# insitro/FastVim

Hardware: AMD Instinct MI355X
Metric: images/sec FastVim-T 224px bs=128/GPU fwd+bwd (+all-reduce +AdamW +EMA), whole job (higher is better)
Workload: dtype bf16; 1 GPU; FastVim-T 224x224 bs=128/GPU bf16 training step, synthetic ImageNet tensors (BASELINE configs[1]); global_batch=128, parallelism=dp1, hip_graph=True, optimizer_in_step=True, final_loss_hex=0x1.779ca20000000p+0

## Files before the change

### fastvim_amd/_lib.py

```python
import ctypes
import os
import threading

import torch

_PKG = os.path.dirname(os.path.abspath(__file__))
LIB_PATH = os.path.join(_PKG, "libfastvim_hip.so")

FV_F32, FV_BF16, FV_F16 = 0, 1, 2
_DTYPES = {torch.float32: FV_F32, torch.bfloat16: FV_BF16, torch.float16: FV_F16}

_lib = None

C_ABI_SYMBOLS = (
    "fv_last_error", "fv_version",
    "fv_selective_scan_fwd", "fv_selective_scan_bwd_workspace", "fv_selective_scan_bwd",
    "fv_causal_conv1d_fwd", "fv_causal_conv1d_bwd", "fv_scan_expand_skip_fwd",
    "fv_mixer_conv_pool_fwd", "fv_mixer_scan_fwd", "fv_mixer_xproj_scan_fwd_ok", "fv_mixer_xproj_scan_fwd", "fv_mixer_combine_fwd",
    "fv_mixer_bwd_blocks", "fv_mixer_combine_bwd", "fv_mixer_scan_bwd_chunks", "fv_mixer_scan_bwd_chunks_b",
    "fv_mixer_scan_bwd_ckpt_floats", "fv_mixer_scan_bwd_partials", "fv_mixer_scan_bwd", "fv_mixer_scan_bwd_dir", "fv_mixer_scan_bwd_ckpt", "fv_mixer_scan_bwd_segments", "fv_mixer_scan_bwd_seg_floats", "fv_mixer_scan_bwd_seg_partials", "fv_mixer_scan_bwd_seg_chunks", "fv_mixer_scan_bwd_seg", "fv_mixer_scan_fwd_ckpt", "fv_mixer_scan_ckpt_floats", "fv_mixer_scan_fwd_segments", "fv_mixer_scan_fwd_seg_floats", "fv_mixer_scan_fwd_seg", "fv_rows_segment_sum", "fv_rows_gather", "fv_mixer_conv_pool_bwd", "fv_mixer_conv_pool_bwd2_ok", "fv_mixer_conv_pool_bwd2", "fv_mixer_scan_bwd_xproj_ok", "fv_mixer_scan_bwd_xproj", "fv_chunk_rows_bf16", "fv_reduce_partials", "fv_reduce_partials_multi",
    "fv_add_norm_blocks", "fv_add_norm_fwd", "fv_add_norm_bwd", "fv_gemm_bf16", "fv_gemm_bf16_tn_grouped", "fv_gemm_bf16_tn_grouped_ld", "fv_mixer_xproj_fwd", "fv_mixer_xproj_bwd_slices", "fv_mixer_xproj_bwd", "fv_mixer_xproj_bwd2", "fv_mixer_xproj_bwd3_ok", "fv_mixer_xproj_bwd3", "fv_adamw_flat", "fv_soft_target_ce",
    "fv_patch_unfold", "fv_gemm_bf16_rowbias", "fv_mean_pool_fwd", "fv_mean_pool_bwd", "fv_droppath_table", "fv_scale_cast",
    "fv_column_sum", "fv_gemm_bf16_addnorm", "fv_gemm_bf16_dgrad_addnorm_blocks", "fv_gemm_bf16_dgrad_addnorm_bwd", "fv_gemm_bf16_dgrad_addnorm_bwd2", "fv_gemm_bf16_addnorm2", "fv_mixer_combine_out_proj_addnorm_ok", "fv_mixer_combine_out_proj_addnorm", "fv_gemm_f32",
    "fv_mixer_conv_pool_bwd_dgrad_ok", "fv_mixer_conv_pool_bwd_dgrad_blocks", "fv_mixer_conv_pool_bwd_dgrad", "fv_transpose_bf16_batched", "fv_gemm_bf16_tn_grouped_wide8",
    "fv_grad_sumsq_blocks", "fv_grad_sumsq_partials", "fv_adamw_flat_groups",
    "fv_pack_weight_frags_batched", "fv_mixer_conv_pool_bwd_dgrad_pk", "fv_mixer_combine_out_proj_addnorm_pk",
    "fv_mix_batch", "fv_patch_unfold_mix", "fv_mixup_target", "fv_label_ce",
    "fv_patch_unfold_chan", "fv_chan_embed_table", "fv_chan_embed_scatter",
    "fv_mixer_plan",
)


_tls = threading.local()


class _DeviceGuarded:

    def __init__(self, cdll):
        self._cdll = cdll
        self._wrapped = {}

    def __getattr__(self, name):
        w = self._wrapped.get(name)
        if w is None:
            fn = getattr(self._cdll, name)

            def call(*args, _fn=fn):
                dev = getattr(_tls, "dev", None)
                if dev is None or dev == torch.cuda.current_device():
                    return _fn(*args)
                with torch.cuda.device(dev):
                    return _fn(*args)

            w = self._wrapped[name] = call
        return w


def lib():
    global _lib
    if _lib is None:
        if not os.path.exists(LIB_PATH):
            raise RuntimeError(
                f"{LIB_PATH} is missing: build it with `python -m fastvim_amd.build` "
                "(or __graft_entry__.build()). fastvim_amd has no CPU / eager fallback.")
        cdll = ctypes.CDLL(LIB_PATH)
        cdll.fv_last_error.restype = ctypes.c_char_p
        cdll.fv_selective_scan_bwd_workspace.restype = ctypes.c_size_t
        cdll.fv_mixer_scan_bwd_ckpt_floats.restype = ctypes.c_size_t
        cdll.fv_mixer_scan_ckpt_floats.restype = ctypes.c_size_t
        cdll.fv_mixer_scan_fwd_seg_floats.restype = ctypes.c_size_t
        cdll.fv_mixer_scan_bwd_seg_floats.restype = ctypes.c_size_t
        _lib = _DeviceGuarded(cdll)
    return _lib


def dtype_code(dt):
    try:
        return _DTYPES[dt]
    except KeyError:
        raise RuntimeError(f"fastvim_amd: unsupported dtype {dt}") from None


def ptr(t):
    return ctypes.c_void_p(0 if t is None else t.data_ptr())


def stream_of(t):
    _tls.dev = t.device.index
    return ctypes.c_void_p(torch.cuda.current_stream(t.device).cuda_stream)


def require_gpu(*tensors):
    for t in tensors:
        if t is not None and not t.is_cuda:
            raise RuntimeError("fastvim_amd ops run on the GPU only (HIP kernels); got a CPU tensor")


def check(rc, what):
    if rc != 0:
        msg = lib().fv_last_error().decode()
        raise RuntimeError(f"{what}: {msg} (code {rc})")


def i32(v):
    return ctypes.c_int(int(v))
```

### fastvim_amd/csrc/combine_gemm.hip

```cpp
#include "mixer_common.h"
#include "packed.h"

namespace {

typedef __bf16 cg_bf16x8 __attribute__((ext_vector_type(8)));
typedef float cg_f32x4 __attribute__((ext_vector_type(4)));

constexpr int CG_K = 384, CG_N = 192, CG_BM = 64, CG_NT = 256;
constexpr int CG_RSA = CG_K * 2 + 16;
constexpr int CG_RSB = CG_N * 2 + 16;
constexpr int CG_PD = 6;
constexpr int CG_KS = CG_K / 32;
#ifndef CG_FORCE_PK
#define CG_FORCE_PK 0
#endif
#ifndef CG_DBG
#define CG_DBG 0
#endif

struct CgParams {
  const void* xz;
  const void* skip;
  const float* yc;
  const float *lnw, *lnb;
  void* g;
  float *mean, *rstd_ln;
  float ln_eps;
  Geo geo;
  int B;
  const bf16_t* W;
  long ldw;
  const float* residual;
  const float* nw;
  const float* row_scale;
  int rows_per_scale;
  float* res_out;
  bf16_t* y;
  float* rstd;
  float eps;
  int M;
  int d_in;
};

__device__ __forceinline__ float cg_hsum(f2 v) { return v.x + v.y; }

template <bool PK>
__global__ __launch_bounds__(CG_NT, 2) void combine_out_proj_addnorm_kernel(CgParams p) {
  extern __shared__ __attribute__((aligned(16))) char smem[];
  typedef PairVec<bf16_t, 3> P;
  const int tid = threadIdx.x, lane = tid & 63;
  const int wv = __builtin_amdgcn_readfirstlane(tid >> 6);
  const Geo g = p.geo;
  const int tiles = (g.rows + 3) / 4;
  const int bimg = blockIdx.x / tiles, i0 = (blockIdx.x - bimg * tiles) * 4;
  const int mimg = bimg * g.L;
  auto tok_of = [&](int rl) {
    const int w = rl >> 4, j = rl & 15;
    return (i0 + w < g.rows && j < g.cols) ? mimg + (i0 + w) * g.s_i + j * g.s_j : -1;
  };

  const int lr = lane % 16, gr = lane / 16;
  const int fn = lane & 15, fk = lane >> 4;
  const bf16_t* wrow[3];
  cg_bf16x8 fb[CG_PD][3];
  const char* wpk = reinterpret_cast<const char*>(p.W) + wv * (CG_KS * 3 * 1024);
  const uint32_t wpk_lane = (uint32_t)lane * 16;
  auto wfrag = [&](int nb, int ks) {
    if constexpr (PK) return *reinterpret_cast<const cg_bf16x8*>(wpk + (ks * 3 + nb) * 1024 + wpk_lane);
    else return *reinterpret_cast<const cg_bf16x8*>(wrow[nb] + ks * 32);
  };
  float4 ne_r[2][2][3], ne_w[3];
  float ne_sc[2][2];
  {
#pragma clang fp reassociate(off) contract(off)
    const int lc = lane * 6, voff = lc * 2;
    const int tok_x = 2 * CG_K * 2, tok_s = CG_K * 2;
    const bool has_ln = p.lnw != nullptr;
    const float inv_d = 1.f / (float)p.d_in;
    const size_t ydir = (size_t)p.B * g.rows * CG_K;
    const __amdgpu_buffer_rsrc_t bz = fv_make_buf((const bf16_t*)p.xz + CG_K, (size_t)p.M * tok_x - tok_s);
    const __amdgpu_buffer_rsrc_t bs = fv_make_buf(p.skip, (size_t)p.M * tok_s);
    const __amdgpu_buffer_rsrc_t bg = fv_make_buf(p.g, (size_t)p.M * tok_s);
    const __amdgpu_buffer_rsrc_t bmean = fv_make_buf(has_ln ? (const void*)p.mean : p.g, has_ln ? (size_t)p.M * 4 : 0);
    const __amdgpu_buffer_rsrc_t brstd = fv_make_buf(has_ln ? (const void*)p.rstd_ln : p.g, has_ln ? (size_t)p.M * 4 : 0);
    const int irow = i0 + wv;
    const bool wlive = irow < g.rows;
    const int irc = wlive ? irow : g.rows - 1;
    const int mbase = mimg + irc * g.s_i;
    char* arow = smem + (wv * 16) * CG_RSA + lane * 12;
    constexpr int TT = 2;
    const int npair = (g.cols + TT - 1) / TT;
    f2 ysum[3], ysf[3], ysb[3];
    {
      const float* yr = p.yc + ((size_t)bimg * g.rows + irc) * CG_K + lc;
#pragma unroll
      for (int q = 0; q < 3; ++q) {
        ysf[q] = *reinterpret_cast<const f2*>(yr + 2 * q);
        ysb[q] = *reinterpret_cast<const f2*>(yr + ydir + 2 * q);
      }
    }
    struct Pre { P sk[TT], z[TT]; };
    Pre pa, pb;
    auto fetch = [&](Pre& r, int j0) {
#pragma unroll
      for (int t = 0; t < TT; ++t) {
        const int m = mbase + min(j0 + t, g.cols - 1) * g.s_j;
        r.sk[t].load(bs, voff, m * tok_s);
        r.z[t].load(bz, voff, m * tok_x);
      }
    };
    fetch(pa, 0);
    fetch(pb, TT);
    __builtin_amdgcn_sched_barrier(0);
    f2 lw[3], lb[3];
    {
      const float* lwp = has_ln ? p.lnw : p.yc;
      const float* lbp = has_ln ? p.lnb : p.yc;
#pragma unroll
      for (int q = 0; q < 3; ++q) {
        lw[q] = *reinterpret_cast<const f2*>(lwp + lc + 2 * q);
        lb[q] = *reinterpret_cast<const f2*>(lbp + lc + 2 * q);
      }
    }
    __builtin_amdgcn_sched_barrier(0);
#pragma unroll
    for (int nb = 0; nb < 3; ++nb) wrow[nb] = PK ? nullptr : p.W + (long)(wv * 48 + nb * 16 + fn) * p.ldw + fk * 8;
#pragma unroll
    for (int s = 0; s < CG_PD; s += 2)
#pragma unroll
      for (int nb = 0; nb < 3; ++nb)
#pragma unroll
        for (int h = 0; h < 2; ++h) fb[s + h][nb] = wfrag(nb, s + h);
    __builtin_amdgcn_sched_barrier(0);
#pragma unroll
    for (int q = 0; q < 3; ++q) ysum[q] = ysf[q] + ysb[q];
    auto process = [&](Pre& r, int j0) {
      f2 o[TT][3], z[TT][3];
      float s1[TT], mean[TT], rstd[TT];
#pragma unroll
      for (int t = 0; t < TT; ++t)
#pragma unroll
        for (int q = 0; q < 3; ++q) {
          o[t][q] = r.sk[t].get(q);
          z[t][q] = r.z[t].get(q);
        }
      fetch(r, j0 + 2 * TT);
      __builtin_amdgcn_sched_barrier(0);
#pragma unroll
      for (int t = 0; t < TT; ++t) {
        f2 acc = splat(0.f);
#pragma unroll
        for (int q = 0; q < 3; ++q) {
          o[t][q] = (ysum[q] + o[t][q]) * 0.5f;
          acc += o[t][q];
        }
        s1[t] = cg_hsum(acc);
      }
      if (has_ln) {
#pragma unroll
        for (int t = 0; t < TT; ++t) s1[t] = wave_sum_uniform(s1[t]);
#pragma unroll
        for (int t = 0; t < TT; ++t) {
          mean[t] = s1[t] * inv_d;
          f2 acc = splat(0.f);
#pragma unroll
          for (int q = 0; q < 3; ++q) {
            const f2 d = o[t][q] - mean[t];
            acc = fma2(d, d, acc);
          }
          s1[t] = cg_hsum(acc);
        }
#pragma unroll
        for (int t = 0; t < TT; ++t) s1[t] = wave_sum_uniform(s1[t]);
#pragma unroll
        for (int t = 0; t < TT; ++t) rstd[t] = rsqrtf(s1[t] * inv_d + p.ln_eps);
      } else {
#pragma unroll
        for (int t = 0; t < TT; ++t) { mean[t] = 0.f; rstd[t] = 1.f; }
      }
#pragma unroll
      for (int t = 0; t < TT; ++t) {
        const bool live = wlive && j0 + t < g.cols;
        const int m = mbase + min(j0 + t, g.cols - 1) * g.s_j;
        f2 out[3];
#pragma unroll
        for (int q = 0; q < 3; ++q) {
          const f2 w_ = has_ln ? lw[q] : splat(1.f), b_ = has_ln ? lb[q] : splat(0.f);
          out[q] = fma2((o[t][q] - mean[t]) * rstd[t], w_, b_) * silu2(z[t][q]);
        }
        uint32_t pk[3];
#pragma unroll
        for (int q = 0; q < 3; ++q) pk[q] = live ? pack_bf16x2(out[q].x, out[q].y) : 0u;
        if (CG_DBG != 4) {
          fv_buf_store_words<3>(bg, live ? voff : 0x7ffffff0, m * tok_s, pk);
          const int so = (has_ln && live && lane == 0) ? 0 : 0x7ffffff0;
          const uint32_t mv[1] = {__float_as_uint(mean[t])}, rv[1] = {__float_as_uint(rstd[t])};
          fv_buf_store_words<1>(bmean, so, m * 4, mv);
          fv_buf_store_words<1>(brstd, so, m * 4, rv);
        }
        uint32_t* ar = reinterpret_cast<uint32_t*>(arow + (j0 + t) * CG_RSA);
        ar[0] = pk[0]; ar[1] = pk[1]; ar[2] = pk[2];
      }
    };
#pragma unroll 1
    for (int pr = 0; pr < (CG_DBG == 1 ? 0 : 8); pr += 2) {
      process(pa, pr * TT);
      process(pb, (pr + 1) * TT);
    }
    (void)npair;
#pragma unroll
    for (int it = 0; it < 2; ++it)
#pragma unroll
      for (int u = 0; u < 2; ++u) {
        const int m = tok_of(wv * 16 + it * 8 + u * 4 + gr), rowc = m >= 0 ? m : mimg;
#pragma unroll
        for (int k = 0; k < 3; ++k)
          ne_r[it][u][k] = *reinterpret_cast<const float4*>(p.residual + (size_t)rowc * CG_N + (k * 16 + lr) * 4);
        ne_sc[it][u] = (p.row_scale ? p.row_scale : p.nw)[p.row_scale ? rowc / p.rows_per_scale : 0];
      }
#pragma unroll
    for (int k = 0; k < 3; ++k) ne_w[k] = *reinterpret_cast<const float4*>(p.nw + (k * 16 + lr) * 4);
    __builtin_amdgcn_sched_barrier(0);
  }
  __syncthreads();

  cg_f32x4 acc[3][4];
#pragma unroll
  for (int a = 0; a < 3; ++a)
#pragma unroll
    for (int b = 0; b < 4; ++b) acc[a][b] = (cg_f32x4){0.f, 0.f, 0.f, 0.f};
  const char* afrag = smem + (lane & 15) * CG_RSA + (lane >> 4) * 16;
  static_assert(CG_PD % 2 == 0 && CG_KS % 2 == 0, "the weight ring is refilled in line pairs");
#pragma unroll
  for (int kp = 0; kp < (CG_DBG == 2 ? 0 : CG_KS); kp += 2) {
    cg_bf16x8 cur[2][3];
#pragma unroll
    for (int h = 0; h < 2; ++h)
#pragma unroll
      for (int nb = 0; nb < 3; ++nb) cur[h][nb] = fb[(kp + h) % CG_PD][nb];
    if (kp + CG_PD < CG_KS) {
#pragma unroll
      for (int nb = 0; nb < 3; ++nb)
#pragma unroll
        for (int h = 0; h < 2; ++h)
          fb[(kp + h) % CG_PD][nb] = wfrag(nb, kp + h + CG_PD);
    }
    __builtin_amdgcn_sched_barrier(0);
#pragma unroll
    for (int h = 0; h < 2; ++h) {
      cg_bf16x8 fa[4];
#pragma unroll
      for (int mb = 0; mb < 4; ++mb) fa[mb] = *reinterpret_cast<const cg_bf16x8*>(afrag + mb * 16 * CG_RSA + (kp + h) * 64);
#pragma unroll
      for (int a = 0; a < 3; ++a)
#pragma unroll
        for (int b = 0; b < 4; ++b) acc[a][b] = __builtin_amdgcn_mfma_f32_16x16x32_bf16(cur[h][a], fa[b], acc[a][b], 0, 0, 0);
    }
    __builtin_amdgcn_sched_barrier(0);
  }
  __syncthreads();

#pragma unroll
  for (int b = 0; b < 4; ++b)
#pragma unroll
    for (int a = 0; a < 3; ++a) {
      const cg_f32x4 v = acc[a][b];
      uint2 pk = {pack_bf16x2(v[0], v[1]), pack_bf16x2(v[2], v[3])};
      *reinterpret_cast<uint2*>(smem + (b * 16 + (lane & 15)) * CG_RSB + (wv * 48 + a * 16 + (lane >> 4) * 4) * 2) = pk;
    }
  __syncthreads();
  if (CG_DBG == 3) return;
  constexpr int LPR = 16, RPW = 4, RU = 2, RW = CG_BM / 4;
  const float inv_n = 1.f / (float)CG_N;
  float w[3][4];
#pragma unroll
  for (int k = 0; k < 3; ++k) {
    const float4 t = ne_w[k];
    w[k][0] = t.x; w[k][1] = t.y; w[k][2] = t.z; w[k][3] = t.w;
  }
#pragma unroll
  for (int it = 0; it < RW / (RPW * RU); ++it) {
    float v[RU][3][4], r[RU][3][4], sc_u[RU];
#pragma unroll
    for (int u = 0; u < RU; ++u) {
      const int rl = wv * RW + it * (RPW * RU) + u * RPW + gr;
      sc_u[u] = p.row_scale ? ne_sc[it][u] : 1.f;
#pragma unroll
      for (int k = 0; k < 3; ++k) {
        const int c = (k * LPR + lr) * 4;
        const uint2 xb = *reinterpret_cast<const uint2*>(smem + rl * CG_RSB + c * 2);
        v[u][k][0] = __uint_as_float(xb.x << 16); v[u][k][1] = __uint_as_float(xb.x & 0xffff0000u);
        v[u][k][2] = __uint_as_float(xb.y << 16); v[u][k][3] = __uint_as_float(xb.y & 0xffff0000u);
        const float4 t = ne_r[it][u][k];
        r[u][k][0] = t.x; r[u][k][1] = t.y; r[u][k][2] = t.z; r[u][k][3] = t.w;
      }
    }
#pragma unroll
    for (int u = 0; u < RU; ++u) {
      const int row = tok_of(wv * RW + it * (RPW * RU) + u * RPW + gr);
      const bool live = row >= 0;
      const size_t base = (size_t)(live ? row : mimg) * CG_N;
      const float sc = sc_u[u];
#pragma unroll
      for (int k = 0; k < 3; ++k) {
        const int c = (k * LPR + lr) * 4;
#pragma unroll
        for (int e = 0; e < 4; ++e) v[u][k][e] = fmaf(v[u][k][e], sc, r[u][k][e]);
        if (live) *reinterpret_cast<float4*>(p.res_out + base + c) = make_float4(v[u][k][0], v[u][k][1], v[u][k][2], v[u][k][3]);
      }
      float q = 0.f;
#pragma unroll
      for (int k = 0; k < 3; ++k)
#pragma unroll
        for (int e = 0; e < 4; ++e) q = fmaf(v[u][k][e], v[u][k][e], q);
#define FV_DPP_ADD(ctrl) q += __int_as_float(__builtin_amdgcn_update_dpp(0, __float_as_int(q), ctrl, 0xf, 0xf, true))
      FV_DPP_ADD(0xB1);
      FV_DPP_ADD(0x4E);
      FV_DPP_ADD(0x141);
      FV_DPP_ADD(0x140);
#undef FV_DPP_ADD
      const float rstd = rsqrtf(q * inv_n + p.eps);
      if (lr == 0 && live) p.rstd[row] = rstd;
#pragma unroll
      for (int k = 0; k < 3; ++k) {
        const int c = (k * LPR + lr) * 4;
        float o[4];
#pragma unroll
        for (int e = 0; e < 4; ++e) {
          float t = v[u][k][e] * rstd;
          asm volatile("" : "+v"(t));
          o[e] = t * w[k][e];
        }
        uint2 pk = {pack_bf16x2(o[0], o[1]), pack_bf16x2(o[2], o[3])};
        if (live) *reinterpret_cast<uint2*>(p.y + base + c) = pk;
      }
    }
  }
}

}

extern "C" int fv_mixer_combine_out_proj_addnorm_ok(int batch, int rows, int cols, int tokens_per_patch, int d_inner,
                                                    int d_model, int dtype) {
  return dtype == FV_BF16 && d_inner == CG_K && d_model == CG_N && tokens_per_patch == 1 && batch > 0 && rows > 0 &&
         cols > 0 && cols <= 16 && (long)batch * rows * cols * CG_K * 4 < 0x7fffffffL;
}

static int cg_launch(bool packed, const void* xz, const void* skip, const float* yc, const float* ln_w,
                                                 const float* ln_b, float ln_eps, void* g, float* mean, float* rstd_ln,
                                                 int batch, int rows, int cols, int tok_stride_row, int tok_stride_col,
                                                 const void* W, long ldw, const float* residual,
                                                 const float* norm_weight, const float* row_scale, int rows_per_scale,
                                                 void* y, float* residual_out, float* rstd, float eps,
                                                 fv_stream_t stream) {
  FV_CHECK(xz && skip && yc && g && W && residual && norm_weight && y && residual_out && rstd,
           "mixer_combine_out_proj_addnorm: null pointer");
  FV_CHECK(!ln_w || (ln_b && mean && rstd_ln), "mixer_combine_out_proj_addnorm: LayerNorm needs weight, bias, mean, rstd");
  FV_CHECK(fv_mixer_combine_out_proj_addnorm_ok(batch, rows, cols, 1, CG_K, CG_N, FV_BF16),
           "mixer_combine_out_proj_addnorm: shape not built (fv_mixer_combine_out_proj_addnorm_ok)");
  FV_CHECK((tok_stride_row == cols && tok_stride_col == 1) || (tok_stride_row == 1 && tok_stride_col == rows),
           "mixer_combine_out_proj_addnorm: token strides (%d,%d) are neither row-major nor transposed for a %dx%d grid",
           tok_stride_row, tok_stride_col, rows, cols);
  FV_CHECK(((uintptr_t)W & 15) == 0 && ldw % 8 == 0 && ldw >= CG_K, "mixer_combine_out_proj_addnorm: weight rows must be 16-byte aligned");
  FV_CHECK(!packed || ldw == CG_K, "mixer_combine_out_proj_addnorm_pk: the packed weight has no row padding (ldw = %d)", CG_K);
  FV_CHECK(((uintptr_t)residual & 15) == 0 && ((uintptr_t)residual_out & 15) == 0 && ((uintptr_t)y & 7) == 0 &&
               ((uintptr_t)norm_weight & 15) == 0, "mixer_combine_out_proj_addnorm: row operands must be 16-byte aligned");
  FV_CHECK(!row_scale || rows_per_scale > 0, "mixer_combine_out_proj_addnorm: rows_per_scale must be positive");
  CgParams p{};
  p.xz = xz; p.skip = skip; p.yc = yc; p.lnw = ln_w; p.lnb = ln_b; p.g = g; p.mean = mean; p.rstd_ln = rstd_ln;
  p.ln_eps = ln_eps;
  p.geo = make_geo(rows, cols, tok_stride_row, tok_stride_col, 1);
  p.B = batch;
  p.W = (const bf16_t*)W; p.ldw = ldw; p.residual = residual; p.nw = norm_weight; p.row_scale = row_scale;
  p.rows_per_scale = rows_per_scale; p.res_out = residual_out; p.y = (bf16_t*)y; p.rstd = rstd; p.eps = eps;
  p.M = batch * rows * cols;
  p.d_in = CG_K;
  const size_t smem = (size_t)CG_BM * CG_RSA;
  const dim3 grid(batch * fv_cdiv(rows, 4)), block(CG_NT);
  if (packed || CG_FORCE_PK) hipLaunchKernelGGL(combine_out_proj_addnorm_kernel<true>, grid, block, smem, (hipStream_t)stream, p);
  else hipLaunchKernelGGL(combine_out_proj_addnorm_kernel<false>, grid, block, smem, (hipStream_t)stream, p);
  FV_LAUNCH_CHECK();
  return FV_OK;
}

#define CG_ARGS_DECL                                                                                                          \
  const void *xz, const void *skip, const float *yc, const float *ln_w, const float *ln_b, float ln_eps, void *g,             \
      float *mean, float *rstd_ln, int batch, int rows, int cols, int tok_stride_row, int tok_stride_col, const void *W,      \
      long ldw, const float *residual, const float *norm_weight, const float *row_scale, int rows_per_scale, void *y,         \
      float *residual_out, float *rstd, float eps, fv_stream_t stream
#define CG_ARGS                                                                                                               \
  xz, skip, yc, ln_w, ln_b, ln_eps, g, mean, rstd_ln, batch, rows, cols, tok_stride_row, tok_stride_col, W, ldw, residual,    \
      norm_weight, row_scale, rows_per_scale, y, residual_out, rstd, eps, stream

extern "C" int fv_mixer_combine_out_proj_addnorm(CG_ARGS_DECL) { return cg_launch(false, CG_ARGS); }

extern "C" int fv_mixer_combine_out_proj_addnorm_pk(CG_ARGS_DECL) { return cg_launch(true, CG_ARGS); }
```

### fastvim_amd/csrc/glue.hip

```cpp
#include "common.h"

namespace {

typedef uint32_t u32x4 __attribute__((ext_vector_type(4)));
typedef uint32_t u32x2 __attribute__((ext_vector_type(2)));

template <typename T> struct Vec4;
template <> struct Vec4<float> {
  static __device__ __forceinline__ void ld(const float* p, float (&v)[4]) {
    const float4 t = *reinterpret_cast<const float4*>(p);
    v[0] = t.x; v[1] = t.y; v[2] = t.z; v[3] = t.w;
  }
  static __device__ __forceinline__ void st(float* p, const float (&v)[4]) {
    *reinterpret_cast<float4*>(p) = make_float4(v[0], v[1], v[2], v[3]);
  }
};
template <> struct Vec4<bf16_t> {
  static __device__ __forceinline__ void ld(const bf16_t* p, float (&v)[4]) {
    const u32x2 t = *reinterpret_cast<const u32x2*>(p);
    v[0] = __uint_as_float(t.x << 16); v[1] = __uint_as_float(t.x & 0xffff0000u);
    v[2] = __uint_as_float(t.y << 16); v[3] = __uint_as_float(t.y & 0xffff0000u);
  }
  static __device__ __forceinline__ void st(bf16_t* p, const float (&v)[4]) {
    u32x2 t;
    t.x = pack_bf16x2(v[0], v[1]);
    t.y = pack_bf16x2(v[2], v[3]);
    *reinterpret_cast<u32x2*>(p) = t;
  }
};

constexpr int UNF_GJ = 16;

template <typename TI, typename TO>
__global__ __launch_bounds__(256) void patch_unfold_kernel(const TI* __restrict__ img, TO* __restrict__ out, int C, int H,
                                                           int W, int ph, int pw, int gw) {
  extern __shared__ __attribute__((aligned(16))) char smem[];
  TO* tile = reinterpret_cast<TO*>(smem);
  const int gj0 = blockIdx.x * UNF_GJ, gi = blockIdx.y, b = blockIdx.z;
  const int gjn = min(UNF_GJ, gw - gj0);
  const int Kp = C * ph * pw;
  const int xv = gjn * pw / 4;
  const TI* src = img + ((size_t)b * C * H + (size_t)gi * ph) * W + (size_t)gj0 * pw;
  for (int e = threadIdx.x; e < C * ph * xv; e += blockDim.x) {
    const int row = e / xv, x = (e - row * xv) * 4;
    const int c = row / ph, pi = row - c * ph;
    float v[4];
    Vec4<TI>::ld(src + ((size_t)c * H + pi) * W + x, v);
    const int gj = x / pw, pj = x - gj * pw;
    Vec4<TO>::st(tile + (size_t)gj * Kp + row * pw + pj, v);
  }
  __syncthreads();
  TO* dst = out + (((size_t)b * gridDim.y + gi) * gw + gj0) * Kp;
  constexpr int EV = 16 / sizeof(TO);
  const int nv = gjn * Kp / EV;
  for (int e = threadIdx.x; e < nv; e += blockDim.x)
    reinterpret_cast<u32x4*>(dst)[e] = reinterpret_cast<const u32x4*>(tile)[e];
}

__device__ __forceinline__ int sel_channel(const int32_t* __restrict__ sel, int k, int Ctot) {
  return sel ? min(max(sel[k], 0), Ctot - 1) : k;
}

template <typename TI, typename TO, bool COLWISE>
__global__ __launch_bounds__(256) void patch_unfold_chan_kernel(const TI* __restrict__ img, TO* __restrict__ out,
                                                                const int32_t* __restrict__ sel, int n, int Ctot, int H, int W,
                                                                int ph, int pw, int gw, int gjc) {
  extern __shared__ __attribute__((aligned(16))) char smem[];
  TO* tile = reinterpret_cast<TO*>(smem);
  const int gj0 = blockIdx.x * gjc, gi = blockIdx.y, b = blockIdx.z, gh = gridDim.y;
  const int gjn = min(gjc, gw - gj0);
  const int Kp = n * ph * pw;
  const int xv = gjn * pw / 4;
  const TI* src = img + ((size_t)b * Ctot * H + (size_t)gi * ph) * W + (size_t)gj0 * pw;
  for (int e = threadIdx.x; e < n * ph * xv; e += blockDim.x) {
    const int row = e / xv, x = (e - row * xv) * 4;
    const int k = row / ph, pi = row - k * ph;
    float v[4];
    Vec4<TI>::ld(src + ((size_t)sel_channel(sel, k, Ctot) * H + pi) * W + x, v);
    const int gj = x / pw, pj = x - gj * pw;
    Vec4<TO>::st(tile + (size_t)gj * Kp + row * pw + pj, v);
  }
  __syncthreads();
  constexpr int EV = 16 / sizeof(TO);
  if constexpr (!COLWISE) {
    TO* dst = out + (((size_t)b * gh + gi) * gw + gj0) * Kp;
    const int nv = gjn * Kp / EV;
    for (int e = threadIdx.x; e < nv; e += blockDim.x)
      reinterpret_cast<u32x4*>(dst)[e] = reinterpret_cast<const u32x4*>(tile)[e];
  } else {
    const int pv = Kp / EV;
    for (int e = threadIdx.x; e < gjn * pv; e += blockDim.x) {
      const int gj = e / pv, r = e - gj * pv;
      TO* dst = out + (((size_t)b * gw + gj0 + gj) * gh + gi) * Kp;
      reinterpret_cast<u32x4*>(dst)[r] = reinterpret_cast<const u32x4*>(tile)[e];
    }
  }
}

__global__ __launch_bounds__(256) void chan_embed_table_kernel(const float* __restrict__ chan, const float* __restrict__ bias,
                                                               const float* __restrict__ pos, float* __restrict__ table,
                                                               const int32_t* __restrict__ sel, int n, int Ctot, int D, size_t total) {
#pragma clang fp reassociate(off) contract(off)
  for (size_t i = (size_t)blockIdx.x * blockDim.x + threadIdx.x; i < total; i += (size_t)gridDim.x * blockDim.x) {
    const int d = (int)(i % D);
    const size_t t = i / D;
    const int k = (int)(t % n);
    const size_t p = t / n;
    float v = chan[(size_t)sel_channel(sel, k, Ctot) * D + d];
    if (bias) v = v + bias[d];
    if (pos) v = v + pos[p * D + d];
    table[i] = v;
  }
}

__global__ __launch_bounds__(256) void chan_embed_scatter_kernel(const float* __restrict__ d_chan, float* __restrict__ d_table,
                                                                 const int32_t* __restrict__ sel, int n, int Ctot, int D) {
  const int i = blockIdx.x * blockDim.x + threadIdx.x;
  if (i >= n * D) return;
  const int k = i / D, d = i - k * D;
  const int c = sel ? sel[k] : k;
  if (c < 0 || c >= Ctot) return;
  d_table[(size_t)c * D + d] += d_chan[i];
}

template <typename T> __device__ __forceinline__ float round_as(float v);
template <> __device__ __forceinline__ float round_as<float>(float v) {
  asm("" : "+v"(v));
  return v;
}
template <> __device__ __forceinline__ float round_as<bf16_t>(float v) { return bf16_bits_to_f32(f32_to_bf16_bits(v)); }

enum { MIX_COPY = 0, MIX_MIXUP = 1, MIX_CUTMIX = 2 };
__device__ __forceinline__ int mix_mode(const fv_mix_params& P) {
  return P.use_cutmix ? MIX_CUTMIX : (P.lam == 1.f ? MIX_COPY : MIX_MIXUP);
}

template <typename T, int N>
__device__ __forceinline__ void mix_pixels(const fv_mix_params& P, int mode, int y, int x0, const float (&a)[N], const float (&p)[N],
                                           float (&oa)[N], float (&op)[N]) {
#pragma clang fp reassociate(off) contract(off)
  if (mode == MIX_MIXUP) {
#pragma unroll
    for (int k = 0; k < N; ++k) {
      oa[k] = round_as<T>(round_as<T>(a[k] * P.lam) + round_as<T>(p[k] * P.one_minus_lam));
      op[k] = round_as<T>(round_as<T>(p[k] * P.lam) + round_as<T>(a[k] * P.one_minus_lam));
    }
  } else {
    const bool in_rows = mode == MIX_CUTMIX && y >= P.yl && y < P.yh;
#pragma unroll
    for (int k = 0; k < N; ++k) {
      const bool in_box = in_rows && x0 + k >= P.xl && x0 + k < P.xh;
      oa[k] = in_box ? p[k] : a[k];
      op[k] = in_box ? a[k] : p[k];
    }
  }
}

template <typename T, int EV>
__global__ __launch_bounds__(256) void mix_batch_kernel(const T* __restrict__ x, T* __restrict__ out,
                                                        const fv_mix_params* __restrict__ mp, int B, int n, int H, int W) {
  const fv_mix_params P = *mp;
  const int mode = mix_mode(P);
  const size_t oa_ = (size_t)blockIdx.y * n, op_ = (size_t)(B - 1 - blockIdx.y) * n;
  for (int e = blockIdx.x * blockDim.x + threadIdx.x; e < n / EV; e += gridDim.x * blockDim.x) {
    const int i = e * EV, row = i / W;
    float a[EV], p[EV], ra[EV], rp[EV];
    if constexpr (EV == 4) {
      Vec4<T>::ld(x + oa_ + i, a);
      Vec4<T>::ld(x + op_ + i, p);
    } else {
      a[0] = io<T>::ld(x + oa_ + i);
      p[0] = io<T>::ld(x + op_ + i);
    }
    mix_pixels<T, EV>(P, mode, row % H, i - row * W, a, p, ra, rp);
    if constexpr (EV == 4) {
      Vec4<T>::st(out + oa_ + i, ra);
      Vec4<T>::st(out + op_ + i, rp);
    } else {
      io<T>::st(out + oa_ + i, ra[0]);
      io<T>::st(out + op_ + i, rp[0]);
    }
  }
}

template <typename TI, typename TO>
__global__ __launch_bounds__(1024) void patch_unfold_mix_kernel(const TI* __restrict__ img, TO* __restrict__ out,
                                                               const fv_mix_params* __restrict__ mp, int B, int C, int H, int W,
                                                               int ph, int pw, int gw, int gjc) {
  extern __shared__ __attribute__((aligned(16))) char smem[];
  const fv_mix_params P = *mp;
  const int mode = mix_mode(P);
  const int gj0 = blockIdx.x * gjc, gi = blockIdx.y, ba = blockIdx.z, bp = B - 1 - ba;
  const int gjn = min(gjc, gw - gj0);
  const int Kp = C * ph * pw;
  const int xv = gjn * pw / 4;
  TO* tile_a = reinterpret_cast<TO*>(smem);
  TO* tile_p = tile_a + (size_t)gjc * Kp;
  const size_t org = (size_t)gi * ph * W + (size_t)gj0 * pw;
  const TI* src_a = img + (size_t)ba * C * H * W + org;
  const TI* src_p = img + (size_t)bp * C * H * W + org;
  for (int e = threadIdx.x; e < C * ph * xv; e += blockDim.x) {
    const int row = e / xv, x = (e - row * xv) * 4;
    const int c = row / ph, pi = row - c * ph;
    const size_t off = ((size_t)c * H + pi) * W + x;
    float a[4], p[4], ra[4], rp[4];
    Vec4<TI>::ld(src_a + off, a);
    Vec4<TI>::ld(src_p + off, p);
    mix_pixels<TI, 4>(P, mode, gi * ph + pi, gj0 * pw + x, a, p, ra, rp);
    const int gj = x / pw, pj = x - gj * pw;
    const size_t t = (size_t)gj * Kp + row * pw + pj;
    Vec4<TO>::st(tile_a + t, ra);
    Vec4<TO>::st(tile_p + t, rp);
  }
  __syncthreads();
  const size_t chunk = ((size_t)gi * gw + gj0) * Kp, image = (size_t)gridDim.y * gw * Kp;
  TO* dst_a = out + (size_t)ba * image + chunk;
  TO* dst_p = out + (size_t)bp * image + chunk;
  constexpr int EV = 16 / sizeof(TO);
  const int nv = gjn * Kp / EV;
  for (int e = threadIdx.x; e < nv; e += blockDim.x) {
    reinterpret_cast<u32x4*>(dst_a)[e] = reinterpret_cast<const u32x4*>(tile_a)[e];
    reinterpret_cast<u32x4*>(dst_p)[e] = reinterpret_cast<const u32x4*>(tile_p)[e];
  }
}

template <typename T> struct Vec2;
template <> struct Vec2<float> {
  static __device__ __forceinline__ void ld(const float* p, float (&v)[2]) {
    const float2 t = *reinterpret_cast<const float2*>(p);
    v[0] = t.x; v[1] = t.y;
  }
  static __device__ __forceinline__ void st(float* p, float a, float b) { *reinterpret_cast<float2*>(p) = make_float2(a, b); }
};
template <> struct Vec2<bf16_t> {
  static __device__ __forceinline__ void ld(const bf16_t* p, float (&v)[2]) {
    const uint32_t t = *reinterpret_cast<const uint32_t*>(p);
    v[0] = __uint_as_float(t << 16); v[1] = __uint_as_float(t & 0xffff0000u);
  }
  static __device__ __forceinline__ void st(bf16_t* p, float a, float b) { *reinterpret_cast<uint32_t*>(p) = pack_bf16x2(a, b); }
};
template <typename T, int LV> __device__ __forceinline__ void ld_row(const T* p, float (&v)[LV]) {
  if constexpr (LV == 4) Vec4<T>::ld(p, v); else Vec2<T>::ld(p, v);
}

template <typename TO, int LV>
__device__ __forceinline__ void place_pairs(TO* tile, int Kp, int pw, int row, int x, const float (&v)[LV]) {
#pragma unroll
  for (int h = 0; h < LV; h += 2) {
    const int gj = (x + h) / pw, pj = (x + h) - gj * pw;
    Vec2<TO>::st(tile + (size_t)gj * Kp + row * pw + pj, v[h], v[h + 1]);
  }
}

template <typename TO>
__device__ __forceinline__ void drain_tile(TO* dst, const TO* tile, int n, int sw) {
  const int nb = n * (int)sizeof(TO);
  if (sw == 16) {
    for (int e = threadIdx.x; e < nb / 16; e += blockDim.x) reinterpret_cast<u32x4*>(dst)[e] = reinterpret_cast<const u32x4*>(tile)[e];
  } else if (sw == 8) {
    for (int e = threadIdx.x; e < nb / 8; e += blockDim.x) reinterpret_cast<u32x2*>(dst)[e] = reinterpret_cast<const u32x2*>(tile)[e];
  } else {
    for (int e = threadIdx.x; e < nb / 4; e += blockDim.x) reinterpret_cast<uint32_t*>(dst)[e] = reinterpret_cast<const uint32_t*>(tile)[e];
  }
}

template <typename TI, typename TO, int LV>
__global__ __launch_bounds__(256) void patch_unfold_even_kernel(const TI* __restrict__ img, TO* __restrict__ out, int C, int H,
                                                                int W, int ph, int pw, int gw, int sw) {
  extern __shared__ __attribute__((aligned(16))) char smem[];
  TO* tile = reinterpret_cast<TO*>(smem);
  const int gj0 = blockIdx.x * UNF_GJ, gi = blockIdx.y, b = blockIdx.z;
  const int gjn = min(UNF_GJ, gw - gj0);
  const int Kp = C * ph * pw;
  const int xv = gjn * pw / LV;
  const TI* src = img + ((size_t)b * C * H + (size_t)gi * ph) * W + (size_t)gj0 * pw;
  for (int e = threadIdx.x; e < C * ph * xv; e += blockDim.x) {
    const int row = e / xv, x = (e - row * xv) * LV;
    const int c = row / ph, pi = row - c * ph;
    float v[LV];
    ld_row<TI, LV>(src + ((size_t)c * H + pi) * W + x, v);
    place_pairs<TO, LV>(tile, Kp, pw, row, x, v);
  }
  __syncthreads();
  drain_tile<TO>(out + (((size_t)b * gridDim.y + gi) * gw + gj0) * Kp, tile, gjn * Kp, sw);
}

template <typename TI, typename TO, int LV>
__global__ __launch_bounds__(1024) void patch_unfold_mix_even_kernel(const TI* __restrict__ img, TO* __restrict__ out,
                                                                    const fv_mix_params* __restrict__ mp, int B, int C, int H,
                                                                    int W, int ph, int pw, int gw, int gjc, int sw) {
  extern __shared__ __attribute__((aligned(16))) char smem[];
  const fv_mix_params P = *mp;
  const int mode = mix_mode(P);
  const int gj0 = blockIdx.x * gjc, gi = blockIdx.y, ba = blockIdx.z, bp = B - 1 - ba;
  const int gjn = min(gjc, gw - gj0);
  const int Kp = C * ph * pw;
  const int xv = gjn * pw / LV;
  TO* tile_a = reinterpret_cast<TO*>(smem);
  TO* tile_p = tile_a + (size_t)gjc * Kp;
  const size_t org = (size_t)gi * ph * W + (size_t)gj0 * pw;
  const TI* src_a = img + (size_t)ba * C * H * W + org;
  const TI* src_p = img + (size_t)bp * C * H * W + org;
  for (int e = threadIdx.x; e < C * ph * xv; e += blockDim.x) {
    const int row = e / xv, x = (e - row * xv) * LV;
    const int c = row / ph, pi = row - c * ph;
    const size_t off = ((size_t)c * H + pi) * W + x;
    float a[LV], p[LV], ra[LV], rp[LV];
    ld_row<TI, LV>(src_a + off, a);
    ld_row<TI, LV>(src_p + off, p);
    mix_pixels<TI, LV>(P, mode, gi * ph + pi, gj0 * pw + x, a, p, ra, rp);
    place_pairs<TO, LV>(tile_a, Kp, pw, row, x, ra);
    place_pairs<TO, LV>(tile_p, Kp, pw, row, x, rp);
  }
  __syncthreads();
  const size_t chunk = ((size_t)gi * gw + gj0) * Kp, image = (size_t)gridDim.y * gw * Kp;
  drain_tile<TO>(out + (size_t)ba * image + chunk, tile_a, gjn * Kp, sw);
  drain_tile<TO>(out + (size_t)bp * image + chunk, tile_p, gjn * Kp, sw);
}

constexpr int MP_WAVES = 16;
template <typename T>
__global__ __launch_bounds__(64 * MP_WAVES) void mean_pool_fwd_kernel(const T* __restrict__ x, T* __restrict__ out, int L, int D, float inv) {
  __shared__ float s_acc[MP_WAVES][256];
  const int lane = threadIdx.x & 63, wv = threadIdx.x >> 6;
  const int d = (blockIdx.x * 64 + lane) * 4, b = blockIdx.y;
  float a[4] = {0.f, 0.f, 0.f, 0.f};
  if (d < D) {
    const T* xp = x + (size_t)b * L * D + d;
    int l = wv;
    for (; l + 3 * MP_WAVES < L; l += 4 * MP_WAVES) {
      float v[4][4];
#pragma unroll
      for (int u = 0; u < 4; ++u) Vec4<T>::ld(xp + (size_t)(l + u * MP_WAVES) * D, v[u]);
#pragma unroll
      for (int u = 0; u < 4; ++u)
#pragma unroll
        for (int k = 0; k < 4; ++k) a[k] += v[u][k];
    }
    for (; l < L; l += MP_WAVES) {
      float v[4];
      Vec4<T>::ld(xp + (size_t)l * D, v);
#pragma unroll
      for (int k = 0; k < 4; ++k) a[k] += v[k];
    }
  }
#pragma unroll
  for (int k = 0; k < 4; ++k) s_acc[wv][lane * 4 + k] = a[k];
  __syncthreads();
  if (wv == 0 && d < D) {
    float r[4];
#pragma unroll
    for (int k = 0; k < 4; ++k) {
      float t = 0.f;
#pragma unroll
      for (int w = 0; w < MP_WAVES; ++w) t += s_acc[w][lane * 4 + k];
      r[k] = t * inv;
    }
    Vec4<T>::st(out + (size_t)b * D + d, r);
  }
}

template <typename T>
__global__ __launch_bounds__(256) void mean_pool_bwd_kernel(const T* __restrict__ g, T* __restrict__ dx, int L, int D,
                                                            int rows_per_block, float inv) {
  const int b = blockIdx.y, dv = D / 4;
  const int l0 = blockIdx.x * rows_per_block, l1 = min(L, l0 + rows_per_block);
  for (int e = threadIdx.x; e < (l1 - l0) * dv; e += blockDim.x) {
    const int l = l0 + e / dv, d = (e % dv) * 4;
    float v[4];
    Vec4<T>::ld(g + (size_t)b * D + d, v);
#pragma unroll
    for (int k = 0; k < 4; ++k) v[k] *= inv;
    Vec4<T>::st(dx + ((size_t)b * L + l) * D + d, v);
  }
}

__global__ __launch_bounds__(256) void droppath_table_kernel(float* __restrict__ table, const float* __restrict__ keep,
                                                             const float* __restrict__ inv, int mods, int batch) {
  const int i = blockIdx.x * blockDim.x + threadIdx.x;
  if (i < mods * batch) {
    const int m = i / batch;
    table[i] = floorf(table[i] + keep[m]) * inv[m];
  }
}

template <typename T>
__global__ __launch_bounds__(256) void scale_cast_kernel(const float* __restrict__ x, const float* __restrict__ scale,
                                                         T* __restrict__ y, size_t n) {
  const float s = scale[0];
  for (size_t i = (size_t)blockIdx.x * blockDim.x + threadIdx.x; i < n; i += (size_t)gridDim.x * blockDim.x)
    io<T>::st(y + i, x[i] * s);
}

template <typename T>
__global__ __launch_bounds__(256) void column_sum_kernel(const T* __restrict__ x, float* __restrict__ out, int rows, int cols,
                                                         int accumulate) {
  __shared__ float s_acc[4][64];
  const int lane = threadIdx.x & 63, wv = threadIdx.x >> 6, c = blockIdx.x * 64 + lane;
  float a = 0.f;
  if (c < cols)
    for (int r = wv; r < rows; r += 4) a += io<T>::ld(x + (size_t)r * cols + c);
  s_acc[wv][lane] = a;
  __syncthreads();
  if (wv == 0 && c < cols) {
    const float t = (s_acc[0][lane] + s_acc[1][lane]) + (s_acc[2][lane] + s_acc[3][lane]);
    out[c] = accumulate ? out[c] + t : t;
  }
}

bool dt_ok(int dt) { return dt == FV_F32 || dt == FV_BF16; }


constexpr int TRJ_MAX = 64;
struct TransposeJobs {
  const uint16_t* src[TRJ_MAX];
  uint16_t* dst[TRJ_MAX];
  int rows, cols;
};
__global__ __launch_bounds__(256) void transpose_bf16_kernel(TransposeJobs J) {
  __shared__ uint16_t t[32][33];
  const uint16_t* src = J.src[blockIdx.z];
  uint16_t* dst = J.dst[blockIdx.z];
  const int r0 = blockIdx.y * 32, c0 = blockIdx.x * 32, tx = threadIdx.x & 31, ty = threadIdx.x >> 5;
#pragma unroll
  for (int i = 0; i < 4; ++i) {
    const int r = r0 + ty + 8 * i, c = c0 + tx;
    t[ty + 8 * i][tx] = (r < J.rows && c < J.cols) ? src[(size_t)r * J.cols + c] : (uint16_t)0;
  }
  __syncthreads();
#pragma unroll
  for (int i = 0; i < 4; ++i) {
    const int c = c0 + ty + 8 * i, r = r0 + tx;
    if (r < J.rows && c < J.cols) dst[(size_t)c * J.rows + r] = t[tx][ty + 8 * i];
  }
}


constexpr int PKW_ROWS = 192;
struct PackJobs {
  const uint4* src[TRJ_MAX];
  uint4* dst[TRJ_MAX];
  int ks_n;
};
__global__ __launch_bounds__(256) void pack_weight_frags_kernel(PackJobs J) {
  const int u = blockIdx.x * 256 + threadIdx.x;
  if (u >= PKW_ROWS * J.ks_n * 4) return;
  const int lane = u & 63, t = u >> 6, nb = t % 3, ks = (t / 3) % J.ks_n, wv = t / (3 * J.ks_n);
  const int row = 48 * wv + 16 * nb + (lane & 15), unit_in_row = 4 * ks + (lane >> 4);
  J.dst[blockIdx.y][u] = J.src[blockIdx.y][row * (J.ks_n * 4) + unit_in_row];
}

int unfold_store_bytes(int gw, int gjc, size_t patch_bytes) {
  int a = gw, b = gjc;
  while (b) { const int t = a % b; a = b; b = t; }
  const size_t unit = (size_t)a * patch_bytes;
  return unit % 16 == 0 ? 16 : unit % 8 == 0 ? 8 : 4;
}

}

extern "C" int fv_patch_unfold(const void* img, int img_dtype, void* out, int out_dtype, int batch, int chans, int height,
                               int width, int ph, int pw, fv_stream_t stream) {
  FV_CHECK(img && out, "patch_unfold: null pointer");
  FV_CHECK(dt_ok(img_dtype) && dt_ok(out_dtype), "patch_unfold: dtypes must be fp32 or bf16");
  FV_CHECK(batch > 0 && chans > 0 && ph > 0 && pw > 0 && height >= ph && width >= pw, "patch_unfold: empty dimension");
  FV_CHECK(height % ph == 0 && width % pw == 0, "patch_unfold: image %dx%d is not whole %dx%d patches", height, width, ph, pw);
  FV_CHECK(pw % 2 == 0 && pw >= 8 && ((uintptr_t)img & 15) == 0 && ((uintptr_t)out & 15) == 0,
           "patch_unfold: patch width must be even and at least 8, and the buffers 16-byte aligned");
  const int gh = height / ph, gw = width / pw;
  const size_t osz = out_dtype == FV_F32 ? 4 : 2;
  const size_t smem = (size_t)UNF_GJ * chans * ph * pw * osz;
  FV_CHECK(smem <= 64 * 1024, "patch_unfold: %d x %d x %d patches do not fit the staging tile", chans, ph, pw);
  FV_CHECK(gh <= 65535 && batch <= 65535, "patch_unfold: grid too large");
  const dim3 grid(fv_cdiv(gw, UNF_GJ), gh, batch), block(256);
  hipStream_t st = (hipStream_t)stream;
  if (pw % 8 != 0) {
    const int sw = unfold_store_bytes(gw, UNF_GJ, (size_t)chans * ph * pw * osz);
#define FV_UNFE(TI, TO) do { if (width % 4 == 0) hipLaunchKernelGGL((patch_unfold_even_kernel<TI, TO, 4>), grid, block, smem, st, (const TI*)img, (TO*)out, chans, height, width, ph, pw, gw, sw); \
                             else hipLaunchKernelGGL((patch_unfold_even_kernel<TI, TO, 2>), grid, block, smem, st, (const TI*)img, (TO*)out, chans, height, width, ph, pw, gw, sw); } while (0)
    if (img_dtype == FV_F32 && out_dtype == FV_BF16) FV_UNFE(float, bf16_t);
    else if (img_dtype == FV_F32) FV_UNFE(float, float);
    else if (out_dtype == FV_BF16) FV_UNFE(bf16_t, bf16_t);
    else FV_UNFE(bf16_t, float);
#undef FV_UNFE
    FV_LAUNCH_CHECK();
    return FV_OK;
  }
#define FV_UNF(TI, TO) hipLaunchKernelGGL((patch_unfold_kernel<TI, TO>), grid, block, smem, st, (const TI*)img, (TO*)out, chans, height, width, ph, pw, gw)
  if (img_dtype == FV_F32 && out_dtype == FV_BF16) FV_UNF(float, bf16_t);
  else if (img_dtype == FV_F32) FV_UNF(float, float);
  else if (out_dtype == FV_BF16) FV_UNF(bf16_t, bf16_t);
  else FV_UNF(bf16_t, float);
#undef FV_UNF
  FV_LAUNCH_CHECK();
  return FV_OK;
}

extern "C" int fv_patch_unfold_chan(const void* img, int img_dtype, void* out, int out_dtype, int batch, int chans_total,
                                    int height, int width, int ph, int pw, const int32_t* sel, int n_sel, int colwise,
                                    fv_stream_t stream) {
  FV_CHECK(img && out, "patch_unfold_chan: null pointer");
  FV_CHECK(dt_ok(img_dtype) && dt_ok(out_dtype), "patch_unfold_chan: dtypes must be fp32 or bf16");
  FV_CHECK(batch > 0 && chans_total > 0 && ph > 0 && pw > 0 && height >= ph && width >= pw, "patch_unfold_chan: empty dimension");
  FV_CHECK(n_sel > 0 && n_sel <= chans_total, "patch_unfold_chan: %d selected channels of %d", n_sel, chans_total);
  FV_CHECK(height % ph == 0 && width % pw == 0, "patch_unfold_chan: image %dx%d is not whole %dx%d patches", height, width, ph, pw);
  FV_CHECK(pw % 8 == 0 && ((uintptr_t)img & 15) == 0 && ((uintptr_t)out & 15) == 0,
           "patch_unfold_chan: patch width must be a multiple of 8 and the buffers 16-byte aligned");
  const int gh = height / ph, gw = width / pw;
  const size_t osz = out_dtype == FV_F32 ? 4 : 2;
  const size_t per_patch = (size_t)n_sel * ph * pw * osz;
  FV_CHECK(per_patch <= 64 * 1024, "patch_unfold_chan: %d x %d x %d patches do not fit the staging tile", n_sel, ph, pw);
  int fit = (int)((32 * 1024) / per_patch);
  fit = fit < 1 ? 1 : (fit > UNF_GJ ? UNF_GJ : fit);
  const int gjc = fv_cdiv(gw, fv_cdiv(gw, fit));
  const size_t smem = gjc * per_patch;
  FV_CHECK(gh <= 65535 && batch <= 65535, "patch_unfold_chan: grid too large");
  const dim3 grid(fv_cdiv(gw, gjc), gh, batch), block(256);
  hipStream_t st = (hipStream_t)stream;
#define FV_UNFC2(TI, TO, CW) hipLaunchKernelGGL((patch_unfold_chan_kernel<TI, TO, CW>), grid, block, smem, st, (const TI*)img, (TO*)out, sel, n_sel, chans_total, height, width, ph, pw, gw, gjc)
#define FV_UNFC(TI, TO) do { if (colwise) FV_UNFC2(TI, TO, true); else FV_UNFC2(TI, TO, false); } while (0)
  if (img_dtype == FV_F32 && out_dtype == FV_BF16) FV_UNFC(float, bf16_t);
  else if (img_dtype == FV_F32) FV_UNFC(float, float);
  else if (out_dtype == FV_BF16) FV_UNFC(bf16_t, bf16_t);
  else FV_UNFC(bf16_t, float);
#undef FV_UNFC
#undef FV_UNFC2
  FV_LAUNCH_CHECK();
  return FV_OK;
}

extern "C" int fv_chan_embed_table(const float* chan_table, const float* bias, const float* pos, float* table, const int32_t* sel,
                                   int n_sel, int chans_total, int positions, int dim, fv_stream_t stream) {
  FV_CHECK(chan_table && table, "chan_embed_table: null pointer");
  FV_CHECK(n_sel > 0 && n_sel <= chans_total && positions > 0 && dim > 0, "chan_embed_table: bad shape (%d of %d channels, %d positions, dim %d)",
           n_sel, chans_total, positions, dim);
  const size_t total = (size_t)positions * n_sel * dim;
  const long blocks = fv_cdiv((long)total, 256l);
  hipLaunchKernelGGL(chan_embed_table_kernel, dim3((unsigned)(blocks < 4096 ? blocks : 4096)), dim3(256), 0, (hipStream_t)stream,
                     chan_table, bias, pos, table, sel, n_sel, chans_total, dim, total);
  FV_LAUNCH_CHECK();
  return FV_OK;
}

extern "C" int fv_chan_embed_scatter(const float* d_chan, float* d_table, const int32_t* sel, int n_sel, int chans_total, int dim,
                                     fv_stream_t stream) {
  FV_CHECK(d_chan && d_table, "chan_embed_scatter: null pointer");
  FV_CHECK(n_sel > 0 && n_sel <= chans_total && dim > 0 && (long)n_sel * dim < (1l << 31), "chan_embed_scatter: bad shape (%d of %d channels, dim %d)",
           n_sel, chans_total, dim);
  hipLaunchKernelGGL(chan_embed_scatter_kernel, dim3(fv_cdiv(n_sel * dim, 256)), dim3(256), 0, (hipStream_t)stream,
                     d_chan, d_table, sel, n_sel, chans_total, dim);
  FV_LAUNCH_CHECK();
  return FV_OK;
}

extern "C" int fv_mix_batch(const void* x, void* out, int dtype, int batch, int chans, int height, int width, const void* mix,
                            fv_stream_t stream) {
  FV_CHECK(x && out && mix && x != out, "mix_batch: null or aliased pointer (the op is out of place)");
  FV_CHECK(dt_ok(dtype), "mix_batch: dtype must be fp32 or bf16");
  FV_CHECK(batch > 0 && chans > 0 && height > 0 && width > 0, "mix_batch: empty dimension");
  FV_CHECK(batch % 2 == 0, "mix_batch: batch mode pairs image b with image batch-1-b, the batch (%d) must be even", batch);
  const long n = (long)chans * height * width;
  FV_CHECK(n < (1l << 31) && batch / 2 <= 65535, "mix_batch: image or batch too large");
  const size_t esz = dtype == FV_F32 ? 4 : 2;
  const bool vec = width % 4 == 0 && ((uintptr_t)x % (4 * esz)) == 0 && ((uintptr_t)out % (4 * esz)) == 0;
  const long work = vec ? n / 4 : n;
  const dim3 grid(fv_cdiv(work, 256) < 1024 ? fv_cdiv(work, 256) : 1024, batch / 2), block(256);
  hipStream_t st = (hipStream_t)stream;
  const fv_mix_params* mp = (const fv_mix_params*)mix;
#define FV_MIXB(T, EV) hipLaunchKernelGGL((mix_batch_kernel<T, EV>), grid, block, 0, st, (const T*)x, (T*)out, mp, batch, (int)n, height, width)
  if (dtype == FV_F32) { if (vec) FV_MIXB(float, 4); else FV_MIXB(float, 1); }
  else { if (vec) FV_MIXB(bf16_t, 4); else FV_MIXB(bf16_t, 1); }
#undef FV_MIXB
  FV_LAUNCH_CHECK();
  return FV_OK;
}

extern "C" int fv_patch_unfold_mix(const void* img, int img_dtype, void* out, int out_dtype, int batch, int chans, int height,
                                   int width, int ph, int pw, const void* mix, fv_stream_t stream) {
  FV_CHECK(img && out && mix, "patch_unfold_mix: null pointer");
  FV_CHECK(dt_ok(img_dtype) && dt_ok(out_dtype), "patch_unfold_mix: dtypes must be fp32 or bf16");
  FV_CHECK(batch > 0 && chans > 0 && ph > 0 && pw > 0 && height >= ph && width >= pw, "patch_unfold_mix: empty dimension");
  FV_CHECK(batch % 2 == 0, "patch_unfold_mix: batch mode pairs image b with image batch-1-b, the batch (%d) must be even", batch);
  FV_CHECK(height % ph == 0 && width % pw == 0, "patch_unfold_mix: image %dx%d is not whole %dx%d patches", height, width, ph, pw);
  FV_CHECK(pw % 2 == 0 && pw >= 8 && ((uintptr_t)img & 15) == 0 && ((uintptr_t)out & 15) == 0,
           "patch_unfold_mix: patch width must be even and at least 8, and the buffers 16-byte aligned");
  const int gh = height / ph, gw = width / pw;
  const size_t osz = out_dtype == FV_F32 ? 4 : 2;
  const size_t per_patch = 2 * (size_t)chans * ph * pw * osz;
  const int gjc = fv_tune("FASTVIM_UNFOLD_MIX_GJ", UNF_GJ / 2);
  const int threads = fv_tune("FASTVIM_UNFOLD_MIX_THREADS", 512);
  const size_t smem = gjc * per_patch;
  FV_CHECK(gjc > 0 && smem <= 64 * 1024, "patch_unfold_mix: %d x %d x %d patches do not fit the staging tiles", chans, ph, pw);
  FV_CHECK(threads >= 64 && threads <= 1024 && threads % 64 == 0, "patch_unfold_mix: bad workgroup size %d", threads);
  FV_CHECK(gh <= 65535 && batch / 2 <= 65535, "patch_unfold_mix: grid too large");
  const dim3 grid(fv_cdiv(gw, gjc), gh, batch / 2), block(threads);
  hipStream_t st = (hipStream_t)stream;
  const fv_mix_params* mp = (const fv_mix_params*)mix;
  if (pw % 8 != 0) {
    FV_CHECK(gjc % 2 == 0, "patch_unfold_mix: patch width %d needs an even number of patches per tile (got %d)", pw, gjc);
    const int sw = unfold_store_bytes(gw, gjc, (size_t)chans * ph * pw * osz);
#define FV_UNFME(TI, TO) do { if (width % 4 == 0) hipLaunchKernelGGL((patch_unfold_mix_even_kernel<TI, TO, 4>), grid, block, smem, st, (const TI*)img, (TO*)out, mp, batch, chans, height, width, ph, pw, gw, gjc, sw); \
                              else hipLaunchKernelGGL((patch_unfold_mix_even_kernel<TI, TO, 2>), grid, block, smem, st, (const TI*)img, (TO*)out, mp, batch, chans, height, width, ph, pw, gw, gjc, sw); } while (0)
    if (img_dtype == FV_F32 && out_dtype == FV_BF16) FV_UNFME(float, bf16_t);
    else if (img_dtype == FV_F32) FV_UNFME(float, float);
    else if (out_dtype == FV_BF16) FV_UNFME(bf16_t, bf16_t);
    else FV_UNFME(bf16_t, float);
#undef FV_UNFME
    FV_LAUNCH_CHECK();
    return FV_OK;
  }
#define FV_UNFM(TI, TO) hipLaunchKernelGGL((patch_unfold_mix_kernel<TI, TO>), grid, block, smem, st, (const TI*)img, (TO*)out, mp, batch, chans, height, width, ph, pw, gw, gjc)
  if (img_dtype == FV_F32 && out_dtype == FV_BF16) FV_UNFM(float, bf16_t);
  else if (img_dtype == FV_F32) FV_UNFM(float, float);
  else if (out_dtype == FV_BF16) FV_UNFM(bf16_t, bf16_t);
  else FV_UNFM(bf16_t, float);
#undef FV_UNFM
  FV_LAUNCH_CHECK();
  return FV_OK;
}

extern "C" int fv_mean_pool_fwd(const void* x, void* out, int batch, int tokens, int dim, int dtype, fv_stream_t stream) {
  FV_CHECK(x && out, "mean_pool_fwd: null pointer");
  FV_CHECK(dt_ok(dtype), "mean_pool_fwd: dtype must be fp32 or bf16");
  FV_CHECK(batch > 0 && tokens > 0 && dim > 0 && dim % 4 == 0 && batch <= 65535, "mean_pool_fwd: bad shape (%d, %d, %d)", batch, tokens, dim);
  const dim3 grid(fv_cdiv(dim, 256), batch), block(64 * MP_WAVES);
  hipStream_t st = (hipStream_t)stream;
  const float inv = 1.f / (float)tokens;
  if (dtype == FV_F32) hipLaunchKernelGGL(mean_pool_fwd_kernel<float>, grid, block, 0, st, (const float*)x, (float*)out, tokens, dim, inv);
  else hipLaunchKernelGGL(mean_pool_fwd_kernel<bf16_t>, grid, block, 0, st, (const bf16_t*)x, (bf16_t*)out, tokens, dim, inv);
  FV_LAUNCH_CHECK();
  return FV_OK;
}

extern "C" int fv_mean_pool_bwd(const void* g, void* dx, int batch, int tokens, int dim, int dtype, fv_stream_t stream) {
  FV_CHECK(g && dx, "mean_pool_bwd: null pointer");
  FV_CHECK(dt_ok(dtype), "mean_pool_bwd: dtype must be fp32 or bf16");
  FV_CHECK(batch > 0 && tokens > 0 && dim > 0 && dim % 4 == 0 && batch <= 65535, "mean_pool_bwd: bad shape (%d, %d, %d)", batch, tokens, dim);
  const int rpb = fv_cdiv(tokens, 8);
  const dim3 grid(fv_cdiv(tokens, rpb), batch), block(256);
  hipStream_t st = (hipStream_t)stream;
  const float inv = 1.f / (float)tokens;
  if (dtype == FV_F32) hipLaunchKernelGGL(mean_pool_bwd_kernel<float>, grid, block, 0, st, (const float*)g, (float*)dx, tokens, dim, rpb, inv);
  else hipLaunchKernelGGL(mean_pool_bwd_kernel<bf16_t>, grid, block, 0, st, (const bf16_t*)g, (bf16_t*)dx, tokens, dim, rpb, inv);
  FV_LAUNCH_CHECK();
  return FV_OK;
}

extern "C" int fv_droppath_table(float* table, const float* keep, const float* inv_keep, int mods, int batch, fv_stream_t stream) {
  FV_CHECK(table && keep && inv_keep && mods > 0 && batch > 0, "droppath_table: bad arguments");
  hipLaunchKernelGGL(droppath_table_kernel, dim3(fv_cdiv((long)mods * batch, 256)), dim3(256), 0, (hipStream_t)stream, table, keep,
                     inv_keep, mods, batch);
  FV_LAUNCH_CHECK();
  return FV_OK;
}

extern "C" int fv_scale_cast(const float* x, const float* scale, void* y, int y_dtype, size_t n, fv_stream_t stream) {
  FV_CHECK(x && scale && y && n > 0, "scale_cast: bad arguments");
  FV_CHECK(dt_ok(y_dtype), "scale_cast: output must be fp32 or bf16");
  const dim3 grid(fv_cdiv((long)n, 256) < 2048 ? fv_cdiv((long)n, 256) : 2048), block(256);
  hipStream_t st = (hipStream_t)stream;
  if (y_dtype == FV_F32) hipLaunchKernelGGL(scale_cast_kernel<float>, grid, block, 0, st, x, scale, (float*)y, n);
  else hipLaunchKernelGGL(scale_cast_kernel<bf16_t>, grid, block, 0, st, x, scale, (bf16_t*)y, n);
  FV_LAUNCH_CHECK();
  return FV_OK;
}

extern "C" int fv_column_sum(const void* x, int dtype, float* out, int rows, int cols, int accumulate, fv_stream_t stream) {
  FV_CHECK(x && out && rows > 0 && cols > 0, "column_sum: bad arguments");
  FV_CHECK(dt_ok(dtype), "column_sum: input must be fp32 or bf16");
  const dim3 grid(fv_cdiv(cols, 64)), block(256);
  hipStream_t st = (hipStream_t)stream;
  if (dtype == FV_F32) hipLaunchKernelGGL(column_sum_kernel<float>, grid, block, 0, st, (const float*)x, out, rows, cols, accumulate);
  else hipLaunchKernelGGL(column_sum_kernel<bf16_t>, grid, block, 0, st, (const bf16_t*)x, out, rows, cols, accumulate);
  FV_LAUNCH_CHECK();
  return FV_OK;
}

extern "C" int fv_transpose_bf16_batched(const void* const* srcs, void* const* dsts, int njobs, int rows, int cols,
                                         fv_stream_t stream) {
  FV_CHECK(srcs && dsts && njobs > 0 && njobs <= TRJ_MAX, "transpose_bf16_batched: 1..%d jobs", TRJ_MAX);
  FV_CHECK(rows > 0 && cols > 0 && fv_cdiv(rows, 32) <= 65535, "transpose_bf16_batched: bad shape (%d, %d)", rows, cols);
  TransposeJobs J{};
  for (int j = 0; j < njobs; ++j) {
    FV_CHECK(srcs[j] && dsts[j], "transpose_bf16_batched: null pointer in job %d", j);
    J.src[j] = (const uint16_t*)srcs[j];
    J.dst[j] = (uint16_t*)dsts[j];
  }
  J.rows = rows; J.cols = cols;
  hipLaunchKernelGGL(transpose_bf16_kernel, dim3(fv_cdiv(cols, 32), fv_cdiv(rows, 32), njobs), dim3(256), 0, (hipStream_t)stream, J);
  FV_LAUNCH_CHECK();
  return FV_OK;
}

extern "C" int fv_pack_weight_frags_batched(const void* const* srcs, void* const* dsts, int njobs, int K, fv_stream_t stream) {
  FV_CHECK(srcs && dsts && njobs > 0 && njobs <= TRJ_MAX, "pack_weight_frags_batched: 1..%d jobs", TRJ_MAX);
  FV_CHECK(K == 384 || K == 768, "pack_weight_frags_batched: K = %d is not a built reduction length (384, 768)", K);
  PackJobs J{};
  for (int j = 0; j < njobs; ++j) {
    FV_CHECK(srcs[j] && dsts[j] && srcs[j] != dsts[j], "pack_weight_frags_batched: null or aliased pointer in job %d", j);
    FV_CHECK(((uintptr_t)srcs[j] & 15) == 0 && ((uintptr_t)dsts[j] & 15) == 0, "pack_weight_frags_batched: job %d is not 16-byte aligned", j);
    J.src[j] = (const uint4*)srcs[j];
    J.dst[j] = (uint4*)dsts[j];
  }
  J.ks_n = K / 32;
  hipLaunchKernelGGL(pack_weight_frags_kernel, dim3(fv_cdiv(PKW_ROWS * J.ks_n * 4, 256), njobs), dim3(256), 0, (hipStream_t)stream, J);
  FV_LAUNCH_CHECK();
  return FV_OK;
}
```

### fastvim_amd/flat.py

```python
import ctypes
import os
import re
import warnings

import torch
import torch.distributed as dist

from . import _lib as L
from .layernorm import RMSNorm
from .mamba_simple_faster import Mamba, _GroupedWgrad, _SideStream, flush_wgrads, group_wgrads
from .mixer_ops import defer_reductions, drop_reductions, flush_reductions, pending_reductions

_LAYER_RE = re.compile(r"^((?:.*\.)?[A-Za-z_]*layers\.\d+)\.")

_MIXER_GROUPS = (
    ("conv", ("conv1d.weight", "conv1d_b.weight", "conv1d.bias", "conv1d_b.bias", "D", "D_b")),
    ("scan", ("A_log", "dt_proj.weight", "dt_proj.bias", "A_b_log", "dt_proj_b.weight", "dt_proj_b.bias")),
    ("ln", ("layernorm.weight", "layernorm.bias")),
    ("xproj", ("x_proj.weight", "x_proj_b.weight")),
)


def _drop_derived_shadows(model):
    for p in model.parameters():
        for a in ("_fv_shadow_t", "_fv_shadow_t_version", "_fv_shadow_pk", "_fv_shadow_pk_version"):
            if hasattr(p, a):
                delattr(p, a)
    for mod in model.modules():
        fv = mod.__dict__.get("_fv")
        if isinstance(fv, dict):
            fv.pop("Wx2_shadow_t", None)
            fv.pop("Wx2_t_params", None)


class FlatTrainingState:
    def __init__(self, model, shadow_dtype=torch.bfloat16, process_group=None, comm_dtype=None,
                 chunk_bytes=256 << 20):
        self.group = process_group
        self.comm_dtype = comm_dtype
        self.chunk = max(1, chunk_bytes // 4)
        self._model = model
        _drop_derived_shadows(model)
        named = dict(model.named_parameters())
        mixers = {mname: mod for mname, mod in model.named_modules() if isinstance(mod, Mamba)}
        units, unit_of = [], {}
        for n, p in named.items():
            if not p.requires_grad:
                continue
            m_ = _LAYER_RE.match(n)
            key = m_.group(1) if m_ else None
            if key is None:
                if not units or units[-1][0] is not None:
                    units.append((None, []))
                units[-1][1].append(n)
            else:
                if key not in unit_of:
                    unit_of[key] = len(units)
                    units.append((key, []))
                units[unit_of[key]][1].append(n)
        order, regions = [], []
        self.units = []
        for key, names in units:
            front = []
            for mname, mod in mixers.items():
                if key is not None and (mname + ".").startswith(key + "."):
                    for gname, keys in _MIXER_GROUPS:
                        full = [f"{mname}.{k}" if mname else k for k in keys]
                        if all(f in named and named[f].requires_grad for f in full):
                            regions.append((mod, gname, full))
                            front += full
            rest = [n for n in names if n not in set(front)]
            self.units.append((key, len(order), len(order) + len(front) + len(rest)))
            order += front + rest
        if not any(k is not None for k, _ in units):
            for mname, mod in mixers.items():
                for gname, keys in _MIXER_GROUPS:
                    full = [f"{mname}.{k}" if mname else k for k in keys]
                    if all(f in named and named[f].requires_grad for f in full):
                        regions.append((mod, gname, full))
            front = [f for _, _, full in regions for f in full]
            order = front + [n for n in order if n not in set(front)]
            self.units = [(None, 0, len(order))]
        self.names = order
        params = [named[n] for n in order]
        dev = params[0].device
        offs, off = [], 0
        for p in params:
            offs.append(off)
            off += (p.numel() + 7) // 8 * 8
        self.param_flat = torch.zeros(off, device=dev, dtype=torch.float32)
        self.grad_flat = torch.zeros(off, device=dev, dtype=torch.float32)
        self.shadow_flat = torch.zeros(off, device=dev, dtype=shadow_dtype)
        self.offsets = dict(zip(order, offs))
        total = off
        self.unit_ranges = [(key, offs[i0] if i0 < len(offs) else total, offs[i1] if i1 < len(offs) else total)
                            for key, i0, i1 in self.units if i1 > i0]
        with torch.no_grad():
            for n, p, o in zip(order, params, offs):
                k = p.numel()
                self.param_flat[o:o + k].copy_(p.detach().reshape(-1))
                p.data = self.param_flat[o:o + k].view_as(p)
                p.grad = self.grad_flat[o:o + k].view_as(p)
                p._fv_shadow = self.shadow_flat[o:o + k].view_as(p)
                p._fv_shadow_version = -1
        self._params = params
        for mod, gname, full in regions:
            lo = self.offsets[full[0]]
            last = named[full[-1]]
            hi = self.offsets[full[-1]] + last.numel()
            contiguous = all(self.offsets[a] + named[a].numel() == self.offsets[b]
                             for a, b in zip(full[:-1], full[1:]))
            if not contiguous:
                continue
            fv = mod.__dict__.setdefault("_fv", {})
            fv[gname + "_grad"] = self.grad_flat[lo:hi]
            if gname == "xproj":
                shp = (2,) + tuple(named[full[0]].shape)
                fv["Wx2"] = self.param_flat[lo:hi].view(shp)
                fv["Wx2_shadow"] = self.shadow_flat[lo:hi].view(shp)
                fv["Wx2_grad"] = self.grad_flat[lo:hi].view(shp)
        for mod in model.modules():
            if isinstance(mod, (RMSNorm, torch.nn.LayerNorm, torch.nn.Linear, torch.nn.Conv2d)) and getattr(mod, "weight", None) is not None:
                if mod.weight.requires_grad:
                    mod.weight._fv_direct = True
                b = getattr(mod, "bias", None)
                if isinstance(mod, (torch.nn.Linear, torch.nn.Conv2d)) and b is not None and b.requires_grad:
                    b._fv_direct = True
        pe = getattr(model, "pos_embed", None)
        if isinstance(pe, torch.nn.Parameter) and pe.requires_grad:
            pe._fv_direct = True
        self._t_src, self._t_dst, self._t_params = [], [], []
        if shadow_dtype == torch.bfloat16 and dev.type == "cuda":
            for mod in mixers.values():
                w = mod.in_proj.weight
                if tuple(w.shape) == (768, 192) and w.requires_grad and getattr(w, "_fv_shadow", None) is not None:
                    wt = torch.empty(192, 768, device=dev, dtype=shadow_dtype)
                    w._fv_shadow_t = wt
                    w._fv_shadow_t_version = -1
                    self._t_src.append(w._fv_shadow)
                    self._t_dst.append(wt)
                    self._t_params.append(w)
        self._pk_jobs = {768: ([], [], []), 384: ([], [], [])}
        if shadow_dtype == torch.bfloat16 and dev.type == "cuda":
            for w, wt in zip(self._t_params, self._t_dst):
                self._add_packed(768, w, wt)
            for mod in mixers.values():
                w = getattr(getattr(mod, "out_proj", None), "weight", None)
                if w is not None and tuple(w.shape) == (192, 384) and w.requires_grad and getattr(w, "_fv_shadow", None) is not None:
                    self._add_packed(384, w, w._fv_shadow)
        self._pk_dst = self._pk_jobs[768][1] + self._pk_jobs[384][1]
        self._tx_src, self._tx_dst, self._tx_params = [], [], []
        if shadow_dtype == torch.bfloat16 and dev.type == "cuda":
            for mod in mixers.values():
                fv = mod.__dict__.get("_fv", {})
                ws = fv.get("Wx2_shadow")
                if ws is None or ws.dtype != torch.bfloat16:
                    continue
                _, Wd, d_in = ws.shape
                if d_in >= 768 and d_in % 64 == 0 and Wd % 8 == 0:
                    wt = torch.empty(2, d_in, Wd, device=dev, dtype=shadow_dtype)
                    fv["Wx2_shadow_t"] = wt
                    fv["Wx2_t_params"] = (mod.x_proj.weight, mod.x_proj_b.weight)
                    for k in range(2):
                        self._tx_src.append(ws[k])
                        self._tx_dst.append(wt[k])
                    for w in fv["Wx2_t_params"]:
                        w._fv_shadow_t_version = -1
                        self._tx_params.append(w)
        self.refresh_shadow()
        self._hook = model.register_load_state_dict_post_hook(lambda module, incompatible: self.refresh_shadow())
        from .mixer_ops import _Deferred
        self._saved_switches = (_Deferred.enabled, _GroupedWgrad.enabled, _SideStream.enabled)
        defer_reductions(True)
        group_wgrads(True)
        _SideStream.enabled = False

    def _add_packed(self, K, w, src):
        pk = torch.empty(192 * K, device=src.device, dtype=src.dtype)
        w._fv_shadow_pk = pk
        w._fv_shadow_pk_version = -1
        srcs, dsts, params = self._pk_jobs[K]
        srcs.append(src)
        dsts.append(pk)
        params.append(w)

    def close(self):
        if self._saved_switches is None:
            return
        self.finish_backward()
        d, g, s_ = self._saved_switches
        defer_reductions(d)
        group_wgrads(g)
        _SideStream.enabled = s_
        self._hook.remove()
        self._saved_switches = None
        _drop_derived_shadows(self._model)

    def __enter__(self):
        return self

    def __exit__(self, *exc):
        self.close()
        return False

    def zero_grad(self):
        _SideStream.join()
        n = len(_GroupedWgrad.jobs) + len(_GroupedWgrad.sums) + pending_reductions()
        if n:
            _GroupedWgrad.jobs = []
            _GroupedWgrad.sums = []
            _GroupedWgrad.rows_jobs = []
            drop_reductions()
            warnings.warn(f"FlatTrainingState.zero_grad(): {n} queued gradient jobs of an unfinished backward pass "
                          "were discarded -- call finish_backward() (or allreduce_mean_() / optimizer.step()) after "
                          "loss.backward()", RuntimeWarning, stacklevel=2)
        self.grad_flat.zero_()

    def finish_backward(self):
        flush_wgrads()
        flush_reductions()

    def refresh_shadow(self):
        self.shadow_flat.copy_(self.param_flat)
        for p in self._params:
            p._fv_shadow_version = p._version
        self.refresh_transposed()

    def refresh_transposed(self):
        from .mixer_ops import pack_weight_frags, transpose_bf16_batched
        for src, dst, params in ((self._t_src, self._t_dst, self._t_params),
                                 (getattr(self, "_tx_src", []), getattr(self, "_tx_dst", []), getattr(self, "_tx_params", []))):
            if src:
                transpose_bf16_batched(src, dst)
                for p in params:
                    p._fv_shadow_t_version = p._version
        for srcs, dsts, params in getattr(self, "_pk_jobs", {}).values():
            if srcs:
                pack_weight_frags(srcs, dsts)
                for p in params:
                    p._fv_shadow_pk_version = p._version

    @property
    def world_size(self):
        return dist.get_world_size(self.group) if dist.is_initialized() else 1

    def buckets(self, n_buckets, taper=True):
        blocks = [(i, u) for i, u in enumerate(self.unit_ranges) if u[0] is not None]
        if not blocks:
            return [{"bounds": (0, self.grad_flat.numel()), "layers": (0, 0)}]
        first_u, last_u = blocks[0][0], blocks[-1][0]
        nb = len(blocks)
        n_buckets = max(1, min(n_buckets, nb))
        sizes = [u[2] - u[1] for _, u in blocks]
        w = [i + 2 if taper else 1 for i in range(n_buckets)]
        cum = [sum(sizes) * sum(w[:i + 1]) / sum(w) for i in range(n_buckets)]
        runs, acc, lo = [], 0, 0
        for j, sz in enumerate(sizes):
            acc += sz
            left = nb - 1 - j
            if (len(runs) < n_buckets - 1 and acc >= cum[len(runs)] - 1e-9 and left >= n_buckets - 1 - len(runs)) \
                    or j == nb - 1:
                runs.append((lo, j + 1))
                lo = j + 1
        out = []
        for k, (a, b) in enumerate(runs):
            e0 = self.unit_ranges[first_u + a][1] if k > 0 else 0
            e1 = self.unit_ranges[first_u + b - 1][2] if k < len(runs) - 1 else self.grad_flat.numel()
            out.append({"bounds": (e0, e1), "layers": (a, b)})
        return out[::-1]

    def make_exchange(self, n_buckets=1):
        from .ddp import GradExchange
        bk = self.buckets(n_buckets)
        self.exchange = GradExchange(self.grad_flat, [b["bounds"] for b in bk], self.group, self.comm_dtype, self.chunk * 4)
        self.exchange.layers = [b["layers"] for b in bk]
        return self.exchange

    def allreduce_mean_(self):
        self._allreduce(True)

    def allreduce_sum_(self):
        self._allreduce(False)

    def _allreduce(self, mean):
        self.finish_backward()
        if self.world_size == 1:
            return
        if getattr(self, "exchange", None) is None:
            self.make_exchange(1)
        self.exchange.allreduce_(mean=mean)


MAX_PARAM_GROUPS = 256


def build_group_map(names, offsets, sizes, total, groups, default_weight_decay=0.0):
    known = set(names)
    rows, table, per_name = {}, [], {}
    ids = torch.zeros(total, dtype=torch.uint8)
    for g in groups:
        key = (float(g.get("lr_scale", 1.0)), float(g.get("weight_decay", default_weight_decay)))
        for n in g["params"]:
            if n not in known:
                raise ValueError(f"param_groups: {n!r} is not a trainable parameter of the flat training state")
            if n in per_name:
                raise ValueError(f"param_groups: parameter {n!r} appears in more than one group")
            if key not in rows:
                if len(table) == MAX_PARAM_GROUPS:
                    raise ValueError(f"param_groups: more than {MAX_PARAM_GROUPS} distinct (lr_scale, weight_decay) pairs "
                                     "(the fused optimizer keeps one group byte per element)")
                rows[key] = len(table)
                table.append(key)
            per_name[n] = key
            ids[offsets[n]:offsets[n] + sizes[n]] = rows[key]
    missing = [n for n in names if n not in per_name]
    if missing:
        raise ValueError(f"param_groups: {len(missing)} trainable parameters of the flat training state are in no group: "
                         f"{missing[:4]} ...")
    return ids, table, per_name


def groups_from_named(per_name):
    out = {}
    for n, (scale, wd) in per_name.items():
        key = (float(scale), float(wd))
        out.setdefault(key, {"lr_scale": key[0], "weight_decay": key[1], "params": []})["params"].append(n)
    return list(out.values())


class FlatAdamW:

    def __init__(self, flat, model, lr=1e-3, betas=(0.9, 0.999), eps=1e-8, weight_decay=0.05, no_decay=(),
                 ema_decay=None, param_groups=None, max_grad_norm=None, skip_nonfinite=False):
        self.flat = flat
        dev = flat.param_flat.device
        n = flat.param_flat.numel()
        self.exp_avg = torch.zeros(n, device=dev, dtype=torch.float32)
        self.exp_avg_sq = torch.zeros(n, device=dev, dtype=torch.float32)
        self.ema = flat.param_flat.clone() if ema_decay is not None else None
        self.ema_decay = float(ema_decay or 0.0)
        no_decay = set(no_decay)
        self.lr = torch.full((1,), float(lr), device=dev, dtype=torch.float32)
        self.step_t = torch.zeros(1, device=dev, dtype=torch.float32)
        self.betas, self.eps, self.weight_decay = betas, eps, weight_decay
        self.skip_nonfinite = bool(skip_nonfinite)
        self._grouped = param_groups is not None or max_grad_norm is not None or self.skip_nonfinite
        self.group_ids = self.group_table = self.max_norm = self.partials = self.stats = None
        self._group_row_of = None
        self.decay_mask = None
        if not self._grouped:
            mask = torch.zeros(n, dtype=torch.uint8)
            named = dict(model.named_parameters())
            for name, off in flat.offsets.items():
                if name not in no_decay:
                    mask[off:off + named[name].numel()] = 1
            self.decay_mask = mask.to(dev)
        else:
            if param_groups is None:
                groups = [{"params": [nm for nm in flat.names if nm not in no_decay], "weight_decay": weight_decay},
                          {"params": [nm for nm in flat.names if nm in no_decay], "weight_decay": 0.0}]
                groups = [g for g in groups if g["params"]]
            else:
                name_of = {id(p): nm for nm, p in zip(flat.names, flat._params)}
                groups = []
                for g in param_groups:
                    names = []
                    for q in g["params"]:
                        nm = q if isinstance(q, str) else name_of.get(id(q))
                        if nm is None:
                            raise ValueError("param_groups: a parameter of a group is not a trainable parameter of the "
                                             "flat training state")
                        names.append(nm)
                    groups.append({**g, "params": names})
            self._group_table_full = torch.zeros(MAX_PARAM_GROUPS, 2, device=dev, dtype=torch.float32)
            self.group_ids = torch.zeros(n, device=dev, dtype=torch.uint8)
            self._set_groups(groups)
            if max_grad_norm is not None or self.skip_nonfinite:
                G = int(L.lib().fv_grad_sumsq_blocks(ctypes.c_size_t(n)))
                self.partials = torch.zeros(G, device=dev, dtype=torch.float32)
                self.stats = torch.zeros(4, device=dev, dtype=torch.float32)
            if max_grad_norm is not None:
                self.max_norm = torch.full((1,), float(max_grad_norm), device=dev, dtype=torch.float32)

    def _set_groups(self, groups):
        f = self.flat
        sizes = {nm: p.numel() for nm, p in zip(f.names, f._params)}
        ids, table, per_name = build_group_map(f.names, f.offsets, sizes, f.param_flat.numel(), groups, self.weight_decay)
        rows = {key: i for i, key in enumerate(table)}
        with torch.no_grad():
            self.group_ids.copy_(ids)
            self._group_table_full.zero_()
            self._group_table_full[:len(table)].copy_(torch.tensor(table, dtype=torch.float32).view(-1, 2))
        self._group_row_of = {nm: rows[key] for nm, key in per_name.items()}
        self.group_table = self._group_table_full[:len(table)]

    def set_lr(self, lr):
        self.lr.fill_(float(lr))

    def set_max_grad_norm(self, v):
        if self.max_norm is None:
            raise RuntimeError("FlatAdamW was built without max_grad_norm")
        self.max_norm.fill_(float(v))

    def last_stats(self):
        if self.stats is None:
            raise RuntimeError("FlatAdamW was built without max_grad_norm / skip_nonfinite: no gradient norm is computed")
        t, c, fin, sk = self.stats.tolist()
        return {"total_norm": t, "clip_coef": c, "finite": bool(fin), "skipped_steps": int(sk)}

    def _named_slices(self, buf):
        f = self.flat
        named = dict(zip(f.names, f._params))
        return {n: buf[o:o + named[n].numel()].view_as(named[n]) for n, o in f.offsets.items()}

    def state_dict(self):
        ea, es = self._named_slices(self.exp_avg), self._named_slices(self.exp_avg_sq)
        return {"state": {n: {"exp_avg": ea[n].detach().clone(), "exp_avg_sq": es[n].detach().clone()} for n in ea},
                "step": float(self.step_t.item()), "lr": float(self.lr.item()), "betas": tuple(self.betas),
                "eps": self.eps, "weight_decay": self.weight_decay, "ema_decay": self.ema_decay,
                "ema": None if self.ema is None else {n: v.detach().clone() for n, v in self._named_slices(self.ema).items()},
                **self._group_state()}

    def _group_state(self):
        if not self._grouped:
            return {"param_groups": None, "max_grad_norm": None, "skipped_steps": 0}
        tab = self.group_table.detach().cpu().double().tolist()
        return {"param_groups": {nm: tuple(tab[r]) for nm, r in self._group_row_of.items()},
                "max_grad_norm": None if self.max_norm is None else float(self.max_norm.item()),
                "skipped_steps": 0 if self.stats is None else int(self.stats[3].item())}

    def _load_group_state(self, sd):
        if not self._grouped:
            if sd.get("param_groups") is not None or sd.get("max_grad_norm") is not None:
                raise ValueError("FlatAdamW.load_state_dict: the state was saved by an optimizer with param_groups / "
                                 "max_grad_norm, this one was built without them -- pass them to the constructor")
            return
        if sd.get("max_grad_norm") is not None and self.max_norm is None:
            raise ValueError("FlatAdamW.load_state_dict: the state carries max_grad_norm, this optimizer was built without it")
        if sd.get("param_groups") is not None:
            self._set_groups(groups_from_named(sd["param_groups"]))
        if self.max_norm is not None and sd.get("max_grad_norm") is not None:
            self.max_norm.fill_(float(sd["max_grad_norm"]))
        if self.stats is not None and "skipped_steps" in sd:
            self.stats[3].fill_(float(sd["skipped_steps"]))

    def load_state_dict(self, sd):
        ea, es = self._named_slices(self.exp_avg), self._named_slices(self.exp_avg_sq)
        missing = set(ea) - set(sd["state"])
        if missing:
            raise KeyError(f"FlatAdamW.load_state_dict: no state for {sorted(missing)[:4]} ...")
        with torch.no_grad():
            for n in ea:
                ea[n].copy_(sd["state"][n]["exp_avg"])
                es[n].copy_(sd["state"][n]["exp_avg_sq"])
            self.step_t.fill_(float(sd["step"]))
            self.lr.fill_(float(sd["lr"]))
            if self.ema is not None and sd.get("ema") is not None:
                for n, v in self._named_slices(self.ema).items():
                    v.copy_(sd["ema"][n])
        self.betas, self.eps, self.weight_decay = tuple(sd["betas"]), sd["eps"], sd["weight_decay"]
        self._load_group_state(sd)

    def ema_state_dict(self, prefix=""):
        if self.ema is None:
            raise RuntimeError("FlatAdamW was built without ema_decay")
        return {prefix + n: v.detach().clone() for n, v in self._named_slices(self.ema).items()}

    def step(self, grad_scale=1.0):
        f = self.flat
        f.finish_backward()
        if self._grouped:
            return self._step_groups(grad_scale)
        rc = L.lib().fv_adamw_flat(
            L.ptr(f.param_flat), L.ptr(f.grad_flat), L.ptr(self.exp_avg), L.ptr(self.exp_avg_sq), L.ptr(self.ema),
            L.ptr(f.shadow_flat), L.ptr(self.decay_mask), L.ptr(self.lr), L.ptr(self.step_t),
            ctypes.c_float(self.betas[0]), ctypes.c_float(self.betas[1]), ctypes.c_float(self.eps),
            ctypes.c_float(self.weight_decay), ctypes.c_float(self.ema_decay), ctypes.c_float(grad_scale),
            ctypes.c_size_t(f.param_flat.numel()), L.stream_of(f.param_flat))
        L.check(rc, "adamw_flat")
        f.refresh_transposed()

    def _step_groups(self, grad_scale):
        f = self.flat
        n = f.param_flat.numel()
        st = L.stream_of(f.param_flat)
        if self.partials is not None:
            rc = L.lib().fv_grad_sumsq_partials(L.ptr(f.grad_flat), L.ptr(self.partials), ctypes.c_size_t(n), st)
            L.check(rc, "grad_sumsq_partials")
        rc = L.lib().fv_adamw_flat_groups(
            L.ptr(f.param_flat), L.ptr(f.grad_flat), L.ptr(self.exp_avg), L.ptr(self.exp_avg_sq), L.ptr(self.ema),
            L.ptr(f.shadow_flat), L.ptr(self.group_ids), L.ptr(self._group_table_full), L.i32(MAX_PARAM_GROUPS),
            L.ptr(self.lr), L.ptr(self.step_t), L.ptr(self.partials),
            L.i32(0 if self.partials is None else self.partials.numel()), L.ptr(self.max_norm), L.ptr(self.stats),
            L.i32(self.skip_nonfinite), ctypes.c_float(self.betas[0]), ctypes.c_float(self.betas[1]),
            ctypes.c_float(self.eps), ctypes.c_float(self.ema_decay), ctypes.c_float(grad_scale), ctypes.c_size_t(n), st)
        L.check(rc, "adamw_flat_groups")
        f.refresh_transposed()


def save_checkpoint(path, model, opt, prefix="backbone.", **extra):
    ck = {"state_dict": {prefix + k: v.detach().clone() for k, v in model.state_dict().items()},
          "optimizer_states": [opt.state_dict()], **extra}
    if opt.ema is not None:
        ck["state_dict_ema"] = opt.ema_state_dict("")
    torch.save(ck, path)
    return ck


def load_checkpoint(path_or_dict, model, opt=None, prefix="backbone.", use_ema=False):
    ck = torch.load(path_or_dict, map_location="cpu", weights_only=False) if isinstance(path_or_dict, (str, os.PathLike)) else path_or_dict
    sd = ck["state_dict_ema"] if (use_ema and "state_dict_ema" in ck) else ck["state_dict"]
    model.load_state_dict({(k[len(prefix):] if prefix and k.startswith(prefix) else k): v for k, v in sd.items()}, strict=True)
    if opt is not None:
        opt.load_state_dict(ck["optimizer_states"][0])
    return ck
```

### fastvim_amd/mamba_simple_faster.py

```python
import ctypes
import math

import torch
import torch.nn as nn
import torch.nn.functional as F

from . import _lib as L
from . import mixer_ops as M
from .gemm import gemm_any_bnn, gemm_any_btn, gemm_any_nn, gemm_any_nt, gemm_any_tn, gemm_nn, gemm_nt, gemm_tn


def _shadow(w, cdt):
    sh = getattr(w, "_fv_shadow", None)
    if sh is not None and sh.dtype == cdt:
        if w._version != w._fv_shadow_version:
            with torch.no_grad():
                sh.copy_(w)
            w._fv_shadow_version = w._version
        return sh
    return w.to(cdt)


def _shadow_t(w, cdt):
    wt = getattr(w, "_fv_shadow_t", None)
    if wt is not None and wt.dtype == cdt:
        if w._version != w._fv_shadow_t_version:
            with torch.no_grad():
                wt.copy_(_shadow(w, cdt).t())
            w._fv_shadow_t_version = w._version
        return wt
    return _shadow(w, cdt).t().contiguous()


class _PackedWeights:
    enabled = True


def use_packed_weights(on):
    was = _PackedWeights.enabled
    _PackedWeights.enabled = bool(on)
    return was


def _shadow_pk(w, cdt, plain):
    pk = getattr(w, "_fv_shadow_pk", None)
    if pk is None or pk.dtype != cdt or not _PackedWeights.enabled:
        return None
    if w._version != w._fv_shadow_pk_version:
        if not (plain.is_contiguous() and plain.numel() == pk.numel()):
            return None
        with torch.no_grad():
            M.pack_weight_frags([plain], [pk])
        w._fv_shadow_pk_version = w._version
    return pk


def _wx2_shadow_t(fv):
    if fv is None:
        return None
    wt = fv.get("Wx2_shadow_t")
    if wt is None:
        return None
    params = fv["Wx2_t_params"]
    if any(w._version != w._fv_shadow_t_version for w in params):
        with torch.no_grad():
            for k, w in enumerate(params):
                wt[k].copy_(_shadow(w, wt.dtype).t())
                w._fv_shadow_t_version = w._version
    return wt


def _direct_grad(w):
    g = w.grad
    if getattr(w, "_fv_direct", False) and g is not None and g.is_contiguous() and g.dtype == torch.float32:
        return g
    return None


def _wgrad(X, Y, W=None, splits=16):
    M_, I = X.shape
    J = Y.shape[1]
    while splits > 1 and (M_ % splits or M_ // splits < 256):
        splits //= 2
    part = gemm_any_tn(X, Y, splits)
    g = _direct_grad(W) if W is not None else None
    if g is not None:
        M.reduce_partials(part, splits, out=g.view(-1), accumulate=True)
        return None
    return M.reduce_partials(part, splits)


def _mfma_ok(*ts):
    return all(t.dtype == torch.bfloat16 and t.stride(-1) == 1 and t.data_ptr() % 16 == 0 for t in ts)


def _any_ok(*ts):
    return all(t.is_cuda and t.dtype in (torch.float32, torch.bfloat16) and t.dim() == 2 for t in ts)


def linear_fwd(a2, w_c, bias=None):
    if _mfma_ok(a2, w_c) and a2.shape[1] % 8 == 0 and w_c.shape[0] % 8 == 0:
        return gemm_nt(a2, w_c, bias=None if bias is None else bias.float())
    if _any_ok(a2, w_c):
        return gemm_any_nt(a2, w_c, bias)
    return F.linear(a2, w_c, None if bias is None else bias.to(a2.dtype))


def linear_dgrad(g2, w_c):
    if _mfma_ok(g2, w_c) and w_c.shape[1] % 8 == 0 and g2.shape[1] % 8 == 0:
        return gemm_nn(g2, w_c)
    if _any_ok(g2, w_c):
        return gemm_any_nn(g2, w_c)
    return g2 @ w_c


class _SideStream:
    enabled = False
    stream = None
    pending = []

    @classmethod
    def run(cls, fn, *keep):
        if not cls.enabled:
            return fn()
        cur = torch.cuda.current_stream()
        if cls.stream is None:
            cls.stream = torch.cuda.Stream()
        cls.stream.wait_stream(cur)
        with torch.cuda.stream(cls.stream):
            out = fn()
        cls.pending.append(keep)
        return out

    @classmethod
    def join(cls):
        if cls.stream is not None and cls.pending:
            torch.cuda.current_stream().wait_stream(cls.stream)
        cls.pending = []


XPROJ_IN_SCAN = True


class _GroupedWgrad:
    enabled = False
    jobs = []
    chunk = 0

    @classmethod
    def add(cls, g2, a2, out):
        from .gemm import grouped_splits
        if any(j[2].data_ptr() == out.data_ptr() for j in cls.jobs):
            cls.flush()
        cls.jobs.append((g2, a2, out, grouped_splits(g2.shape[0], M=g2.shape[1], N=a2.shape[1])))
        if cls.chunk and len(cls.jobs) >= cls.chunk:
            cls.flush()

    sums = []
    rows_jobs = []

    @classmethod
    def flush(cls):
        if cls.rows_jobs:
            rj, cls.rows_jobs = cls.rows_jobs, []
            M.chunk_rows_bf16(rj)
        if cls.jobs:
            from .gemm import gemm_tn_grouped
            jobs, cls.jobs = cls.jobs, []
            if _SideStream.enabled:
                cls.sums += _SideStream.run(lambda: gemm_tn_grouped(jobs, reduce=False), jobs)
            else:
                gemm_tn_grouped(jobs)

    @classmethod
    def reduce(cls):
        sums, cls.sums = cls.sums, []
        for part, sp, out in sums:
            M.reduce_partials(part, sp, out=out, accumulate=True)


def group_wgrads(on):
    flush_wgrads()
    _GroupedWgrad.enabled = bool(on)


def flush_wgrads():
    _GroupedWgrad.flush()
    _SideStream.join()
    _GroupedWgrad.reduce()


def linear_wgrad(g2, a2, W=None, splits=None):
    if _mfma_ok(g2, a2) and g2.shape[1] % 8 == 0 and a2.shape[1] % 8 == 0 and g2.shape[0] % 64 == 0:
        gdir = _direct_grad(W) if W is not None else None
        if gdir is not None and _GroupedWgrad.enabled and splits is None and g2.is_contiguous() and a2.is_contiguous():
            _GroupedWgrad.add(g2, a2, gdir.view(-1))
            return None
        if gdir is not None:
            gemm_tn(g2, a2, splits=splits, out=gdir.view(-1), accumulate=True, defer=not _SideStream.enabled)
            return None
        return gemm_tn(g2, a2, splits=splits)
    return _wgrad(g2, a2, W)


class LinearFn(torch.autograd.Function):

    @staticmethod
    def forward(ctx, a, W, cdt, bias=None):
        with torch.autocast("cuda", enabled=False):
            a2 = a.reshape(-1, a.shape[-1]).to(cdt).contiguous()
            W2 = W.reshape(W.shape[0], -1)
            y = linear_fwd(a2, _shadow(W, cdt).reshape(W2.shape), bias)
        ctx.save_for_backward(a2, W)
        ctx.a_shape, ctx.a_dtype, ctx.cdt = a.shape, a.dtype, cdt
        ctx.need_da = a.requires_grad
        ctx.has_bias = bias is not None
        ctx.bias_ref = bias
        return y.view(*a.shape[:-1], W.shape[0])

    @staticmethod
    def backward(ctx, g):
        a2, W = ctx.saved_tensors
        cdt = ctx.cdt
        with torch.autocast("cuda", enabled=False):
            g2 = g.reshape(-1, g.shape[-1]).to(cdt).contiguous()
            W2s = _shadow(W, cdt).reshape(W.shape[0], -1)
            da = linear_dgrad(g2, W2s).view(ctx.a_shape).to(ctx.a_dtype) if ctx.need_da else None
            dW = linear_wgrad(g2, a2, W)
            if dW is not None:
                dW = dW.view(W.shape)
            db = None
            if ctx.has_bias:
                bias = ctx.bias_ref
                gd = _direct_grad(bias) if bias is not None else None
                if g2.is_cuda and g2.dtype in (torch.float32, torch.bfloat16):
                    from .glue_ops import column_sum
                    if gd is not None:
                        column_sum(g2, out=gd.view(-1), accumulate=True)
                    else:
                        db = column_sum(g2)
                else:
                    db = g2.float().sum(0)
        return da, dW, None, db


def linear_module(mod, x):
    if isinstance(mod, nn.Linear) and x.is_cuda:
        return LinearFn.apply(x, mod.weight, _compute_dtype(x), mod.bias)
    return mod(x)


class OutProjAddNormFn(torch.autograd.Function):

    @staticmethod
    def forward(ctx, g, W_out, residual, norm_w, eps, row_scale, cdt):
        L.require_gpu(g, W_out, residual, norm_w)
        B, Ltok, d_in = g.shape
        d = W_out.shape[0]
        Mrows = B * Ltok
        with torch.autocast("cuda", enabled=False):
            y, res_out, rstd, w32, row_scale, rows_per_scale = _out_proj_add_norm_fwd(g, W_out, residual, norm_w, eps, row_scale, cdt)
        ctx.save_for_backward(g, W_out, res_out, w32, rstd, row_scale)
        ctx.rows_per_scale = rows_per_scale
        ctx.cdt = cdt
        ctx.shape = (B, Ltok, d)
        ctx.w_param = norm_w
        return y.view(B, Ltok, d), res_out.view(B, Ltok, d)

    @staticmethod
    def backward(ctx, dy, dres_out):
        g, W_out, r, w32, rstd, row_scale = ctx.saved_tensors
        B, Ltok, d = ctx.shape
        Mrows, d_in = B * Ltok, g.shape[2]
        cdt, dev = ctx.cdt, g.device
        with torch.autocast("cuda", enabled=False):
            dy = dy.reshape(Mrows, d).contiguous()
            dres_out = dres_out.reshape(Mrows, d).contiguous() if dres_out is not None else None
            dx = torch.empty(Mrows, d, device=dev, dtype=cdt)
            dres_in = torch.empty(Mrows, d, device=dev, dtype=torch.float32)
            lib = L.lib()
            nb = lib.fv_add_norm_blocks(L.i32(Mrows))
            pw = torch.empty(nb, d, device=dev, dtype=torch.float32)
            rc = lib.fv_add_norm_bwd(
                L.ptr(dy), L.i32(L.dtype_code(dy.dtype)), L.ptr(dres_out),
                L.i32(L.dtype_code(dres_out.dtype) if dres_out is not None else 0), L.ptr(r), L.i32(L.FV_F32),
                L.ptr(w32), L.ptr(None), L.ptr(rstd), L.ptr(row_scale), L.i32(ctx.rows_per_scale), L.ptr(dx),
                L.i32(L.dtype_code(cdt)), L.ptr(dres_in), L.i32(L.FV_F32), L.ptr(pw), L.ptr(None), L.i32(Mrows), L.i32(d),
                L.i32(1), L.stream_of(r))
            L.check(rc, "add_norm_bwd")
            gd = _direct_grad(ctx.w_param)
            if gd is not None:
                M.reduce_partials(pw, nb, out=gd.view(-1), accumulate=True)
                dw = None
            else:
                dw = M.reduce_partials(pw, nb).to(ctx.w_param.dtype)
            g2 = g.view(Mrows, d_in)
            dg = linear_dgrad(dx, _shadow(W_out, cdt)).view(B, Ltok, d_in)
            dW_out = _SideStream.run(lambda: linear_wgrad(dx, g2, W_out), dx, g)
        return dg, dW_out, dres_in.view(B, Ltok, d), dw, None, None, None


class _Ctx:

    def save_for_backward(self, *tensors):
        self.saved_tensors = tensors


COMBINE_IN_OUT_PROJ = True
CONV_IN_DGRAD = True
XPROJ_TWO_ADDENDS = True


def resolve_combine(pack):
    if pack is not None:
        M.combine_fwd(pack["xz"], pack["skip"], pack["yc"], pack["ln_w"], pack["ln_b"], pack["eps"], pack["rows"],
                      pack["cols"], pack["transposed"], out=pack["out"])


def _out_proj_add_norm_fwd(g, W_out, residual, norm_w, eps, row_scale, cdt, W_in=None, pack=None):
    B, Ltok, d_in = g.shape
    d = W_out.shape[0]
    Mrows = B * Ltok
    g2 = g.view(Mrows, d_in)
    res2 = residual.reshape(Mrows, d).contiguous()
    w32 = norm_w.float().contiguous()
    y = torch.empty(Mrows, d, device=g.device, dtype=cdt)
    res_out = torch.empty(Mrows, d, device=g.device, dtype=torch.float32)
    rstd = torch.empty(Mrows, device=g.device, dtype=torch.float32)
    rows_per_scale = 1
    if row_scale is not None:
        row_scale = row_scale.float().contiguous()
        rows_per_scale = Mrows // row_scale.numel()
    xz = None
    if W_in is not None and W_in.shape[0] % 128 == 0:
        xz = torch.empty(Mrows, W_in.shape[0], device=g.device, dtype=cdt)
    W_out_c = _shadow(W_out, cdt)
    W_in_c = _shadow(W_in, cdt) if xz is not None else None
    lib = L.lib()
    if pack is not None:
        if xz is None and W_out_c.stride(1) == 1 and W_out_c.stride(0) % 8 == 0 and W_out_c.data_ptr() % 16 == 0:
            y, res_out, rstd = M.combine_out_proj_addnorm(pack["xz"], pack["skip"], pack["yc"], pack["ln_w"], pack["ln_b"],
                                                          pack["eps"], pack["rows"], pack["cols"], pack["transposed"],
                                                          pack["out"], W_out_c, res2, w32, row_scale, rows_per_scale, eps,
                                                          W_out_pk=_shadow_pk(W_out, cdt, W_out_c))
            return y, res_out, rstd, w32, row_scale, rows_per_scale
        resolve_combine(pack)
    rc = lib.fv_gemm_bf16_addnorm2(
        L.ptr(g2), L.ptr(W_out_c), L.ptr(res2), L.ptr(w32), L.ptr(row_scale), L.i32(rows_per_scale),
        L.ptr(y), L.ptr(res_out), L.ptr(rstd), L.i32(Mrows), L.i32(d), L.i32(d_in), ctypes.c_long(g2.stride(0)),
        ctypes.c_long(d_in), ctypes.c_float(eps), L.ptr(W_in_c), L.ptr(xz),
        L.i32(W_in.shape[0] if xz is not None else 0), ctypes.c_long(d), L.stream_of(g2))
    L.check(rc, "gemm_bf16_addnorm")
    if W_in is not None:
        return y, res_out, rstd, w32, row_scale, rows_per_scale, xz
    return y, res_out, rstd, w32, row_scale, rows_per_scale


class ChainedBlockFn(torch.autograd.Function):

    in_proj_in_launch = False
    pending_in = None
    pending_out = None
    defer = False

    @staticmethod
    def forward(ctx, g_prev, W_out_prev, residual, norm_w, eps, row_scale, *mixer_args):
        L.require_gpu(g_prev, W_out_prev, residual, norm_w)
        B, Ltok, _ = g_prev.shape
        d = W_out_prev.shape[0]
        cdt = mixer_args[26]
        W_in, b_in = mixer_args[0], mixer_args[1]
        pack, ChainedBlockFn.pending_in = ChainedBlockFn.pending_in, None
        assert pack is None or pack["out"][0].data_ptr() == g_prev.data_ptr()
        with torch.autocast("cuda", enabled=False):
            if pack is not None:
                y, res_out, rstd, w32, rs, rps = _out_proj_add_norm_fwd(g_prev, W_out_prev, residual, norm_w, eps, row_scale,
                                                                      cdt, pack=pack)
                xz = None
            elif ChainedBlockFn.in_proj_in_launch and b_in is None:
                y, res_out, rstd, w32, rs, rps, xz = _out_proj_add_norm_fwd(g_prev, W_out_prev, residual, norm_w, eps,
                                                                          row_scale, cdt, W_in=W_in)
            else:
                y, res_out, rstd, w32, rs, rps = _out_proj_add_norm_fwd(g_prev, W_out_prev, residual, norm_w, eps, row_scale, cdt)
                xz = None
        fctx = _Ctx()
        fctx.precomputed_xz = xz
        fctx.defer_combine = ChainedBlockFn.defer
        g = FastVimMixerFn.forward(fctx, y.view(B, Ltok, d), *mixer_args)
        mixer_saved = fctx.__dict__.pop("saved_tensors")
        fctx.__dict__.pop("precomputed_xz", None)
        fctx.__dict__.pop("defer_combine", None)
        ChainedBlockFn.pending_out = fctx.__dict__.pop("pending_combine", None)
        ctx.save_for_backward(g_prev, W_out_prev, res_out, w32, rstd, rs, *mixer_saved)
        ctx.mixer_attrs = fctx.__dict__
        ctx.rows_per_scale = rps
        ctx.cdt = cdt
        ctx.shape = (B, Ltok, d)
        ctx.w_param = norm_w
        ctx.W_in = mixer_args[0]
        ctx.n_mixer_args = len(mixer_args)
        return g, res_out.view(B, Ltok, d)

    @staticmethod
    def backward(ctx, dg, dres_out):
        g_prev, W_out_prev, r, w32, rstd, row_scale = ctx.saved_tensors[:6]
        B, Ltok, d = ctx.shape
        Mrows, cdt, dev = B * Ltok, ctx.cdt, r.device
        fctx = _Ctx()
        fctx.__dict__.update(ctx.mixer_attrs)
        fctx.saved_tensors = ctx.saved_tensors[6:]
        out = {}

        def fused_in_dgrad(dxz2):
            lib = L.lib()
            nb = lib.fv_gemm_bf16_dgrad_addnorm_blocks(L.i32(Mrows))
            dx = torch.empty(Mrows, d, device=dev, dtype=cdt)
            dres_in = torch.empty(Mrows, d, device=dev, dtype=torch.float32)
            pw = torch.empty(nb, d, device=dev, dtype=torch.float32)
            gg = dres_out.reshape(Mrows, d).contiguous() if dres_out is not None else None
            d_prev = g_prev.shape[2]
            W2 = _shadow(W_out_prev, cdt) if d_prev % 128 == 0 else None
            W_in_c = _shadow(ctx.W_in, cdt)
            dg_prev = torch.empty(Mrows, d_prev, device=dev, dtype=cdt) if W2 is not None else None
            rc = lib.fv_gemm_bf16_dgrad_addnorm_bwd2(
                L.ptr(dxz2), L.ptr(W_in_c), L.ptr(gg), L.ptr(r), L.ptr(rstd), L.ptr(w32), L.ptr(row_scale),
                L.i32(ctx.rows_per_scale), L.ptr(dx), L.ptr(dres_in), L.ptr(pw), L.i32(Mrows), L.i32(d),
                L.i32(dxz2.shape[1]), ctypes.c_long(dxz2.stride(0)), ctypes.c_long(d), L.ptr(W2), L.ptr(dg_prev),
                L.i32(d_prev if W2 is not None else 0), ctypes.c_long(d_prev), L.stream_of(dxz2))
            L.check(rc, "gemm_bf16_dgrad_addnorm_bwd")
            out.update(dx=dx, dres_in=dres_in, pw=pw, nb=nb, dg_prev=dg_prev)

        def fused_conv_dgrad(xz, d_o, dxc, dxc2, cw2, cb, cwb2, cb_b, D, D_b, dxz, rows, cols, transposed, scaling, conv_grad_out):
            gg = dres_out.reshape(Mrows, d).contiguous() if dres_out is not None else None
            d_prev = g_prev.shape[2]
            W2 = _shadow(W_out_prev, cdt) if d_prev % 128 == 0 else None
            W_in_t = _shadow_t(ctx.W_in, cdt)
            p2, dx, dres_in, pw, nb, dg_prev = M.conv_pool_bwd_dgrad(
                xz, d_o, dxc, dxc2, cw2, cb, cwb2, cb_b, D, D_b, dxz, rows, cols, transposed, scaling, W_in_t, gg, r, rstd,
                w32, row_scale, ctx.rows_per_scale, W2=W2, conv_grad_out=conv_grad_out, W_in_pk=_shadow_pk(ctx.W_in, cdt, W_in_t))
            out.update(dx=dx, dres_in=dres_in, pw=pw, nb=nb, dg_prev=dg_prev)
            return p2

        fctx.fused_in_dgrad = fused_in_dgrad
        if (CONV_IN_DGRAD and cdt == torch.bfloat16 and d == 192 and ctx.W_in.shape[0] == 768 and (row_scale is None or row_scale.dtype == torch.float32)):
            fctx.fused_conv_dgrad = fused_conv_dgrad
        grads = FastVimMixerFn.backward(fctx, dg)
        with torch.autocast("cuda", enabled=False):
            gd = _direct_grad(ctx.w_param)
            if gd is not None:
                M.reduce_partials(out["pw"], out["nb"], out=gd.view(-1), accumulate=True)
                dw = None
            else:
                dw = M.reduce_partials(out["pw"], out["nb"]).to(ctx.w_param.dtype)
            dx = out["dx"]
            d_in = g_prev.shape[2]
            g2 = g_prev.view(Mrows, d_in)
            dg_prev = out["dg_prev"] if out["dg_prev"] is not None else linear_dgrad(dx, _shadow(W_out_prev, cdt))
            dg_prev = dg_prev.view(B, Ltok, d_in)
            dW_out = _SideStream.run(lambda: linear_wgrad(dx, g2, W_out_prev), dx, g_prev)
        return (dg_prev, dW_out, out["dres_in"].view(B, Ltok, d), dw, None, None) + tuple(grads[1:1 + ctx.n_mixer_args])


def out_proj_add_norm_ok(g, W_out, residual, norm_w, cdt):
    return (g.is_cuda and cdt == torch.bfloat16 and g.dtype == torch.bfloat16 and g.is_contiguous()
            and W_out.shape[0] == 192 and W_out.shape[1] % 64 == 0 and residual is not None
            and residual.dtype == torch.float32 and norm_w.dtype == torch.float32)


def _compute_dtype(t):
    if torch.is_autocast_enabled():
        dt = torch.get_autocast_dtype('cuda')
        return torch.float32 if dt == torch.float16 else dt
    return torch.float32 if t.dtype == torch.float16 else t.dtype


def half_io(t):
    if torch.is_autocast_enabled():
        return torch.get_autocast_dtype('cuda') == torch.float16
    return t.dtype == torch.float16


def mixer_apply(fn, hidden, *args):
    if any(torch.is_tensor(a) and a.dtype == torch.float16 for a in args):
        args = tuple(a.float() if torch.is_tensor(a) and a.dtype == torch.float16 else a for a in args)
    out = fn.apply(hidden, *args)
    return out.to(torch.float16) if hidden.dtype == torch.float16 else out


class FastVimMixerFn(torch.autograd.Function):

    @staticmethod
    def forward(ctx, hidden, W_in, b_in, cw, cb, cw_b, cb_b, Wx, Wx_b, Wdt, bdt, Wdt_b, bdt_b, A_log, A_b_log,
                D, D_b, ln_w, ln_b, W_out, b_out, rows, cols, transposed, pool_max, scaling, ln_eps, cdt, fv, tpp=1,
                valid=None):
        L.require_gpu(hidden)
        B, Ltok, d = hidden.shape
        if Ltok != rows * cols * tpp:
            raise RuntimeError(f"Mamba: sequence length {Ltok} != token grid {rows}x{cols}x{tpp}")
        d_in = W_in.shape[0] // 2
        with torch.autocast("cuda", enabled=False):
            h_c = hidden.to(cdt).contiguous()
            W_in_c = _shadow(W_in, cdt)
            W_out_c = _shadow(W_out, cdt) if W_out is not None else None
            xz = getattr(ctx, "precomputed_xz", None)
            if xz is None:
                xz = linear_fwd(h_c.view(B * Ltok, d), W_in_c, b_in)
            xz = xz.view(B, Ltok, 2 * d_in)
            cw2, cwb2 = cw.reshape(d_in, -1), cw_b.reshape(d_in, -1)
            amax = None
            if fv is not None and "Wx2" in fv:
                Wx2 = fv["Wx2"]
                if fv["Wx2_shadow"].dtype == cdt:
                    _shadow(Wx, cdt), _shadow(Wx_b, cdt)
                    Wx2_c = fv["Wx2_shadow"]
                else:
                    Wx2_c = Wx2.to(cdt)
            else:
                Wx2 = torch.stack([Wx, Wx_b])
                Wx2_c = Wx2.to(cdt)
            if pool_max:
                xc, skip, amax = M.conv_pool_fwd(xz, cw2, cb, cwb2, cb_b, rows, cols, transposed, pool_max, scaling, tpp,
                                                 D=D, D_b=D_b)
            else:
                xc, skip = M.conv_pool_fwd(xz, cw2, cb, cwb2, cb_b, rows, cols, transposed, pool_max, scaling, tpp,
                                           D=D, D_b=D_b)
            if valid is not None and valid < rows * tpp:
                xc[:, :, valid:].zero_()
            fused = M.xproj_scan_fwd(xc, Wx2_c, Wdt, bdt, A_log, Wdt_b, bdt_b, A_b_log)
            if fused is not None:
                x_dbl, yc = fused
            else:
                x_dbl = M.xproj_fwd(xc, Wx2_c)
                nig = getattr(ctx, "needs_input_grad", None)
                yc, ctx.scan_ckpt = M.scan_fwd(xc, x_dbl, Wdt, bdt, A_log, Wdt_b, bdt_b, A_b_log,
                                               want_ckpt=nig is None or any(nig))
            if (getattr(ctx, "defer_combine", False) and W_out is None and not pool_max and valid is None
                    and M.combine_out_proj_addnorm_ok(xz, rows, cols, tpp, d)):
                g, mean, rstd = M.combine_buffers(xz, ln_w)
                ctx.pending_combine = dict(xz=xz, skip=skip, yc=yc, ln_w=ln_w, ln_b=ln_b, eps=ln_eps, rows=rows, cols=cols,
                                           transposed=transposed, out=(g, mean, rstd))
            else:
                g, mean, rstd = M.combine_fwd(xz, skip, yc, ln_w, ln_b, ln_eps, rows, cols, transposed, tpp=tpp)
            out = g if W_out is None else linear_fwd(g.view(B * Ltok, d_in), W_out_c, b_out).view(B, Ltok, d)
        ctx.save_for_backward(h_c, W_in, cw, cb, cw_b, cb_b, Wx2, Wdt, bdt, Wdt_b, bdt_b, A_log, A_b_log, D, D_b,
                              ln_w, ln_b, W_out, xz, xc, x_dbl, g, skip, yc, mean, rstd, amax)
        ctx.geo = (rows, cols, transposed, pool_max, scaling, tpp)
        ctx.has_bias = (b_in is not None, b_out is not None)
        ctx.cdt = cdt
        ctx.in_dtype = hidden.dtype
        ctx.fv = fv
        return out

    @staticmethod
    def backward(ctx, dout):
        (h_c, W_in, cw, cb, cw_b, cb_b, Wx2, Wdt, bdt, Wdt_b, bdt_b, A_log, A_b_log, D, D_b, ln_w, ln_b, W_out,
         xz, xc, x_dbl, g, skip, yc, mean, rstd, amax) = ctx.saved_tensors
        rows, cols, transposed, pool_max, scaling, tpp = ctx.geo
        cdt = ctx.cdt
        B, Ltok, d = h_c.shape
        d_in = W_in.shape[0] // 2
        fv = ctx.fv or {}
        with torch.autocast("cuda", enabled=False):
            dout = dout.to(cdt).contiguous()
            if W_out is None:
                dg, dW_out, db_out = dout.view(B * Ltok, d_in), None, None
            else:
                do2 = dout.view(B * Ltok, d)
                dg = linear_dgrad(do2, _shadow(W_out, cdt))
                dW_out = _SideStream.run(lambda: linear_wgrad(do2, g.view(B * Ltok, d_in), W_out), do2, g)
                db_out = do2.float().sum(0) if ctx.has_bias[1] else None
            cw2, cwb2 = cw.reshape(d_in, -1), cw_b.reshape(d_in, -1)
            dxz = torch.empty_like(xz)
            d_o, dyc, p1 = M.combine_bwd(dg, xz, skip, yc, ln_w, ln_b, mean, rstd, dxz, rows, cols, transposed,
                                         grad_out=fv.get("ln_grad") if ln_w is not None else None, tpp=tpp)
            W_ = x_dbl.shape[-1]
            fused_xproj = W_ in M.XPROJ_WIDTHS
            Mrows = B * rows * tpp
            grouped_x = (fused_xproj and _GroupedWgrad.enabled and "Wx2_grad" in fv and xc.dtype == torch.bfloat16
                         and Mrows % 64 == 0 and d_in % 8 == 0)
            dxc2 = None
            if (grouped_x and XPROJ_IN_SCAN and amax is None and getattr(ctx, "scan_ckpt", None) is None
                    and M.scan_bwd_xproj_ok(xc, Wdt, pool_max, rows, cols, tpp)):
                wsh = fv.get("Wx2_shadow")
                dxc, dxc2, dx_dbl, ps = M.scan_bwd_xproj(xc, x_dbl, Wdt, bdt, A_log, Wdt_b, bdt_b, A_b_log, dyc,
                                                         Wx2[0], Wx2[1], grad_out=fv.get("scan_grad"),
                                                         Wx2_bf16=wsh if wsh is not None and wsh.dtype == torch.bfloat16 else None)
                dxb = torch.empty(2, Mrows, (W_ + 7) // 8 * 8, device=xc.device, dtype=torch.bfloat16)
                _GroupedWgrad.rows_jobs.append((dx_dbl, dxb))
                xc2 = xc.view(2, Mrows, d_in)
                for k_ in range(2):
                    _GroupedWgrad.add(dxb[k_][:, :W_], xc2[k_], fv["Wx2_grad"][k_].reshape(-1))
                dWx2 = (None, None)
            else:
                dxc, dx_dbl, ps = M.scan_bwd(xc, x_dbl, Wdt, bdt, A_log, Wdt_b, bdt_b, A_b_log, dyc,
                                             grad_out=fv.get("scan_grad"), keep_chunks=fused_xproj,
                                             ckpt=getattr(ctx, "scan_ckpt", None))
            if dxc2 is not None:
                pass
            elif grouped_x:
                wt = _wx2_shadow_t(fv)
                if (wt is not None and amax is None and XPROJ_TWO_ADDENDS and M.xproj_bwd3_ok(Mrows, d_in, W_, xc.dtype)
                        and M.conv_pool_bwd2_ok(rows, cols, tpp, d_in, pool_max)):
                    dxc2 = torch.empty(dxc.shape, device=dxc.device, dtype=xc.dtype)
                dxb = M.xproj_bwd(dx_dbl, xc, Wx2[0], Wx2[1], dxc, dw=False, Wx2_t=wt, dxc2=dxc2)
                xc2 = xc.view(2, Mrows, d_in)
                for k_ in range(2):
                    _GroupedWgrad.add(dxb[k_][:, :W_], xc2[k_], fv["Wx2_grad"][k_].reshape(-1))
                dWx2 = (None, None)
            elif fused_xproj:
                dWx2 = M.xproj_bwd(dx_dbl, xc, Wx2[0], Wx2[1], dxc, grad_out=fv.get("Wx2_grad"))
                if dWx2 is None:
                    dWx2 = (None, None)
            else:
                xc2 = xc.view(2, B * rows * tpp, d_in)
                dWx2 = gemm_any_btn(dx_dbl, xc2)
                if "Wx2_grad" in fv:
                    fv["Wx2_grad"].add_(dWx2)
                    dWx2 = (None, None)
                dxc = dxc.view(2, B * rows * tpp, d_in) + gemm_any_bnn(dx_dbl, Wx2.float(), out_dtype=torch.float32)
            conv_grad = fv.get("conv_grad") if cb is not None and cb_b is not None else None
            fused_cd = getattr(ctx, "fused_conv_dgrad", None)
            dxz2 = dxz.view(B * Ltok, 2 * d_in)
            if (fused_cd is not None and amax is None and dxc.dtype == torch.float32 and dxc.is_contiguous()
                    and M.conv_pool_bwd_dgrad_ok(xz, rows, cols, tpp, d, pool_max)):
                p2 = fused_cd(xz, d_o, dxc, dxc2, cw2, cb, cwb2, cb_b, D, D_b, dxz, rows, cols, transposed, scaling, conv_grad)
                fused_dgrad = "done"
            else:
                p2 = M.conv_pool_bwd(xz, d_o, dxc, cw2, cb, cwb2, cb_b, D, D_b, dxz, rows, cols, transposed,
                                     pool_max, scaling, grad_out=conv_grad, tpp=tpp, amax=amax, dxc2=dxc2)
                fused_dgrad = getattr(ctx, "fused_in_dgrad", None)
            if fused_dgrad == "done":
                dhidden = None
            elif fused_dgrad is not None:
                fused_dgrad(dxz2)
                dhidden = None
            else:
                dhidden = linear_dgrad(dxz2, _shadow(W_in, cdt)).view(B, Ltok, d).to(ctx.in_dtype)
            dW_in = _SideStream.run(lambda: linear_wgrad(dxz2, h_c.view(B * Ltok, d), W_in), dxz2, h_c)
            db_in = dxz2.float().sum(0) if ctx.has_bias[0] else None
        has_ln = ln_w is not None
        n4 = 4 * d_in
        N_, R_ = A_log.shape[1], Wdt.shape[1]
        if p2 is None:
            g_cw = g_cb = g_cwb = g_cbb = g_D = g_Db = None
        else:
            g_cw, g_cwb = p2[0:n4].view(cw.shape), p2[n4:2 * n4].view(cw_b.shape)
            g_cb = p2[2 * n4:2 * n4 + d_in] if cb is not None else None
            g_cbb = p2[2 * n4 + d_in:2 * n4 + 2 * d_in] if cb_b is not None else None
            g_D, g_Db = p2[2 * n4 + 2 * d_in:2 * n4 + 3 * d_in], p2[2 * n4 + 3 * d_in:2 * n4 + 4 * d_in]
        if ps is None:
            g_A = g_Wdt = g_bdt = (None, None)
        else:
            g_A = [ps[k, :d_in * N_].view(d_in, N_) for k in range(2)]
            g_Wdt = [ps[k, d_in * N_:d_in * (N_ + R_)].view(d_in, R_) for k in range(2)]
            g_bdt = [ps[k, d_in * (N_ + R_):] for k in range(2)]
        g_lw = p1[0] if (has_ln and p1 is not None) else None
        g_lb = p1[1] if (has_ln and p1 is not None) else None
        return (dhidden, dW_in, db_in, g_cw, g_cb, g_cwb, g_cbb,
                dWx2[0], dWx2[1], g_Wdt[0], g_bdt[0], g_Wdt[1], g_bdt[1], g_A[0], g_A[1],
                g_D, g_Db, g_lw, g_lb, dW_out, db_out, None, None, None, None, None, None, None, None, None, None)


class Mamba(nn.Module):
    def __init__(self, d_model, d_state=16, d_conv=4, expand=2, dt_rank="auto", dt_min=0.001, dt_max=0.1,
                 dt_init="random", dt_scale=1.0, dt_init_floor=1e-4, conv_bias=True, bias=False,
                 use_fast_path=False, layer_idx=None, device=None, dtype=None, init_layer_scale=None,
                 scanpath_type="rowwise", token_size=None, use_norm_after_ssm=True,
                 use_our_selective_scan=False, collapse_method="mean", scaling_factor=1):
        factory_kwargs = {"device": device, "dtype": dtype}
        super().__init__()
        self.d_model = d_model
        self.d_state = d_state
        self.d_conv = d_conv
        self.expand = expand
        self.d_inner = int(self.expand * self.d_model)
        self.dt_rank = math.ceil(self.d_model / 16) if dt_rank == "auto" else dt_rank
        self.use_fast_path = use_fast_path
        self.layer_idx = layer_idx
        self.use_our_selective_scan = use_our_selective_scan
        self.num_of_rows, self.num_of_col = token_size[0], token_size[1]
        self.scanpath_type = scanpath_type
        self.scaling_factor = scaling_factor
        if collapse_method not in ("mean", "max"):
            raise NotImplementedError(collapse_method)
        self.collapse_method = collapse_method
        self.init_layer_scale = init_layer_scale
        if init_layer_scale is not None:
            self.gamma = nn.Parameter(init_layer_scale * torch.ones(d_model), requires_grad=True)

        self.in_proj = nn.Linear(self.d_model, self.d_inner * 2, bias=bias, **factory_kwargs)
        self.use_norm_after_ssm = use_norm_after_ssm
        if use_norm_after_ssm:
            self.layernorm = nn.LayerNorm(self.d_inner, **factory_kwargs)

        def conv():
            return nn.Conv1d(self.d_inner, self.d_inner, bias=conv_bias, kernel_size=d_conv, groups=self.d_inner,
                             padding=d_conv - 1, **factory_kwargs)

        self.conv1d = conv()
        self.activation = "silu"
        self.act = nn.SiLU()
        self.x_proj = nn.Linear(self.d_inner, self.dt_rank + self.d_state * 2, bias=False, **factory_kwargs)
        self.dt_proj = nn.Linear(self.dt_rank, self.d_inner, bias=True, **factory_kwargs)

        dt_init_std = self.dt_rank ** -0.5 * dt_scale
        if dt_init == "constant":
            nn.init.constant_(self.dt_proj.weight, dt_init_std)
        elif dt_init == "random":
            nn.init.uniform_(self.dt_proj.weight, -dt_init_std, dt_init_std)
        else:
            raise NotImplementedError
        dt = torch.exp(torch.rand(self.d_inner, **factory_kwargs) * (math.log(dt_max) - math.log(dt_min))
                       + math.log(dt_min)).clamp(min=dt_init_floor)
        inv_dt = dt + torch.log(-torch.expm1(-dt))
        with torch.no_grad():
            self.dt_proj.bias.copy_(inv_dt)
        self.dt_proj.bias._no_reinit = True

        def s4d_real():
            A = torch.arange(1, self.d_state + 1, dtype=torch.float32, device=device).repeat(self.d_inner, 1)
            p = nn.Parameter(torch.log(A).contiguous())
            p._no_weight_decay = True
            return p

        self.A_log = s4d_real()
        self.D = nn.Parameter(torch.ones(self.d_inner, device=device))
        self.D._no_weight_decay = True
        self.A_b_log = s4d_real()
        self.conv1d_b = conv()
        self.x_proj_b = nn.Linear(self.d_inner, self.dt_rank + self.d_state * 2, bias=False, **factory_kwargs)
        self.dt_proj_b = nn.Linear(self.dt_rank, self.d_inner, bias=True, **factory_kwargs)
        self.D_b = nn.Parameter(torch.ones(self.d_inner, device=device))
        self.D_b._no_weight_decay = True
        self.out_proj = nn.Linear(self.d_inner, self.d_model, bias=bias, **factory_kwargs)
        self.pre_x_shape = (-1, self.d_inner, self.num_of_rows, self.num_of_col)

    def mixer_fn_args(self, cdt, transposed_grid=False, defer_out_proj=False):
        ln_w = self.layernorm.weight if self.use_norm_after_ssm else None
        ln_b = self.layernorm.bias if self.use_norm_after_ssm else None
        ln_eps = self.layernorm.eps if self.use_norm_after_ssm else 0.0
        return (self.in_proj.weight, self.in_proj.bias,
                self.conv1d.weight, self.conv1d.bias, self.conv1d_b.weight, self.conv1d_b.bias,
                self.x_proj.weight, self.x_proj_b.weight,
                self.dt_proj.weight, self.dt_proj.bias, self.dt_proj_b.weight, self.dt_proj_b.bias,
                self.A_log, self.A_b_log, self.D, self.D_b, ln_w, ln_b,
                None if defer_out_proj else self.out_proj.weight, None if defer_out_proj else self.out_proj.bias,
                self.num_of_rows, self.num_of_col, bool(transposed_grid), self.collapse_method == "max",
                float(self.scaling_factor), float(ln_eps), cdt, self.__dict__.get("_fv"))

    def forward(self, hidden_states, inference_params=None, transposed_grid=False, defer_out_proj=False):
        if inference_params is not None:
            raise NotImplementedError("FastVim mixers have no inference cache (reference: no step())")
        if self.d_conv != 4 or self.d_state != 16:
            raise RuntimeError("fastvim_amd kernels are built for d_conv=4, d_state=16 (the FastVim configs)")
        cdt = _compute_dtype(hidden_states)
        ln_w = self.layernorm.weight if self.use_norm_after_ssm else None
        ln_b = self.layernorm.bias if self.use_norm_after_ssm else None
        ln_eps = self.layernorm.eps if self.use_norm_after_ssm else 0.0
        out = mixer_apply(
            FastVimMixerFn, hidden_states, self.in_proj.weight, self.in_proj.bias,
            self.conv1d.weight, self.conv1d.bias, self.conv1d_b.weight, self.conv1d_b.bias,
            self.x_proj.weight, self.x_proj_b.weight,
            self.dt_proj.weight, self.dt_proj.bias, self.dt_proj_b.weight, self.dt_proj_b.bias,
            self.A_log, self.A_b_log, self.D, self.D_b, ln_w, ln_b,
            None if defer_out_proj else self.out_proj.weight, None if defer_out_proj else self.out_proj.bias,
            self.num_of_rows, self.num_of_col, bool(transposed_grid), self.collapse_method == "max",
            float(self.scaling_factor), float(ln_eps), cdt, self.__dict__.get("_fv"))
        if defer_out_proj:
            if self.init_layer_scale is not None or self.out_proj.bias is not None:
                raise RuntimeError("defer_out_proj: layer scale / out_proj bias are applied after out_proj")
            return out
        if self.init_layer_scale is not None:
            out = out * self.gamma
        return out
```

### fastvim_amd/mixer_ops.py

```python
import ctypes

import torch

from . import _lib as L

f32 = ctypes.c_float


def _geo(rows, cols, transposed):
    return (1, rows) if transposed else (cols, 1)


def conv_pool_fwd(xz, conv_w, conv_b, conv_w_b, conv_b_b, rows, cols, transposed, pool_max, scaling, tpp=1,
                  D=None, D_b=None):
    B, Ltok, two_d = xz.shape
    d_in = two_d // 2
    s_i, s_j = _geo(rows, cols, transposed)
    xc = torch.empty(2, B, rows * tpp, d_in, device=xz.device, dtype=xz.dtype)
    skip = torch.empty(B, Ltok, d_in, device=xz.device, dtype=xz.dtype) if D is not None else None
    amax = torch.empty_like(xc) if pool_max else None
    rc = L.lib().fv_mixer_conv_pool_fwd(
        L.ptr(xz), L.ptr(conv_w), L.ptr(conv_b), L.ptr(conv_w_b), L.ptr(conv_b_b), L.ptr(D), L.ptr(D_b), L.ptr(xc),
        L.ptr(skip), L.ptr(amax), L.i32(B), L.i32(rows), L.i32(cols), L.i32(s_i), L.i32(s_j), L.i32(tpp), L.i32(d_in),
        L.i32(conv_w.shape[-1]), L.i32(pool_max), f32(scaling), L.i32(L.dtype_code(xz.dtype)), L.stream_of(xz))
    L.check(rc, "mixer_conv_pool_fwd")
    if pool_max:
        return (xc, amax) if D is None else (xc, skip, amax)
    return xc if D is None else (xc, skip)


def scan_fwd(xc, x_dbl, dt_w, dt_b, A_log, dt_w_b, dt_b_b, A_log_b, want_ckpt=False):
    _, B, Lc, d_in = xc.shape
    R = dt_w.shape[1]
    N = A_log.shape[1]
    lib = L.lib()
    yc = torch.empty(2, B, Lc, d_in, device=xc.device, dtype=torch.float32)
    ckpt = None
    if want_ckpt:
        nck = lib.fv_mixer_scan_ckpt_floats(L.i32(B), L.i32(Lc), L.i32(d_in), L.i32(N), L.i32(R))
        ckpt = torch.empty(nck, device=xc.device, dtype=torch.float32) if nck else None
    nws = lib.fv_mixer_scan_fwd_seg_floats(L.i32(B), L.i32(Lc), L.i32(d_in), L.i32(N), L.i32(R))
    ws = torch.empty(nws, device=xc.device, dtype=torch.float32) if nws else None
    rc = lib.fv_mixer_scan_fwd_seg(
        L.ptr(xc), L.ptr(x_dbl), L.ptr(dt_w), L.ptr(dt_b), L.ptr(A_log), L.ptr(dt_w_b), L.ptr(dt_b_b),
        L.ptr(A_log_b), L.ptr(yc), L.ptr(ckpt), L.ptr(ws), L.i32(B), L.i32(Lc), L.i32(d_in), L.i32(R), L.i32(N),
        L.i32(L.dtype_code(xc.dtype)), L.stream_of(xc))
    L.check(rc, "mixer_scan_fwd")
    return (yc, ckpt) if want_ckpt else yc


def xproj_scan_fwd(xc, Wx2_c, dt_w, dt_b, A_log, dt_w_b, dt_b_b, A_log_b):
    _, B, Lc, d_in = xc.shape
    R, N = dt_w.shape[1], A_log.shape[1]
    W = Wx2_c.shape[1]
    lib = L.lib()
    if (xc.dtype != torch.bfloat16 or Wx2_c.dtype != torch.bfloat16 or N != 16 or W != R + 2 * N
            or not xc.is_contiguous() or not Wx2_c.is_contiguous() or xc.data_ptr() % 16 or Wx2_c.data_ptr() % 16
            or not lib.fv_mixer_xproj_scan_fwd_ok(L.i32(Lc), L.i32(d_in), L.i32(R), L.i32(L.dtype_code(xc.dtype)))):
        return None
    x_dbl = torch.empty(2, B * Lc, W, device=xc.device, dtype=xc.dtype)
    yc = torch.empty(2, B, Lc, d_in, device=xc.device, dtype=torch.float32)
    rc = lib.fv_mixer_xproj_scan_fwd(
        L.ptr(xc), L.ptr(Wx2_c), L.ptr(dt_w), L.ptr(dt_b), L.ptr(A_log), L.ptr(dt_w_b), L.ptr(dt_b_b), L.ptr(A_log_b),
        L.ptr(x_dbl), L.ptr(yc), L.i32(B), L.i32(Lc), L.i32(d_in), L.i32(R), L.i32(N), L.i32(L.dtype_code(xc.dtype)),
        L.stream_of(xc))
    L.check(rc, "mixer_xproj_scan_fwd")
    return x_dbl, yc


def combine_buffers(xz, ln_w):
    B, Ltok, two_d = xz.shape
    g = torch.empty(B, Ltok, two_d // 2, device=xz.device, dtype=xz.dtype)
    if ln_w is not None:
        return g, torch.empty(B * Ltok, device=xz.device, dtype=torch.float32), torch.empty(B * Ltok, device=xz.device, dtype=torch.float32)
    return g, None, None


def combine_fwd(xz, skip, yc, ln_w, ln_b, eps, rows, cols, transposed, tpp=1, out=None):
    B, Ltok, two_d = xz.shape
    d_in = two_d // 2
    s_i, s_j = _geo(rows, cols, transposed)
    g, mean, rstd = out if out is not None else combine_buffers(xz, ln_w)
    rc = L.lib().fv_mixer_combine_fwd(
        L.ptr(xz), L.ptr(skip), L.ptr(yc), L.ptr(ln_w), L.ptr(ln_b), f32(eps), L.ptr(g), L.ptr(mean), L.ptr(rstd),
        L.i32(B), L.i32(rows), L.i32(cols), L.i32(s_i), L.i32(s_j), L.i32(tpp), L.i32(d_in),
        L.i32(L.dtype_code(xz.dtype)), L.stream_of(xz))
    L.check(rc, "mixer_combine_fwd")
    return g, mean, rstd


class _Deferred:
    enabled = False
    max_jobs = 144
    side = False
    jobs = []
    stream = None
    pending = []

    @classmethod
    def add(cls, part, out, n_partials):
        lo, hi = out.data_ptr(), out.data_ptr() + out.numel() * 4
        if any(j[1].data_ptr() < hi and lo < j[1].data_ptr() + j[1].numel() * 4 for j in cls.jobs):
            cls.flush()
        cls.jobs.append((part, out, n_partials))
        if len(cls.jobs) >= cls.max_jobs:
            cls.flush()

    @classmethod
    def _launch(cls, jobs):
        k = len(jobs)
        ins = (ctypes.c_void_p * k)(*[j[0].data_ptr() for j in jobs])
        outs = (ctypes.c_void_p * k)(*[j[1].data_ptr() for j in jobs])
        Ss = (ctypes.c_int * k)(*[j[2] for j in jobs])
        ns = (ctypes.c_size_t * k)(*[j[0].numel() // j[2] for j in jobs])
        rc = L.lib().fv_reduce_partials_multi(ins, outs, Ss, ns, L.i32(k), L.i32(1), L.stream_of(jobs[0][0]))
        L.check(rc, "reduce_partials_multi")

    @classmethod
    def flush(cls):
        if not cls.jobs:
            return
        jobs, cls.jobs = cls.jobs, []
        if not cls.side:
            cls._launch(jobs)
            return
        cur = torch.cuda.current_stream()
        if cls.stream is None:
            cls.stream = torch.cuda.Stream()
        cls.stream.wait_stream(cur)
        with torch.cuda.stream(cls.stream):
            cls._launch(jobs)
        cls.pending.append(jobs)

    @classmethod
    def join(cls):
        if cls.pending:
            torch.cuda.current_stream().wait_stream(cls.stream)
            cls.pending = []


def defer_reductions(on):
    flush_reductions()
    _Deferred.enabled = bool(on)


def pending_reductions():
    return len(_Deferred.jobs)


def drop_reductions():
    n = len(_Deferred.jobs)
    _Deferred.jobs = []
    return n


def flush_reductions():
    _Deferred.flush()
    _Deferred.join()


def reduce_partials(part, n_partials, out=None, accumulate=False, defer=True):
    if out is not None and accumulate and defer and _Deferred.enabled:
        assert out.numel() == part.numel() // n_partials and out.is_contiguous() and out.dtype == torch.float32
        _Deferred.add(part, out, n_partials)
        return out
    if out is None:
        out = torch.empty(part.shape[1:], device=part.device, dtype=torch.float32)
    n = part.numel() // n_partials
    assert out.numel() == n and out.is_contiguous() and out.dtype == torch.float32
    rc = L.lib().fv_reduce_partials(L.ptr(part), L.ptr(out), L.i32(n_partials), ctypes.c_size_t(n),
                                    L.i32(accumulate), L.stream_of(part))
    L.check(rc, "reduce_partials")
    return out


def combine_out_proj_addnorm_ok(xz, rows, cols, tpp, d_model):
    B, Ltok, two_d = xz.shape
    return bool(xz.dtype == torch.bfloat16 and xz.is_contiguous() and
                L.lib().fv_mixer_combine_out_proj_addnorm_ok(L.i32(B), L.i32(rows), L.i32(cols), L.i32(tpp), L.i32(two_d // 2),
                                                             L.i32(d_model), L.i32(L.FV_BF16)))


def combine_out_proj_addnorm(xz, skip, yc, ln_w, ln_b, ln_eps, rows, cols, transposed, out, W_out_c, residual2, norm_w32,
                             row_scale, rows_per_scale, eps, W_out_pk=None):
    B, Ltok, two_d = xz.shape
    d = W_out_c.shape[0]
    Mrows = B * Ltok
    s_i, s_j = _geo(rows, cols, transposed)
    g, mean, rstd_ln = out
    y = torch.empty(Mrows, d, device=xz.device, dtype=torch.bfloat16)
    res_out = torch.empty(Mrows, d, device=xz.device, dtype=torch.float32)
    rstd = torch.empty(Mrows, device=xz.device, dtype=torch.float32)
    if W_out_pk is not None:
        assert W_out_pk.dtype == torch.bfloat16 and W_out_pk.is_contiguous() and W_out_pk.numel() == d * (two_d // 2)
        fn, W_arg, ldw = L.lib().fv_mixer_combine_out_proj_addnorm_pk, W_out_pk, two_d // 2
    else:
        fn, W_arg, ldw = L.lib().fv_mixer_combine_out_proj_addnorm, W_out_c, W_out_c.stride(0)
    rc = fn(
        L.ptr(xz), L.ptr(skip), L.ptr(yc), L.ptr(ln_w), L.ptr(ln_b), f32(ln_eps), L.ptr(g), L.ptr(mean), L.ptr(rstd_ln),
        L.i32(B), L.i32(rows), L.i32(cols), L.i32(s_i), L.i32(s_j), L.ptr(W_arg), ctypes.c_long(ldw),
        L.ptr(residual2), L.ptr(norm_w32), L.ptr(row_scale), L.i32(rows_per_scale), L.ptr(y), L.ptr(res_out), L.ptr(rstd),
        f32(eps), L.stream_of(xz))
    L.check(rc, "mixer_combine_out_proj_addnorm")
    return y, res_out, rstd


def combine_bwd(dg, xz, skip, yc, ln_w, ln_b, mean, rstd, dxz, rows, cols, transposed, grad_out=None, tpp=1):
    B, Ltok, two_d = xz.shape
    d_in = two_d // 2
    s_i, s_j = _geo(rows, cols, transposed)
    lib = L.lib()
    nb = lib.fv_mixer_bwd_blocks(L.i32(B), L.i32(rows), L.i32(d_in), L.i32(tpp), L.i32(0))
    d_o = torch.empty(B, Ltok, d_in, device=xz.device, dtype=xz.dtype)
    dyc = torch.empty(B, rows * tpp, d_in, device=xz.device, dtype=torch.float32)
    part = torch.empty(nb, 2, d_in, device=xz.device, dtype=torch.float32)
    rc = lib.fv_mixer_combine_bwd(
        L.ptr(dg), L.ptr(xz), L.ptr(skip), L.ptr(yc), L.ptr(ln_w), L.ptr(ln_b), L.ptr(mean), L.ptr(rstd), L.ptr(dxz), L.ptr(d_o),
        L.ptr(dyc), L.ptr(part), L.i32(B), L.i32(rows), L.i32(cols), L.i32(s_i), L.i32(s_j), L.i32(tpp), L.i32(d_in),
        L.i32(L.dtype_code(xz.dtype)), L.stream_of(xz))
    L.check(rc, "mixer_combine_bwd")
    if grad_out is not None:
        reduce_partials(part, nb, out=grad_out, accumulate=True)
        return d_o, dyc, None
    return d_o, dyc, reduce_partials(part, nb)


def scan_bwd(xc, x_dbl, dt_w, dt_b, A_log, dt_w_b, dt_b_b, A_log_b, dyc, grad_out=None, keep_chunks=False,
             dyc_per_direction=False, ckpt=None):
    _, B, Lc, d_in = xc.shape
    assert dyc.numel() == (2 if dyc_per_direction else 1) * B * Lc * d_in and dyc.dtype == torch.float32
    R, N = dt_w.shape[1], A_log.shape[1]
    W = R + 2 * N
    dev = xc.device
    lib = L.lib()
    f32o = dict(device=dev, dtype=torch.float32)
    given = ckpt is not None
    nws = lib.fv_mixer_scan_bwd_seg_floats(L.i32(B), L.i32(Lc), L.i32(d_in), L.i32(N), L.i32(R)) if given else 0
    nchunks = lib.fv_mixer_scan_bwd_seg_chunks(L.i32(B), L.i32(d_in), L.i32(Lc), L.i32(R), L.i32(int(nws > 0)))
    dxc = torch.empty(2, B, Lc, d_in, **f32o)
    dx_dbl = torch.empty(nchunks, 2, B * Lc, W, **f32o)
    if not given:
        nck = lib.fv_mixer_scan_bwd_ckpt_floats(L.i32(B), L.i32(Lc), L.i32(d_in), L.i32(N), L.i32(R))
        ckpt = torch.empty(nck, **f32o) if nck else None
    ws = torch.empty(nws, **f32o) if nws else None
    nprt = lib.fv_mixer_scan_bwd_seg_partials(L.i32(B), L.i32(Lc), L.i32(d_in), L.i32(R)) if nws else \
        lib.fv_mixer_scan_bwd_partials(L.i32(B), L.i32(Lc), L.i32(R))
    part = torch.empty(nprt, 2 * d_in * (N + R + 1), **f32o)
    rc = lib.fv_mixer_scan_bwd_seg(
        L.ptr(xc), L.ptr(x_dbl), L.ptr(dt_w), L.ptr(dt_b), L.ptr(A_log), L.ptr(dt_w_b), L.ptr(dt_b_b),
        L.ptr(A_log_b), L.ptr(dyc), L.i32(int(dyc_per_direction)), L.ptr(dxc), L.ptr(dx_dbl), L.ptr(ckpt), L.i32(int(given)),
        L.ptr(part), L.ptr(ws), L.i32(B), L.i32(Lc), L.i32(d_in), L.i32(R), L.i32(N), L.i32(L.dtype_code(xc.dtype)),
        L.stream_of(xc))
    L.check(rc, "mixer_scan_bwd")
    if not keep_chunks:
        dx_dbl = dx_dbl[0] if nchunks == 1 else reduce_partials(dx_dbl, nchunks)
    if grad_out is not None:
        reduce_partials(part, nprt, out=grad_out, accumulate=True)
        return dxc, dx_dbl, None
    return dxc, dx_dbl, reduce_partials(part, nprt).view(2, d_in * (N + R + 1))


def scan_bwd_xproj_ok(xc, dt_w, pool_max, rows, cols, tpp):
    _, B, Lc, d_in = xc.shape
    lib = L.lib()
    return bool(xc.dtype in (torch.float32, torch.bfloat16)
                and lib.fv_mixer_scan_bwd_xproj_ok(L.i32(B), L.i32(Lc), L.i32(d_in), L.i32(dt_w.shape[1]), L.i32(L.dtype_code(xc.dtype)))
                and lib.fv_mixer_conv_pool_bwd2_ok(L.i32(rows), L.i32(cols), L.i32(tpp), L.i32(d_in), L.i32(int(bool(pool_max)))))


def scan_bwd_xproj(xc, x_dbl, dt_w, dt_b, A_log, dt_w_b, dt_b_b, A_log_b, dyc, Wx, Wx_b, grad_out=None, Wx2_bf16=None):
    _, B, Lc, d_in = xc.shape
    R, N = dt_w.shape[1], A_log.shape[1]
    W = R + 2 * N
    lib = L.lib()
    f32o = dict(device=xc.device, dtype=torch.float32)
    dxc = torch.empty(2, B, Lc, d_in, **f32o)
    dxc2 = torch.empty(2, B, Lc, d_in, device=xc.device, dtype=xc.dtype)
    dx_dbl = torch.empty(2, 2, B * Lc, W, **f32o)
    nprt = lib.fv_mixer_scan_bwd_partials(L.i32(B), L.i32(Lc), L.i32(R))
    part = torch.empty(nprt, 2 * d_in * (N + R + 1), **f32o)
    if xc.dtype == torch.bfloat16 and Wx2_bf16 is None:
        Wx2_bf16 = torch.stack([Wx, Wx_b]).to(torch.bfloat16)
    assert Wx2_bf16 is None or (Wx2_bf16.dtype == torch.bfloat16 and Wx2_bf16.is_contiguous() and Wx2_bf16.shape == (2, W, d_in))
    rc = lib.fv_mixer_scan_bwd_xproj(
        L.ptr(xc), L.ptr(x_dbl), L.ptr(dt_w), L.ptr(dt_b), L.ptr(A_log), L.ptr(dt_w_b), L.ptr(dt_b_b), L.ptr(A_log_b),
        L.ptr(dyc), L.ptr(Wx), L.ptr(Wx_b), L.ptr(Wx2_bf16), L.ptr(dxc), L.ptr(dxc2), L.ptr(dx_dbl), L.ptr(part), L.i32(B), L.i32(Lc),
        L.i32(d_in), L.i32(R), L.i32(N), L.i32(L.dtype_code(xc.dtype)), L.stream_of(xc))
    L.check(rc, "mixer_scan_bwd_xproj")
    if grad_out is not None:
        reduce_partials(part, nprt, out=grad_out, accumulate=True)
        return dxc, dxc2, dx_dbl, None
    return dxc, dxc2, dx_dbl, reduce_partials(part, nprt).view(2, d_in * (N + R + 1))


def chunk_rows_bf16(jobs):
    lib = L.lib()
    buckets = {}
    for j in jobs:
        assert j[1].dtype == torch.bfloat16 and j[1].is_contiguous() and j[0].dtype == torch.float32 and j[0].is_contiguous()
        buckets.setdefault((tuple(j[0].shape), tuple(j[1].shape)), []).append(j)
    for (ishape, _), bjobs in buckets.items():
        nchunks, _, Mrows, W = ishape
        for lo in range(0, len(bjobs), 64):
            grp = bjobs[lo:lo + 64]
            k = len(grp)
            ins = (ctypes.c_void_p * k)(*[j[0].data_ptr() for j in grp])
            outs = (ctypes.c_void_p * k)(*[j[1].data_ptr() for j in grp])
            rc = lib.fv_chunk_rows_bf16(ins, outs, L.i32(k), L.i32(nchunks), ctypes.c_long(2 * Mrows), L.i32(W), L.stream_of(grp[0][0]))
            L.check(rc, "chunk_rows_bf16")


def conv_pool_bwd(xz, d_o, dxc, conv_w, conv_b, conv_w_b, conv_b_b, D, D_b, dxz, rows, cols, transposed,
                  pool_max, scaling, grad_out=None, tpp=1, amax=None, dxc2=None):
    B, Ltok, two_d = xz.shape
    d_in = two_d // 2
    s_i, s_j = _geo(rows, cols, transposed)
    lib = L.lib()
    nb = lib.fv_mixer_bwd_blocks(L.i32(B), L.i32(rows), L.i32(d_in), L.i32(tpp), L.i32(1))
    part = torch.empty(nb, 12 * d_in, device=xz.device, dtype=torch.float32)
    assert dxc2 is None or (dxc2.dtype == xz.dtype and dxc2.shape == dxc.shape and dxc2.is_contiguous())
    rc = lib.fv_mixer_conv_pool_bwd2(
        L.ptr(xz), L.ptr(d_o), L.ptr(dxc), L.ptr(dxc2), L.ptr(conv_w), L.ptr(conv_b), L.ptr(conv_w_b), L.ptr(conv_b_b),
        L.ptr(D), L.ptr(D_b), L.ptr(amax), L.ptr(dxz), L.ptr(part), L.i32(B), L.i32(rows), L.i32(cols), L.i32(s_i),
        L.i32(s_j), L.i32(tpp), L.i32(d_in), L.i32(conv_w.shape[-1]), L.i32(pool_max), f32(scaling),
        L.i32(L.dtype_code(xz.dtype)), L.stream_of(xz))
    L.check(rc, "mixer_conv_pool_bwd")
    if grad_out is not None:
        reduce_partials(part, nb, out=grad_out, accumulate=True)
        return None
    return reduce_partials(part, nb)


def conv_pool_bwd_dgrad_ok(xz, rows, cols, tpp, d_model, pool_max):
    B, Ltok, two_d = xz.shape
    return bool(xz.dtype == torch.bfloat16 and xz.is_contiguous() and
                L.lib().fv_mixer_conv_pool_bwd_dgrad_ok(L.i32(B), L.i32(rows), L.i32(cols), L.i32(tpp), L.i32(two_d // 2),
                                                        L.i32(d_model), L.i32(int(bool(pool_max))), L.i32(L.FV_BF16)))


def conv_pool_bwd_dgrad(xz, d_o, dxc, dxc2, conv_w, conv_b, conv_w_b, conv_b_b, D, D_b, dxz, rows, cols, transposed, scaling,
                        W_in_t, dres_out, r, rstd, norm_w32, row_scale, rows_per_scale, W2=None, conv_grad_out=None,
                        W_in_pk=None):
    B, Ltok, two_d = xz.shape
    d_in = two_d // 2
    d = W_in_t.shape[0]
    Mrows = B * Ltok
    s_i, s_j = _geo(rows, cols, transposed)
    lib = L.lib()
    dev = xz.device
    nb = lib.fv_mixer_conv_pool_bwd_dgrad_blocks(L.i32(B), L.i32(rows))
    part = torch.empty(nb, 12 * d_in, device=dev, dtype=torch.float32)
    dx = torch.empty(Mrows, d, device=dev, dtype=torch.bfloat16)
    dres_in = torch.empty(Mrows, d, device=dev, dtype=torch.float32)
    pw = torch.empty(nb, d, device=dev, dtype=torch.float32)
    N2 = W2.shape[1] if W2 is not None else 0
    dg_prev = torch.empty(Mrows, N2, device=dev, dtype=torch.bfloat16) if W2 is not None else None
    assert dxc2 is None or (dxc2.dtype == xz.dtype and dxc2.shape == dxc.shape and dxc2.is_contiguous())
    assert W_in_t.dtype == torch.bfloat16 and W_in_t.stride(1) == 1 and W_in_t.shape[1] == two_d
    if W_in_pk is not None:
        assert W_in_pk.dtype == torch.bfloat16 and W_in_pk.is_contiguous() and W_in_pk.numel() == d * two_d
        fn, W_arg, ldwt = lib.fv_mixer_conv_pool_bwd_dgrad_pk, W_in_pk, two_d
    else:
        fn, W_arg, ldwt = lib.fv_mixer_conv_pool_bwd_dgrad, W_in_t, W_in_t.stride(0)
    rc = fn(
        L.ptr(xz), L.ptr(d_o), L.ptr(dxc), L.ptr(dxc2), L.ptr(conv_w), L.ptr(conv_b), L.ptr(conv_w_b), L.ptr(conv_b_b),
        L.ptr(D), L.ptr(D_b), L.ptr(dxz), L.ptr(part), L.i32(B), L.i32(rows), L.i32(cols), L.i32(s_i), L.i32(s_j),
        f32(scaling), L.ptr(W_arg), ctypes.c_long(ldwt), L.ptr(dres_out), L.ptr(r), L.ptr(rstd), L.ptr(norm_w32),
        L.ptr(row_scale), L.i32(rows_per_scale), L.ptr(dx), L.ptr(dres_in), L.ptr(pw), L.ptr(W2), L.ptr(dg_prev), L.i32(N2),
        ctypes.c_long(W2.stride(0) if W2 is not None else 0), L.stream_of(xz))
    L.check(rc, "mixer_conv_pool_bwd_dgrad")
    if conv_grad_out is not None:
        reduce_partials(part, nb, out=conv_grad_out, accumulate=True)
        p2 = None
    else:
        p2 = reduce_partials(part, nb)
    return p2, dx, dres_in, pw, nb, dg_prev


def transpose_bf16_batched(srcs, dsts):
    lib = L.lib()
    rows, cols = srcs[0].shape
    for lo in range(0, len(srcs), 64):
        a, b = srcs[lo:lo + 64], dsts[lo:lo + 64]
        assert all(t.dtype == torch.bfloat16 and t.is_contiguous() and tuple(t.shape) == (rows, cols) for t in a)
        assert all(t.dtype == torch.bfloat16 and t.is_contiguous() and tuple(t.shape) == (cols, rows) for t in b)
        k = len(a)
        ins = (ctypes.c_void_p * k)(*[t.data_ptr() for t in a])
        outs = (ctypes.c_void_p * k)(*[t.data_ptr() for t in b])
        L.check(lib.fv_transpose_bf16_batched(ins, outs, L.i32(k), L.i32(rows), L.i32(cols), L.stream_of(a[0])), "transpose_bf16_batched")


PACK_ROWS = 192


def pack_index(K):
    assert K % 32 == 0
    KS = K // 32
    u = torch.arange(PACK_ROWS * K // 8)
    lane, t = u % 64, u // 64
    nb, ks, wv = t % 3, (t // 3) % KS, t // (3 * KS)
    return torch.stack([48 * wv + 16 * nb + (lane % 16), 32 * ks + 8 * (lane // 16)], dim=1)


def pack_weight_frags_ref(W):
    rows, K = W.shape
    assert rows == PACK_ROWS
    idx = pack_index(K).to(W.device)
    cols = idx[:, 1:2] + torch.arange(8, device=W.device)
    return W[idx[:, 0:1], cols].reshape(rows, K)


def pack_weight_frags(srcs, dsts):
    lib = L.lib()
    rows, K = srcs[0].shape
    for lo in range(0, len(srcs), 64):
        a, b = srcs[lo:lo + 64], dsts[lo:lo + 64]
        assert all(t.dtype == torch.bfloat16 and t.is_contiguous() and tuple(t.shape) == (rows, K) for t in a)
        assert all(t.dtype == torch.bfloat16 and t.is_contiguous() and t.numel() == rows * K for t in b)
        assert rows == PACK_ROWS
        k = len(a)
        ins = (ctypes.c_void_p * k)(*[t.data_ptr() for t in a])
        outs = (ctypes.c_void_p * k)(*[t.data_ptr() for t in b])
        L.check(lib.fv_pack_weight_frags_batched(ins, outs, L.i32(k), L.i32(K), L.stream_of(a[0])), "pack_weight_frags_batched")


XPROJ_WIDTHS = (44, 56, 80, 96, 112, 34, 36, 38, 64)


def xproj_fwd(xc, Wx2_c):
    d_in = xc.shape[-1]
    Mrows = xc.numel() // (2 * d_in)
    W = Wx2_c.shape[1]
    if (xc.dtype != torch.bfloat16 or Wx2_c.dtype != torch.bfloat16 or d_in % 32 or W > 112
            or not xc.is_contiguous() or not Wx2_c.is_contiguous() or xc.data_ptr() % 16 or Wx2_c.data_ptr() % 16):
        if xc.is_cuda and xc.dtype in (torch.float32, torch.bfloat16) and Wx2_c.dtype in (torch.float32, torch.bfloat16):
            from .gemm import gemm_any_bnt
            return gemm_any_bnt(xc.reshape(2, Mrows, d_in), Wx2_c)
        return torch.bmm(xc.view(2, Mrows, d_in), Wx2_c.transpose(1, 2))
    out = torch.empty(2, Mrows, W, device=xc.device, dtype=xc.dtype)
    rc = L.lib().fv_mixer_xproj_fwd(L.ptr(xc), L.ptr(Wx2_c), L.ptr(out), L.i32(Mrows), L.i32(d_in), L.i32(W), L.stream_of(xc))
    L.check(rc, "mixer_xproj_fwd")
    return out


_XPROJ_PRESUM = 8


def xproj_bwd3_ok(Mrows, d_in, W, dtype):
    return bool(dtype == torch.bfloat16 and L.lib().fv_mixer_xproj_bwd3_ok(L.i32(Mrows), L.i32(d_in), L.i32(W), L.i32(L.dtype_code(dtype))))


def conv_pool_bwd2_ok(rows, cols, tpp, d_in, pool_max):
    return bool(L.lib().fv_mixer_conv_pool_bwd2_ok(L.i32(rows), L.i32(cols), L.i32(tpp), L.i32(d_in), L.i32(int(pool_max))))


def xproj_bwd(dx_dbl_chunks, xc, Wx, Wx_b, dxc, grad_out=None, dw=True, Wx2_t=None, dxc2=None):
    nchunks, _, Mrows, W = dx_dbl_chunks.shape
    d_in = xc.shape[-1]
    lib = L.lib()
    if nchunks >= _XPROJ_PRESUM:
        dx_dbl_chunks = reduce_partials(dx_dbl_chunks, nchunks, defer=False).view(1, 2, Mrows, W)
        nchunks = 1
    if not dw:
        WP = (W + 7) // 8 * 8
        dxb = torch.empty(2, Mrows, WP, device=xc.device, dtype=torch.bfloat16)
        if Wx2_t is not None:
            assert Wx2_t.dtype == torch.bfloat16 and Wx2_t.is_contiguous() and tuple(Wx2_t.shape) == (2, d_in, W)
            assert dxc2 is None or (dxc2.dtype == torch.bfloat16 and dxc2.is_contiguous() and dxc2.numel() == dxc.numel())
            rc = lib.fv_mixer_xproj_bwd3(L.ptr(dx_dbl_chunks), L.i32(nchunks), L.ptr(xc), L.ptr(Wx), L.ptr(Wx_b), L.ptr(Wx2_t),
                                         L.ptr(dxc), L.ptr(dxc2), L.ptr(dxb), L.i32(Mrows), L.i32(d_in), L.i32(W),
                                         L.i32(L.dtype_code(xc.dtype)), L.stream_of(xc))
        else:
            assert dxc2 is None
            rc = lib.fv_mixer_xproj_bwd2(L.ptr(dx_dbl_chunks), L.i32(nchunks), L.ptr(xc), L.ptr(Wx), L.ptr(Wx_b), L.ptr(dxc),
                                         None, L.ptr(dxb), L.i32(Mrows), L.i32(d_in), L.i32(W),
                                         L.i32(L.dtype_code(xc.dtype)), L.stream_of(xc))
        L.check(rc, "mixer_xproj_bwd")
        return dxb
    ns = lib.fv_mixer_xproj_bwd_slices(L.i32(Mrows))
    part = torch.empty(ns, 2, W, d_in, device=xc.device, dtype=torch.float32)
    rc = lib.fv_mixer_xproj_bwd(L.ptr(dx_dbl_chunks), L.i32(nchunks), L.ptr(xc), L.ptr(Wx), L.ptr(Wx_b), L.ptr(dxc),
                                L.ptr(part), L.i32(Mrows), L.i32(d_in), L.i32(W), L.i32(L.dtype_code(xc.dtype)),
                                L.stream_of(xc))
    L.check(rc, "mixer_xproj_bwd")
    if grad_out is not None:
        reduce_partials(part, ns, out=grad_out.view(-1), accumulate=True)
        return None
    return reduce_partials(part, ns)


def rows_segment_sum(x, idx, rows, scale=1.0, out_dtype=None):
    per_dir = x.dim() == 4
    B, Lk, d = x.shape[-3:]
    assert idx.shape == (2, B, Lk) and idx.dtype == torch.int32 and idx.is_contiguous() and x.is_contiguous()
    out = torch.empty(2, B, rows, d, device=x.device, dtype=out_dtype or x.dtype)
    rc = L.lib().fv_rows_segment_sum(L.ptr(x), L.i32(L.dtype_code(x.dtype)), L.i32(int(per_dir)), L.ptr(idx), L.ptr(out),
                                     L.i32(L.dtype_code(out.dtype)), L.i32(B), L.i32(Lk), L.i32(rows), L.i32(d),
                                     f32(scale), L.stream_of(x))
    L.check(rc, "rows_segment_sum")
    return out


def rows_gather(x, idx, scale=1.0, out_dtype=None):
    _, B, rows, d = x.shape
    Lk = idx.shape[-1]
    assert idx.shape == (2, B, Lk) and idx.dtype == torch.int32 and idx.is_contiguous() and x.is_contiguous()
    out = torch.empty(2, B, Lk, d, device=x.device, dtype=out_dtype or x.dtype)
    rc = L.lib().fv_rows_gather(L.ptr(x), L.i32(L.dtype_code(x.dtype)), L.ptr(idx), L.ptr(out),
                                L.i32(L.dtype_code(out.dtype)), L.i32(B), L.i32(Lk), L.i32(rows), L.i32(d), f32(scale),
                                L.stream_of(x))
    L.check(rc, "rows_gather")
    return out
```

### include/fastvim_hip.h

```cpp
#ifndef FASTVIM_HIP_H
#define FASTVIM_HIP_H

#include <stddef.h>
#include <stdint.h>

#ifdef __cplusplus
extern "C" {
#endif

typedef void* fv_stream_t;

enum { FV_F32 = 0, FV_BF16 = 1, FV_F16 = 2 };
enum { FV_OK = 0, FV_ERR_INVALID = -1, FV_ERR_HIP = -2, FV_ERR_UNSUPPORTED = -3 };

const char* fv_last_error(void);
#define FV_ABI_VERSION 3
int fv_version(void);

int fv_selective_scan_fwd(const void* u, const void* delta, const float* A, const void* B,
                          const void* C, const float* D, const void* z, const float* delta_bias,
                          void* out, float* last_state, int batch, int dim, int seqlen, int dstate,
                          int n_groups, int B_variable, int C_variable, int delta_softplus,
                          int dtype, fv_stream_t stream);

size_t fv_selective_scan_bwd_workspace(int batch, int dim, int seqlen, int dstate, int n_groups,
                                       int B_variable, int C_variable);

int fv_selective_scan_bwd(const void* u, const void* delta, const float* A, const void* B,
                          const void* C, const float* D, const void* z, const float* delta_bias,
                          const void* dout, void* du, void* ddelta, float* dA, float* dB, float* dC,
                          float* dD, void* dz, float* ddelta_bias, void* workspace, int batch, int dim,
                          int seqlen, int dstate, int n_groups, int B_variable, int C_variable,
                          int delta_softplus, int dtype, fv_stream_t stream);

int fv_causal_conv1d_fwd(const void* x, const float* weight, const float* bias, void* y, int batch, int dim,
                         int seqlen, int width, int silu, int dtype, fv_stream_t stream);
int fv_causal_conv1d_bwd(const void* x, const float* weight, const float* bias, const void* dy, void* dx,
                         float* partials, int batch, int dim, int seqlen, int width, int silu, int dtype,
                         fv_stream_t stream);

int fv_scan_expand_skip_fwd(const void* yc, const void* u_full, const float* D, void* out, int batch, int dim,
                            int seqlen, int seqlen_compressed, int dtype, fv_stream_t stream);

int fv_mixer_conv_pool_fwd(const void* xz, const float* conv_w, const float* conv_b,
                           const float* conv_w_b, const float* conv_b_b, const float* D, const float* D_b,
                           void* xc, void* skip, void* amax, int batch, int rows, int cols, int tok_stride_row,
                           int tok_stride_col, int tokens_per_patch, int d_inner, int d_conv, int pool_max,
                           float scaling_factor, int dtype, fv_stream_t stream);

int fv_mixer_scan_fwd(const void* xc, const void* x_dbl, const float* dt_w, const float* dt_bias,
                      const float* A_log, const float* dt_w_b, const float* dt_bias_b,
                      const float* A_log_b, float* yc, int batch, int Lc, int d_inner, int dt_rank,
                      int d_state, int dtype, fv_stream_t stream);
size_t fv_mixer_scan_ckpt_floats(int batch, int Lc, int d_inner, int d_state, int dt_rank);
int fv_mixer_scan_fwd_ckpt(const void* xc, const void* x_dbl, const float* dt_w, const float* dt_bias,
                           const float* A_log, const float* dt_w_b, const float* dt_bias_b,
                           const float* A_log_b, float* yc, float* ckpt, int batch, int Lc, int d_inner, int dt_rank,
                           int d_state, int dtype, fv_stream_t stream);
int fv_mixer_scan_fwd_segments(int batch, int Lc, int d_inner, int dt_rank);
size_t fv_mixer_scan_fwd_seg_floats(int batch, int Lc, int d_inner, int d_state, int dt_rank);
int fv_mixer_scan_fwd_seg(const void* xc, const void* x_dbl, const float* dt_w, const float* dt_bias,
                          const float* A_log, const float* dt_w_b, const float* dt_bias_b, const float* A_log_b,
                          float* yc, float* ckpt, float* seg_ws, int batch, int Lc, int d_inner, int dt_rank,
                          int d_state, int dtype, fv_stream_t stream);

int fv_mixer_xproj_scan_fwd_ok(int Lc, int d_inner, int dt_rank, int dtype);
int fv_mixer_xproj_scan_fwd(const void* xc, const void* x_proj_w2, const float* dt_w, const float* dt_bias,
                            const float* A_log, const float* dt_w_b, const float* dt_bias_b, const float* A_log_b,
                            void* x_dbl, float* yc, int batch, int Lc, int d_inner, int dt_rank, int d_state,
                            int dtype, fv_stream_t stream);

int fv_mixer_combine_fwd(const void* xz, const void* skip, const float* yc, const float* ln_w,
                         const float* ln_b, float ln_eps, void* g, float* mean, float* rstd, int batch,
                         int rows, int cols, int tok_stride_row, int tok_stride_col, int tokens_per_patch,
                         int d_inner, int dtype, fv_stream_t stream);

int fv_mixer_bwd_blocks(int batch, int rows, int d_inner, int tokens_per_patch, int which);

int fv_mixer_plan(int family, int batch, int rows, int cols, int tokens_per_patch, int d_inner, int pool_max, int dtype,
                  int* plan);

int fv_mixer_combine_bwd(const void* dg, const void* xz, const void* skip, const float* yc,
                         const float* ln_w, const float* ln_b, const float* mean, const float* rstd,
                         void* dxz, void* d_o, float* dyc, float* partials, int batch, int rows, int cols, int tok_stride_row,
                         int tok_stride_col, int tokens_per_patch, int d_inner, int dtype, fv_stream_t stream);

int fv_mixer_scan_bwd_chunks(int d_inner, int Lc, int dt_rank);
int fv_mixer_scan_bwd_chunks_b(int batch, int d_inner, int Lc, int dt_rank);
int fv_mixer_scan_bwd_partials(int batch, int Lc, int dt_rank);
size_t fv_mixer_scan_bwd_ckpt_floats(int batch, int Lc, int d_inner, int d_state, int dt_rank);
int fv_mixer_scan_bwd(const void* xc, const void* x_dbl, const float* dt_w, const float* dt_bias,
                      const float* A_log, const float* dt_w_b, const float* dt_bias_b, const float* A_log_b,
                      const float* dyc, float* dxc, float* dx_dbl, float* ckpt, float* partials, int batch,
                      int Lc, int d_inner, int dt_rank, int d_state, int dtype, fv_stream_t stream);
int fv_mixer_scan_bwd_dir(const void* xc, const void* x_dbl, const float* dt_w, const float* dt_bias,
                          const float* A_log, const float* dt_w_b, const float* dt_bias_b, const float* A_log_b,
                          const float* dyc, int dyc_per_direction, float* dxc, float* dx_dbl, float* ckpt,
                          float* partials, int batch, int Lc, int d_inner, int dt_rank, int d_state, int dtype,
                          fv_stream_t stream);
int fv_mixer_scan_bwd_ckpt(const void* xc, const void* x_dbl, const float* dt_w, const float* dt_bias,
                           const float* A_log, const float* dt_w_b, const float* dt_bias_b, const float* A_log_b,
                           const float* dyc, int dyc_per_direction, float* dxc, float* dx_dbl, float* ckpt,
                           int ckpt_given, float* partials, int batch, int Lc, int d_inner, int dt_rank, int d_state,
                           int dtype, fv_stream_t stream);
int fv_mixer_scan_bwd_segments(int batch, int Lc, int d_inner, int dt_rank);
size_t fv_mixer_scan_bwd_seg_floats(int batch, int Lc, int d_inner, int d_state, int dt_rank);
int fv_mixer_scan_bwd_seg_partials(int batch, int Lc, int d_inner, int dt_rank);
int fv_mixer_scan_bwd_seg_chunks(int batch, int d_inner, int Lc, int dt_rank, int seg_ws_given);
int fv_mixer_scan_bwd_seg(const void* xc, const void* x_dbl, const float* dt_w, const float* dt_bias, const float* A_log,
                          const float* dt_w_b, const float* dt_bias_b, const float* A_log_b, const float* dyc,
                          int dyc_per_direction, float* dxc, float* dx_dbl, float* ckpt, int ckpt_given, float* partials,
                          float* seg_ws, int batch, int Lc, int d_inner, int dt_rank, int d_state, int dtype,
                          fv_stream_t stream);

int fv_mixer_scan_bwd_xproj_ok(int batch, int Lc, int d_inner, int dt_rank, int dtype);
int fv_mixer_scan_bwd_xproj(const void* xc, const void* x_dbl, const float* dt_w, const float* dt_bias, const float* A_log,
                            const float* dt_w_b, const float* dt_bias_b, const float* A_log_b, const float* dyc,
                            const float* x_proj_w, const float* x_proj_w_b, const void* x_proj_w2_bf16, float* dxc,
                            void* dxc2, float* dx_dbl, float* partials, int batch, int Lc, int d_inner, int dt_rank,
                            int d_state, int dtype, fv_stream_t stream);
int fv_chunk_rows_bf16(const float* const* partials, void* const* outs, int njobs, int nchunks, long rows, int width,
                       fv_stream_t stream);

int fv_rows_segment_sum(const void* in, int in_dtype, int in_per_direction, const int* idx, void* out, int out_dtype,
                        int batch, int n_tokens, int rows, int d_inner, float scale, fv_stream_t stream);
int fv_rows_gather(const void* in, int in_dtype, const int* idx, void* out, int out_dtype, int batch, int n_tokens,
                   int rows, int d_inner, float scale, fv_stream_t stream);

int fv_mixer_conv_pool_bwd(const void* xz, const void* d_o, const float* dxc, const float* conv_w,
                           const float* conv_b, const float* conv_w_b, const float* conv_b_b, const float* D,
                           const float* D_b, const void* amax, void* dxz, float* partials, int batch, int rows,
                           int cols, int tok_stride_row, int tok_stride_col, int tokens_per_patch, int d_inner,
                           int d_conv, int pool_max, float scaling_factor, int dtype, fv_stream_t stream);

int fv_mixer_conv_pool_bwd2_ok(int rows, int cols, int tokens_per_patch, int d_inner, int pool_max);
int fv_mixer_conv_pool_bwd2(const void* xz, const void* d_o, const float* dxc, const void* dxc2, const float* conv_w,
                            const float* conv_b, const float* conv_w_b, const float* conv_b_b, const float* D,
                            const float* D_b, const void* amax, void* dxz, float* partials, int batch, int rows,
                            int cols, int tok_stride_row, int tok_stride_col, int tokens_per_patch, int d_inner,
                            int d_conv, int pool_max, float scaling_factor, int dtype, fv_stream_t stream);

int fv_reduce_partials(const float* partials, float* out, int n_partials, size_t n, int accumulate,
                       fv_stream_t stream);
int fv_reduce_partials_multi(const float* const* partials, float* const* outs, const int* n_partials,
                             const size_t* ns, int njobs, int accumulate, fv_stream_t stream);

int fv_add_norm_blocks(int M);
int fv_add_norm_fwd(const void* x, int x_dtype, const void* residual, int residual_dtype,
                    const float* weight, const float* bias, const float* row_scale, int rows_per_scale,
                    void* y, int y_dtype, void* residual_out, int residual_out_dtype, float* mean,
                    float* rstd, int M, int N, float eps, int is_rms_norm, fv_stream_t stream);
int fv_add_norm_bwd(const void* dy, int dy_dtype, const void* dresidual_out, int dresidual_out_dtype,
                    const void* r, int r_dtype, const float* weight, const float* mean, const float* rstd,
                    const float* row_scale, int rows_per_scale, void* dx, int dx_dtype, void* dresidual_in,
                    int dresidual_in_dtype, float* partial_dw, float* partial_db, int M, int N,
                    int is_rms_norm, fv_stream_t stream);

int fv_gemm_bf16(const void* A, const void* B, void* C, const float* bias, int M, int N, int K, long lda,
                 long ldb, long ldc, int a_k_slow, int b_k_slow, int c_fp32, int splits, fv_stream_t stream);

int fv_gemm_f32(const void* A, int a_dtype, const void* B, int b_dtype, void* C, int c_dtype, const float* bias, int M,
                int N, int K, long lda, long ldb, long ldc, int a_k_slow, int b_k_slow, int batch, long strideA,
                long strideB, long strideC, fv_stream_t stream);

int fv_gemm_bf16_addnorm(const void* A, const void* W, const float* residual, const float* norm_weight,
                         const float* row_scale, int rows_per_scale, void* y, float* residual_out, float* rstd, int M,
                         int N, int K, long lda, long ldw, float eps, fv_stream_t stream);

int fv_gemm_bf16_dgrad_addnorm_blocks(int M);
int fv_gemm_bf16_dgrad_addnorm_bwd(const void* A, const void* W, const float* dresidual_out, const float* r,
                                   const float* rstd, const float* norm_weight, const float* row_scale,
                                   int rows_per_scale, void* dx, float* dresidual_in, float* partial_dw, int M, int N,
                                   int K, long lda, long ldw, fv_stream_t stream);

int fv_gemm_bf16_dgrad_addnorm_bwd2(const void* A, const void* W, const float* dresidual_out, const float* r,
                                    const float* rstd, const float* norm_weight, const float* row_scale,
                                    int rows_per_scale, void* dx, float* dresidual_in, float* partial_dw, int M, int N,
                                    int K, long lda, long ldw, const void* W2, void* C2, int N2, long ldw2,
                                    fv_stream_t stream);

int fv_mixer_combine_out_proj_addnorm_ok(int batch, int rows, int cols, int tokens_per_patch, int d_inner, int d_model,
                                         int dtype);
int fv_mixer_combine_out_proj_addnorm(const void* xz, const void* skip, const float* yc, const float* ln_w,
                                      const float* ln_b, float ln_eps, void* g, float* mean, float* rstd_ln, int batch,
                                      int rows, int cols, int tok_stride_row, int tok_stride_col, const void* W, long ldw,
                                      const float* residual, const float* norm_weight, const float* row_scale,
                                      int rows_per_scale, void* y, float* residual_out, float* rstd, float eps,
                                      fv_stream_t stream);
int fv_mixer_combine_out_proj_addnorm_pk(const void* xz, const void* skip, const float* yc, const float* ln_w,
                                         const float* ln_b, float ln_eps, void* g, float* mean, float* rstd_ln, int batch,
                                         int rows, int cols, int tok_stride_row, int tok_stride_col, const void* W,
                                         long ldw, const float* residual, const float* norm_weight,
                                         const float* row_scale, int rows_per_scale, void* y, float* residual_out,
                                         float* rstd, float eps, fv_stream_t stream);

int fv_mixer_conv_pool_bwd_dgrad_ok(int batch, int rows, int cols, int tokens_per_patch, int d_inner, int d_model,
                                    int pool_max, int dtype);
int fv_mixer_conv_pool_bwd_dgrad_blocks(int batch, int rows);
int fv_mixer_conv_pool_bwd_dgrad(const void* xz, const void* dskip, const float* dxc, const void* dxc2,
                                 const float* conv_w, const float* conv_b, const float* conv_w_b, const float* conv_b_b,
                                 const float* D, const float* D_b, void* dxz, float* conv_partials, int batch, int rows,
                                 int cols, int tok_stride_row, int tok_stride_col, float scaling, const void* W_in_t,
                                 long ldwt, const float* dresidual_out, const float* r, const float* rstd,
                                 const float* norm_weight, const float* row_scale, int rows_per_scale, void* dx,
                                 float* dresidual_in, float* partial_dw, const void* W2, void* C2, int N2, long ldw2,
                                 fv_stream_t stream);
int fv_mixer_conv_pool_bwd_dgrad_pk(const void* xz, const void* dskip, const float* dxc, const void* dxc2,
                                    const float* conv_w, const float* conv_b, const float* conv_w_b,
                                    const float* conv_b_b, const float* D, const float* D_b, void* dxz,
                                    float* conv_partials, int batch, int rows, int cols, int tok_stride_row,
                                    int tok_stride_col, float scaling, const void* W_in_t, long ldwt,
                                    const float* dresidual_out, const float* r, const float* rstd,
                                    const float* norm_weight, const float* row_scale, int rows_per_scale, void* dx,
                                    float* dresidual_in, float* partial_dw, const void* W2, void* C2, int N2, long ldw2,
                                    fv_stream_t stream);

int fv_transpose_bf16_batched(const void* const* srcs, void* const* dsts, int njobs, int rows, int cols,
                              fv_stream_t stream);

int fv_pack_weight_frags_batched(const void* const* srcs, void* const* dsts, int njobs, int K, fv_stream_t stream);

int fv_gemm_bf16_addnorm2(const void* A, const void* W, const float* residual, const float* norm_weight,
                          const float* row_scale, int rows_per_scale, void* y, float* residual_out, float* rstd, int M,
                          int N, int K, long lda, long ldw, float eps, const void* W2, void* C2, int N2, long ldw2,
                          fv_stream_t stream);

int fv_gemm_bf16_tn_grouped(const void* const* x, const void* const* y, float* const* parts, const int* Kd,
                            const int* M, const int* N, const int* splits, int count, fv_stream_t stream);
int fv_gemm_bf16_tn_grouped_ld(const void* const* x, const void* const* y, float* const* parts, const int* Kd,
                               const int* M, const int* N, const int* ldx, const int* ldy, const int* splits, int count,
                               fv_stream_t stream);

int fv_gemm_bf16_tn_grouped_wide8(int M, int N, int Kd);

int fv_mixer_xproj_fwd(const void* xc, const void* x_proj_w2, void* x_dbl, int M, int d_inner, int width,
                       fv_stream_t stream);

int fv_mixer_xproj_bwd_slices(int M);
int fv_mixer_xproj_bwd(const float* dx_dbl_partials, int nchunks, const void* xc, const float* x_proj_w,
                       const float* x_proj_w_b, float* dxc, float* dW_partials, int M, int d_inner, int width,
                       int dtype, fv_stream_t stream);
int fv_mixer_xproj_bwd2(const float* dx_dbl_partials, int nchunks, const void* xc, const float* x_proj_w,
                        const float* x_proj_w_b, float* dxc, float* dW_partials, void* dx_dbl_bf16, int M, int d_inner,
                        int width, int dtype, fv_stream_t stream);
int fv_mixer_xproj_bwd3_ok(int M, int d_inner, int width, int dtype);
int fv_mixer_xproj_bwd3(const float* dx_dbl_partials, int nchunks, const void* xc, const float* x_proj_w,
                        const float* x_proj_w_b, const void* x_proj_w_t_bf16, float* dxc, void* dxc2_bf16,
                        void* dx_dbl_bf16, int M, int d_inner, int width, int dtype, fv_stream_t stream);

int fv_soft_target_ce(const void* logits, int logits_dtype, const float* target, float* loss_rows, float* loss,
                      float* dlogits, int batch, int classes, fv_stream_t stream);

int fv_patch_unfold(const void* img, int img_dtype, void* out, int out_dtype, int batch, int chans, int height,
                    int width, int ph, int pw, fv_stream_t stream);
int fv_gemm_bf16_rowbias(const void* A, const void* B, float* C, const float* table, int period, int M, int N, int K,
                         long lda, long ldb, long ldc, fv_stream_t stream);
int fv_mean_pool_fwd(const void* x, void* out, int batch, int tokens, int dim, int dtype, fv_stream_t stream);
int fv_mean_pool_bwd(const void* g, void* dx, int batch, int tokens, int dim, int dtype, fv_stream_t stream);
int fv_droppath_table(float* table, const float* keep, const float* inv_keep, int mods, int batch, fv_stream_t stream);
int fv_scale_cast(const float* x, const float* scale, void* y, int y_dtype, size_t n, fv_stream_t stream);
int fv_column_sum(const void* x, int dtype, float* out, int rows, int cols, int accumulate, fv_stream_t stream);

typedef struct fv_mix_params {
  float lam;
  float one_minus_lam;
  int32_t use_cutmix;
  int32_t yl, yh, xl, xh;
  int32_t reserved;
} fv_mix_params;

int fv_mix_batch(const void* x, void* out, int dtype, int batch, int chans, int height, int width, const void* mix,
                 fv_stream_t stream);
int fv_patch_unfold_mix(const void* img, int img_dtype, void* out, int out_dtype, int batch, int chans, int height,
                        int width, int ph, int pw, const void* mix, fv_stream_t stream);
int fv_mixup_target(const int64_t* labels, float* target, int batch, int classes, double smoothing, const void* mix,
                    fv_stream_t stream);
int fv_label_ce(const void* logits, int logits_dtype, const int64_t* labels, const void* mix, double smoothing,
                float* loss_rows, float* loss, float* dlogits, int32_t* correct_rows, int32_t* n_correct, int batch,
                int classes, fv_stream_t stream);

int fv_patch_unfold_chan(const void* img, int img_dtype, void* out, int out_dtype, int batch, int chans_total,
                         int height, int width, int ph, int pw, const int32_t* sel, int n_sel, int colwise,
                         fv_stream_t stream);
int fv_chan_embed_table(const float* chan_table, const float* bias, const float* pos, float* table, const int32_t* sel,
                        int n_sel, int chans_total, int positions, int dim, fv_stream_t stream);
int fv_chan_embed_scatter(const float* d_chan, float* d_table, const int32_t* sel, int n_sel, int chans_total, int dim,
                          fv_stream_t stream);

int fv_adamw_flat(float* params, const float* grads, float* exp_avg, float* exp_avg_sq, float* ema,
                  void* shadow_bf16, const uint8_t* decay_mask, const float* lr, float* step, float beta1,
                  float beta2, float eps, float weight_decay, float ema_decay, float grad_scale, size_t n,
                  fv_stream_t stream);

int fv_grad_sumsq_blocks(size_t n);
int fv_grad_sumsq_partials(const float* grads, float* partials, size_t n, fv_stream_t stream);
int fv_adamw_flat_groups(float* params, const float* grads, float* exp_avg, float* exp_avg_sq, float* ema,
                         void* shadow_bf16, const uint8_t* group_ids, const float* group_table, int n_groups,
                         const float* lr, float* step, const float* partials, int n_partials, const float* max_norm,
                         float* stats, int skip_nonfinite, float beta1, float beta2, float eps, float ema_decay,
                         float grad_scale, size_t n, fv_stream_t stream);

#ifdef __cplusplus
}
#endif
#endif
```

Baseline: 25700 images/sec.

## Fuse next block's in_proj GEMM into combine/out_proj/addnorm kernel

Adds an INP variant of the combine+out_proj+addnorm kernel. It stages the normalized output tile in shared memory and immediately multiplies it by a fragment-packed in_proj weight, writing the next block's xz directly. This removes a separate in_proj GEMM launch and the global re-read of the normalized activations. It also adds a mixed-layout weight packing kernel that packs all weight layouts in one launch. The cost is more shared memory, register pressure and extra serial work inside the fused kernel.

```diff
diff --git a/fastvim_amd/_lib.py b/fastvim_amd/_lib.py
--- a/fastvim_amd/_lib.py
+++ b/fastvim_amd/_lib.py
@@ -28,6 +28,8 @@
     "fv_mix_batch", "fv_patch_unfold_mix", "fv_mixup_target", "fv_label_ce",
     "fv_patch_unfold_chan", "fv_chan_embed_table", "fv_chan_embed_scatter",
     "fv_mixer_plan",
+    "fv_pack_weight_frags_jobs",
+    "fv_mixer_combine_out_proj_addnorm_inproj_ok", "fv_mixer_combine_out_proj_addnorm_inproj_pk",
 )
 
 
diff --git a/fastvim_amd/csrc/combine_gemm.hip b/fastvim_amd/csrc/combine_gemm.hip
--- a/fastvim_amd/csrc/combine_gemm.hip
+++ b/fastvim_amd/csrc/combine_gemm.hip
@@ -1,5 +1,6 @@
 #include "mixer_common.h"
 #include "packed.h"
+#include "gemm_tiles.h"
 
 namespace {
 
@@ -17,6 +18,9 @@
 #ifndef CG_DBG
 #define CG_DBG 0
 #endif
+constexpr int CG_IP = 4, CG_IKS = CG_N / 32, CG_IS = CG_IP * CG_IKS, CG_IPD = 4, CG_RS4 = 48 * 2 + 16;
+constexpr int CG_O_SL = CG_BM * CG_RSB, CG_SMEM_INP = CG_O_SL + 4 * CG_BM * CG_RS4;
+static_assert(CG_O_SL % 16 == 0 && CG_SMEM_INP >= CG_BM * CG_RSA && 2 * CG_SMEM_INP <= 160 * 1024, "INP: slabs, two workgroups per CU");
 
 struct CgParams {
   const void* xz;
@@ -40,11 +44,13 @@
   float eps;
   int M;
   int d_in;
+  const bf16_t* Win;
+  bf16_t* xz_out;
 };
 
 __device__ __forceinline__ float cg_hsum(f2 v) { return v.x + v.y; }
 
-template <bool PK>
+template <bool PK, bool INP>
 __global__ __launch_bounds__(CG_NT, 2) void combine_out_proj_addnorm_kernel(CgParams p) {
   extern __shared__ __attribute__((aligned(16))) char smem[];
   typedef PairVec<bf16_t, 3> P;
@@ -270,6 +276,18 @@
     }
   __syncthreads();
   if (CG_DBG == 3) return;
+  cg_bf16x8 f4[INP ? CG_IPD : 1][3];
+  const char* ipk = INP ? reinterpret_cast<const char*>(p.Win) + wv * (CG_IS * 3 * 1024) : nullptr;
+  auto ifrag = [&](int nb, int s) { return *reinterpret_cast<const cg_bf16x8*>(ipk + (s * 3 + nb) * 1024 + wpk_lane); };
+  if constexpr (INP) {
+    if (CG_DBG != 5) {
+#pragma unroll
+      for (int s = 0; s < CG_IPD; ++s)
+#pragma unroll
+        for (int nb = 0; nb < 3; ++nb) f4[s][nb] = ifrag(nb, s);
+    }
+    __builtin_amdgcn_sched_barrier(0);
+  }
   constexpr int LPR = 16, RPW = 4, RU = 2, RW = CG_BM / 4;
   const float inv_n = 1.f / (float)CG_N;
   float w[3][4];
@@ -297,7 +315,8 @@
     }
 #pragma unroll
     for (int u = 0; u < RU; ++u) {
-      const int row = tok_of(wv * RW + it * (RPW * RU) + u * RPW + gr);
+      const int rl = wv * RW + it * (RPW * RU) + u * RPW + gr;
+      const int row = tok_of(rl);
       const bool live = row >= 0;
       const size_t base = (size_t)(live ? row : mimg) * CG_N;
       const float sc = sc_u[u];
@@ -333,7 +352,70 @@
         }
         uint2 pk = {pack_bf16x2(o[0], o[1]), pack_bf16x2(o[2], o[3])};
         if (live) *reinterpret_cast<uint2*>(p.y + base + c) = pk;
-      }
+        if constexpr (INP) *reinterpret_cast<uint2*>(smem + rl * CG_RSB + c * 2) = live ? pk : make_uint2(0u, 0u);
+      }
+    }
+  }
+  if constexpr (INP) {
+    __syncthreads();
+    if (CG_DBG != 5) {
+      static_assert(CG_IKS % 2 == 0 && CG_IPD % 2 == 0 && CG_IPD <= CG_IS, "fragments are refilled in k-step pairs inside a pass");
+      char* my = smem + CG_O_SL + wv * (CG_BM * CG_RS4);
+      const char* yfrag = smem + (lane & 15) * CG_RSB + (lane >> 4) * 16;
+      cg_f32x4 acc2[3][4];
+      static_for<CG_IS / 2>([&](auto sp_c) {
+        constexpr int sp = 2 * decltype(sp_c)::value, KP = CG_IKS;
+        if constexpr (sp % KP == 0) {
+#pragma unroll
+          for (int a = 0; a < 3; ++a)
+#pragma unroll
+            for (int b = 0; b < 4; ++b) acc2[a][b] = (cg_f32x4){0.f, 0.f, 0.f, 0.f};
+        }
+        cg_bf16x8 cur[2][3];
+#pragma unroll
+        for (int h = 0; h < 2; ++h)
+#pragma unroll
+          for (int nb = 0; nb < 3; ++nb) cur[h][nb] = f4[(sp + h) % CG_IPD][nb];
+        if constexpr (sp + CG_IPD < CG_IS) {
+#pragma unroll
+          for (int nb = 0; nb < 3; ++nb)
+#pragma unroll
+            for (int h = 0; h < 2; ++h) f4[(sp + h) % CG_IPD][nb] = ifrag(nb, sp + h + CG_IPD);
+        }
+        __builtin_amdgcn_sched_barrier(0);
+#pragma unroll
+        for (int h = 0; h < 2; ++h) {
+          cg_bf16x8 fa[4];
+#pragma unroll
+          for (int mb = 0; mb < 4; ++mb) fa[mb] = *reinterpret_cast<const cg_bf16x8*>(yfrag + mb * 16 * CG_RSB + ((sp + h) % KP) * 64);
+#pragma unroll
+          for (int a = 0; a < 3; ++a)
+#pragma unroll
+            for (int b = 0; b < 4; ++b) acc2[a][b] = __builtin_amdgcn_mfma_f32_16x16x32_bf16(cur[h][a], fa[b], acc2[a][b], 0, 0, 0);
+        }
+        if constexpr (sp % KP == KP - 2) {
+          constexpr int pass = sp / KP, CH = 48 / 8;
+#pragma unroll
+          for (int b = 0; b < 4; ++b)
+#pragma unroll
+            for (int a = 0; a < 3; ++a) {
+              const cg_f32x4 v = acc2[a][b];
+              uint2 pk = {pack_bf16x2(v[0], v[1]), pack_bf16x2(v[2], v[3])};
+              *reinterpret_cast<uint2*>(my + (b * 16 + (lane & 15)) * CG_RS4 + (a * 16 + (lane >> 4) * 4) * 2) = pk;
+            }
+          __builtin_amdgcn_wave_barrier();
+#pragma unroll
+          for (int i = 0; i < CG_BM * CH / 64; ++i) {
+            const int idx = i * 64 + lane, r = idx / CH, ch = idx - r * CH;
+            const int m = tok_of(r);
+            if (m >= 0)
+              *reinterpret_cast<uint4*>(p.xz_out + (long)m * (2 * CG_K) + pass * 192 + wv * 48 + ch * 8) =
+                  *reinterpret_cast<const uint4*>(my + r * CG_RS4 + ch * 16);
+          }
+          __builtin_amdgcn_wave_barrier();
+        }
+        __builtin_amdgcn_sched_barrier(0);
+      });
     }
   }
 }
@@ -346,7 +428,7 @@
          cols > 0 && cols <= 16 && (long)batch * rows * cols * CG_K * 4 < 0x7fffffffL;
 }
 
-static int cg_launch(bool packed, const void* xz, const void* skip, const float* yc, const float* ln_w,
+static int cg_launch(int packed, const void* Win_pk, void* xz_out, const void* xz, const void* skip, const float* yc, const float* ln_w,
                                                  const float* ln_b, float ln_eps, void* g, float* mean, float* rstd_ln,
                                                  int batch, int rows, int cols, int tok_stride_row, int tok_stride_col,
                                                  const void* W, long ldw, const float* residual,
@@ -377,8 +459,13 @@
   p.d_in = CG_K;
   const size_t smem = (size_t)CG_BM * CG_RSA;
   const dim3 grid(batch * fv_cdiv(rows, 4)), block(CG_NT);
-  if (packed || CG_FORCE_PK) hipLaunchKernelGGL(combine_out_proj_addnorm_kernel<true>, grid, block, smem, (hipStream_t)stream, p);
-  else hipLaunchKernelGGL(combine_out_proj_addnorm_kernel<false>, grid, block, smem, (hipStream_t)stream, p);
+  if (packed == 2) {
+    FV_CHECK(Win_pk && xz_out && ((uintptr_t)Win_pk & 15) == 0 && ((uintptr_t)xz_out & 15) == 0 && xz_out != xz,
+             "mixer_combine_out_proj_addnorm_inproj_pk: the packed in_proj weight and its output must be 16-byte aligned, not null");
+    p.Win = (const bf16_t*)Win_pk; p.xz_out = (bf16_t*)xz_out;
+    hipLaunchKernelGGL((combine_out_proj_addnorm_kernel<true, true>), grid, block, CG_SMEM_INP, (hipStream_t)stream, p);
+  } else if (packed || CG_FORCE_PK) hipLaunchKernelGGL((combine_out_proj_addnorm_kernel<true, false>), grid, block, smem, (hipStream_t)stream, p);
+  else hipLaunchKernelGGL((combine_out_proj_addnorm_kernel<false, false>), grid, block, smem, (hipStream_t)stream, p);
   FV_LAUNCH_CHECK();
   return FV_OK;
 }
@@ -392,6 +479,14 @@
   xz, skip, yc, ln_w, ln_b, ln_eps, g, mean, rstd_ln, batch, rows, cols, tok_stride_row, tok_stride_col, W, ldw, residual,    \
       norm_weight, row_scale, rows_per_scale, y, residual_out, rstd, eps, stream
 
-extern "C" int fv_mixer_combine_out_proj_addnorm(CG_ARGS_DECL) { return cg_launch(false, CG_ARGS); }
-
-extern "C" int fv_mixer_combine_out_proj_addnorm_pk(CG_ARGS_DECL) { return cg_launch(true, CG_ARGS); }
+extern "C" int fv_mixer_combine_out_proj_addnorm(CG_ARGS_DECL) { return cg_launch(0, nullptr, nullptr, CG_ARGS); }
+
+extern "C" int fv_mixer_combine_out_proj_addnorm_pk(CG_ARGS_DECL) { return cg_launch(1, nullptr, nullptr, CG_ARGS); }
+
+extern "C" int fv_mixer_combine_out_proj_addnorm_inproj_ok(int batch, int rows, int cols, int tokens_per_patch, int d_inner,
+                                                           int d_model, int dtype) {
+  return fv_mixer_combine_out_proj_addnorm_ok(batch, rows, cols, tokens_per_patch, d_inner, d_model, dtype);
+}
+extern "C" int fv_mixer_combine_out_proj_addnorm_inproj_pk(CG_ARGS_DECL, const void* W_in_pk, void* xz_out) {
+  return cg_launch(2, W_in_pk, xz_out, CG_ARGS);
+}
diff --git a/fastvim_amd/csrc/glue.hip b/fastvim_amd/csrc/glue.hip
--- a/fastvim_amd/csrc/glue.hip
+++ b/fastvim_amd/csrc/glue.hip
@@ -448,6 +448,22 @@
   const int lane = u & 63, t = u >> 6, nb = t % 3, ks = (t / 3) % J.ks_n, wv = t / (3 * J.ks_n);
   const int row = 48 * wv + 16 * nb + (lane & 15), unit_in_row = 4 * ks + (lane >> 4);
   J.dst[blockIdx.y][u] = J.src[blockIdx.y][row * (J.ks_n * 4) + unit_in_row];
+}
+
+constexpr int PKJ_MAX = 96;
+struct PackJobsMixed {
+  const uint16_t* src[PKJ_MAX];
+  uint4* dst[PKJ_MAX];
+  uint8_t steps[PKJ_MAX], kper[PKJ_MAX], nwv[PKJ_MAX], npass[PKJ_MAX];
+  int sn[PKJ_MAX];
+};
+__global__ __launch_bounds__(256) void pack_weight_frags_mixed_kernel(PackJobsMixed J) {
+  const int j = blockIdx.y, steps = J.steps[j], kper = J.kper[j];
+  const int u = blockIdx.x * 256 + threadIdx.x;
+  if (u >= 4 * steps * 3 * 64) return;
+  const int lane = u & 63, t = u >> 6, nb = t % 3, s = (t / 3) % steps, wv = t / (3 * steps);
+  const int n = J.nwv[j] * wv + J.npass[j] * (s / kper) + 16 * nb + (lane & 15), k = 32 * (s % kper) + 8 * (lane >> 4);
+  J.dst[j][u] = *reinterpret_cast<const uint4*>(J.src[j] + (size_t)n * J.sn[j] + k);
 }
 
 int unfold_store_bytes(int gw, int gjc, size_t patch_bytes) {
@@ -707,3 +723,25 @@
   FV_LAUNCH_CHECK();
   return FV_OK;
 }
+
+extern "C" int fv_pack_weight_frags_jobs(const void* const* srcs, void* const* dsts, const int* layouts, int njobs, fv_stream_t stream) {
+  FV_CHECK(srcs && dsts && layouts && njobs > 0 && njobs <= PKJ_MAX, "pack_weight_frags_jobs: 1..%d jobs", PKJ_MAX);
+  PackJobsMixed J{};
+  int most = 0;
+  for (int j = 0; j < njobs; ++j) {
+    FV_CHECK(srcs[j] && dsts[j] && srcs[j] != dsts[j], "pack_weight_frags_jobs: null or aliased pointer in job %d", j);
+    FV_CHECK(((uintptr_t)srcs[j] & 15) == 0 && ((uintptr_t)dsts[j] & 15) == 0, "pack_weight_frags_jobs: job %d is not 16-byte aligned", j);
+    J.src[j] = (const uint16_t*)srcs[j];
+    J.dst[j] = (uint4*)dsts[j];
+    switch (layouts[j]) {
+      case FV_PACK_K384: J.steps[j] = 12; J.kper[j] = 12; J.nwv[j] = 48; J.npass[j] = 0;   J.sn[j] = 384; break;
+      case FV_PACK_K768: J.steps[j] = 24; J.kper[j] = 24; J.nwv[j] = 48; J.npass[j] = 0;   J.sn[j] = 768; break;
+      case FV_PACK_IN:   J.steps[j] = 24; J.kper[j] = 6;  J.nwv[j] = 48; J.npass[j] = 192; J.sn[j] = 192; break;
+      default: FV_CHECK(false, "pack_weight_frags_jobs: job %d has unknown layout %d", j, layouts[j]);
+    }
+    most = J.steps[j] > most ? J.steps[j] : most;
+  }
+  hipLaunchKernelGGL(pack_weight_frags_mixed_kernel, dim3(4 * most * 3 * 64 / 256, njobs), dim3(256), 0, (hipStream_t)stream, J);
+  FV_LAUNCH_CHECK();
+  return FV_OK;
+}
diff --git a/fastvim_amd/flat.py b/fastvim_amd/flat.py
--- a/fastvim_amd/flat.py
+++ b/fastvim_amd/flat.py
@@ -23,7 +23,7 @@
 
 def _drop_derived_shadows(model):
     for p in model.parameters():
-        for a in ("_fv_shadow_t", "_fv_shadow_t_version", "_fv_shadow_pk", "_fv_shadow_pk_version"):
+        for a in ("_fv_shadow_t", "_fv_shadow_t_version", "_fv_shadow_pk", "_fv_shadow_pk_version", "_fv_shadow_pkin", "_fv_shadow_pkin_version"):
             if hasattr(p, a):
                 delattr(p, a)
     for mod in model.modules():
@@ -140,15 +140,16 @@
                     self._t_src.append(w._fv_shadow)
                     self._t_dst.append(wt)
                     self._t_params.append(w)
-        self._pk_jobs = {768: ([], [], []), 384: ([], [], [])}
+        self._pk_jobs = {768: ([], [], []), 384: ([], [], []), "in": ([], [], [])}
         if shadow_dtype == torch.bfloat16 and dev.type == "cuda":
             for w, wt in zip(self._t_params, self._t_dst):
                 self._add_packed(768, w, wt)
+                self._add_packed("in", w, w._fv_shadow)
             for mod in mixers.values():
                 w = getattr(getattr(mod, "out_proj", None), "weight", None)
                 if w is not None and tuple(w.shape) == (192, 384) and w.requires_grad and getattr(w, "_fv_shadow", None) is not None:
                     self._add_packed(384, w, w._fv_shadow)
-        self._pk_dst = self._pk_jobs[768][1] + self._pk_jobs[384][1]
+        self._pk_dst = self._pk_jobs[768][1] + self._pk_jobs[384][1] + self._pk_jobs["in"][1]
         self._tx_src, self._tx_dst, self._tx_params = [], [], []
         if shadow_dtype == torch.bfloat16 and dev.type == "cuda":
             for mod in mixers.values():
@@ -175,10 +176,13 @@
         group_wgrads(True)
         _SideStream.enabled = False
 
+    _PK_ATTR = {768: "_fv_shadow_pk", 384: "_fv_shadow_pk", "in": "_fv_shadow_pkin"}
+
     def _add_packed(self, K, w, src):
-        pk = torch.empty(192 * K, device=src.device, dtype=src.dtype)
-        w._fv_shadow_pk = pk
-        w._fv_shadow_pk_version = -1
+        pk = torch.empty(src.numel(), device=src.device, dtype=src.dtype)
+        attr = self._PK_ATTR[K]
+        setattr(w, attr, pk)
+        setattr(w, attr + "_version", -1)
         srcs, dsts, params = self._pk_jobs[K]
         srcs.append(src)
         dsts.append(pk)
@@ -227,18 +231,22 @@
         self.refresh_transposed()
 
     def refresh_transposed(self):
-        from .mixer_ops import pack_weight_frags, transpose_bf16_batched
+        from .mixer_ops import PACK_IN, PACK_K384, PACK_K768, pack_weight_frags_jobs, transpose_bf16_batched
         for src, dst, params in ((self._t_src, self._t_dst, self._t_params),
                                  (getattr(self, "_tx_src", []), getattr(self, "_tx_dst", []), getattr(self, "_tx_params", []))):
             if src:
                 transpose_bf16_batched(src, dst)
                 for p in params:
                     p._fv_shadow_t_version = p._version
-        for srcs, dsts, params in getattr(self, "_pk_jobs", {}).values():
-            if srcs:
-                pack_weight_frags(srcs, dsts)
-                for p in params:
-                    p._fv_shadow_pk_version = p._version
+        srcs, dsts, lays = [], [], []
+        for key, (s_, d_, params) in getattr(self, "_pk_jobs", {}).items():
+            srcs += s_
+            dsts += d_
+            lays += [{768: PACK_K768, 384: PACK_K384, "in": PACK_IN}[key]] * len(s_)
+            for p in params:
+                setattr(p, self._PK_ATTR[key] + "_version", p._version)
+        if srcs:
+            pack_weight_frags_jobs(srcs, dsts, lays)
 
     @property
     def world_size(self):
diff --git a/fastvim_amd/mamba_simple_faster.py b/fastvim_amd/mamba_simple_faster.py
--- a/fastvim_amd/mamba_simple_faster.py
+++ b/fastvim_amd/mamba_simple_faster.py
@@ -42,17 +42,36 @@
     return was
 
 
-def _shadow_pk(w, cdt, plain):
-    pk = getattr(w, "_fv_shadow_pk", None)
-    if pk is None or pk.dtype != cdt or not _PackedWeights.enabled:
+class _InProjPhase:
+    enabled = True
+
+
+def use_inproj_phase(on):
+    was = _InProjPhase.enabled
+    _InProjPhase.enabled = bool(on)
+    return was
+
+
+def _shadow_packed(w, cdt, plain, attr, layout, enabled):
+    pk = getattr(w, attr, None)
+    if pk is None or pk.dtype != cdt or not enabled:
         return None
-    if w._version != w._fv_shadow_pk_version:
+    if w._version != getattr(w, attr + "_version"):
         if not (plain.is_contiguous() and plain.numel() == pk.numel()):
             return None
         with torch.no_grad():
-            M.pack_weight_frags([plain], [pk])
-        w._fv_shadow_pk_version = w._version
+            M.pack_weight_frags_jobs([plain], [pk], [layout])
+        setattr(w, attr + "_version", w._version)
     return pk
+
+
+def _shadow_pk(w, cdt, plain):
+    return _shadow_packed(w, cdt, plain, "_fv_shadow_pk", M.PACK_K768 if plain.shape[-1] == 768 else M.PACK_K384,
+                          _PackedWeights.enabled)
+
+
+def _shadow_pkin(w, cdt, plain):
+    return _shadow_packed(w, cdt, plain, "_fv_shadow_pkin", M.PACK_IN, _PackedWeights.enabled and _InProjPhase.enabled)
 
 
 def _wx2_shadow_t(fv):
@@ -259,7 +278,7 @@
         d = W_out.shape[0]
         Mrows = B * Ltok
         with torch.autocast("cuda", enabled=False):
-            y, res_out, rstd, w32, row_scale, rows_per_scale = _out_proj_add_norm_fwd(g, W_out, residual, norm_w, eps, row_scale, cdt)
+            y, res_out, rstd, w32, row_scale, rows_per_scale, _ = _out_proj_add_norm_fwd(g, W_out, residual, norm_w, eps, row_scale, cdt)
         ctx.save_for_backward(g, W_out, res_out, w32, rstd, row_scale)
         ctx.rows_per_scale = rows_per_scale
         ctx.cdt = cdt
@@ -317,7 +336,7 @@
                       pack["cols"], pack["transposed"], out=pack["out"])
 
 
-def _out_proj_add_norm_fwd(g, W_out, residual, norm_w, eps, row_scale, cdt, W_in=None, pack=None):
+def _out_proj_add_norm_fwd(g, W_out, residual, norm_w, eps, row_scale, cdt, W_in=None, pack=None, W_in_chain=None):
     B, Ltok, d_in = g.shape
     d = W_out.shape[0]
     Mrows = B * Ltok
@@ -339,11 +358,16 @@
     lib = L.lib()
     if pack is not None:
         if xz is None and W_out_c.stride(1) == 1 and W_out_c.stride(0) % 8 == 0 and W_out_c.data_ptr() % 16 == 0:
-            y, res_out, rstd = M.combine_out_proj_addnorm(pack["xz"], pack["skip"], pack["yc"], pack["ln_w"], pack["ln_b"],
-                                                          pack["eps"], pack["rows"], pack["cols"], pack["transposed"],
-                                                          pack["out"], W_out_c, res2, w32, row_scale, rows_per_scale, eps,
-                                                          W_out_pk=_shadow_pk(W_out, cdt, W_out_c))
-            return y, res_out, rstd, w32, row_scale, rows_per_scale
+            W_out_pk = _shadow_pk(W_out, cdt, W_out_c)
+            W_in_pk = None
+            if W_in_chain is not None and W_out_pk is not None and tuple(W_in_chain.shape) == (768, 192):
+                W_in_plain = _shadow(W_in_chain, cdt)
+                W_in_pk = _shadow_pkin(W_in_chain, cdt, W_in_plain)
+            res = M.combine_out_proj_addnorm(pack["xz"], pack["skip"], pack["yc"], pack["ln_w"], pack["ln_b"],
+                                             pack["eps"], pack["rows"], pack["cols"], pack["transposed"],
+                                             pack["out"], W_out_c, res2, w32, row_scale, rows_per_scale, eps,
+                                             W_out_pk=W_out_pk, W_in_pk=W_in_pk)
+            return (*res[:3], w32, row_scale, rows_per_scale, res[3] if W_in_pk is not None else None)
         resolve_combine(pack)
     rc = lib.fv_gemm_bf16_addnorm2(
         L.ptr(g2), L.ptr(W_out_c), L.ptr(res2), L.ptr(w32), L.ptr(row_scale), L.i32(rows_per_scale),
@@ -351,9 +375,7 @@
         ctypes.c_long(d_in), ctypes.c_float(eps), L.ptr(W_in_c), L.ptr(xz),
         L.i32(W_in.shape[0] if xz is not None else 0), ctypes.c_long(d), L.stream_of(g2))
     L.check(rc, "gemm_bf16_addnorm")
-    if W_in is not None:
-        return y, res_out, rstd, w32, row_scale, rows_per_scale, xz
-    return y, res_out, rstd, w32, row_scale, rows_per_scale
+    return y, res_out, rstd, w32, row_scale, rows_per_scale, xz
 
 
 class ChainedBlockFn(torch.autograd.Function):
@@ -374,15 +396,13 @@
         assert pack is None or pack["out"][0].data_ptr() == g_prev.data_ptr()
         with torch.autocast("cuda", enabled=False):
             if pack is not None:
-                y, res_out, rstd, w32, rs, rps = _out_proj_add_norm_fwd(g_prev, W_out_prev, residual, norm_w, eps, row_scale,
-                                                                      cdt, pack=pack)
-                xz = None
+                y, res_out, rstd, w32, rs, rps, xz = _out_proj_add_norm_fwd(g_prev, W_out_prev, residual, norm_w, eps, row_scale, cdt,
+                                                                          pack=pack, W_in_chain=W_in if b_in is None else None)
             elif ChainedBlockFn.in_proj_in_launch and b_in is None:
                 y, res_out, rstd, w32, rs, rps, xz = _out_proj_add_norm_fwd(g_prev, W_out_prev, residual, norm_w, eps,
                                                                           row_scale, cdt, W_in=W_in)
             else:
-                y, res_out, rstd, w32, rs, rps = _out_proj_add_norm_fwd(g_prev, W_out_prev, residual, norm_w, eps, row_scale, cdt)
-                xz = None
+                y, res_out, rstd, w32, rs, rps, xz = _out_proj_add_norm_fwd(g_prev, W_out_prev, residual, norm_w, eps, row_scale, cdt)
         fctx = _Ctx()
         fctx.precomputed_xz = xz
         fctx.defer_combine = ChainedBlockFn.defer
@@ -435,9 +455,10 @@
             d_prev = g_prev.shape[2]
             W2 = _shadow(W_out_prev, cdt) if d_prev % 128 == 0 else None
             W_in_t = _shadow_t(ctx.W_in, cdt)
+            W_in_pk = _shadow_pk(ctx.W_in, cdt, W_in_t)
             p2, dx, dres_in, pw, nb, dg_prev = M.conv_pool_bwd_dgrad(
                 xz, d_o, dxc, dxc2, cw2, cb, cwb2, cb_b, D, D_b, dxz, rows, cols, transposed, scaling, W_in_t, gg, r, rstd,
-                w32, row_scale, ctx.rows_per_scale, W2=W2, conv_grad_out=conv_grad_out, W_in_pk=_shadow_pk(ctx.W_in, cdt, W_in_t))
+                w32, row_scale, ctx.rows_per_scale, W2=W2, conv_grad_out=conv_grad_out, W_in_pk=W_in_pk)
             out.update(dx=dx, dres_in=dres_in, pw=pw, nb=nb, dg_prev=dg_prev)
             return p2
 
diff --git a/fastvim_amd/mixer_ops.py b/fastvim_amd/mixer_ops.py
--- a/fastvim_amd/mixer_ops.py
+++ b/fastvim_amd/mixer_ops.py
@@ -182,7 +182,7 @@
 
 
 def combine_out_proj_addnorm(xz, skip, yc, ln_w, ln_b, ln_eps, rows, cols, transposed, out, W_out_c, residual2, norm_w32,
-                             row_scale, rows_per_scale, eps, W_out_pk=None):
+                             row_scale, rows_per_scale, eps, W_out_pk=None, *, W_in_pk=None):
     B, Ltok, two_d = xz.shape
     d = W_out_c.shape[0]
     Mrows = B * Ltok
@@ -196,12 +196,21 @@
         fn, W_arg, ldw = L.lib().fv_mixer_combine_out_proj_addnorm_pk, W_out_pk, two_d // 2
     else:
         fn, W_arg, ldw = L.lib().fv_mixer_combine_out_proj_addnorm, W_out_c, W_out_c.stride(0)
+    extra, xz_next = (), None
+    if W_in_pk is not None:
+        if W_out_pk is None:
+            raise ValueError("combine_out_proj_addnorm: W_in_pk needs the packed out_proj weight W_out_pk too")
+        assert W_in_pk.dtype == torch.bfloat16 and W_in_pk.is_contiguous() and W_in_pk.numel() == 768 * d and d == PACK_ROWS
+        xz_next = torch.empty(Mrows, 768, device=xz.device, dtype=torch.bfloat16)
+        fn, extra = L.lib().fv_mixer_combine_out_proj_addnorm_inproj_pk, (L.ptr(W_in_pk), L.ptr(xz_next))
     rc = fn(
         L.ptr(xz), L.ptr(skip), L.ptr(yc), L.ptr(ln_w), L.ptr(ln_b), f32(ln_eps), L.ptr(g), L.ptr(mean), L.ptr(rstd_ln),
         L.i32(B), L.i32(rows), L.i32(cols), L.i32(s_i), L.i32(s_j), L.ptr(W_arg), ctypes.c_long(ldw),
         L.ptr(residual2), L.ptr(norm_w32), L.ptr(row_scale), L.i32(rows_per_scale), L.ptr(y), L.ptr(res_out), L.ptr(rstd),
-        f32(eps), L.stream_of(xz))
+        f32(eps), L.stream_of(xz), *extra)
     L.check(rc, "mixer_combine_out_proj_addnorm")
+    if W_in_pk is not None:
+        return y, res_out, rstd, xz_next
     return y, res_out, rstd
 
 
@@ -422,6 +431,38 @@
         ins = (ctypes.c_void_p * k)(*[t.data_ptr() for t in a])
         outs = (ctypes.c_void_p * k)(*[t.data_ptr() for t in b])
         L.check(lib.fv_pack_weight_frags_batched(ins, outs, L.i32(k), L.i32(K), L.stream_of(a[0])), "pack_weight_frags_batched")
+
+
+PACK_K384, PACK_K768, PACK_IN = 0, 1, 2
+_PACK_SHAPES = {PACK_K384: (PACK_ROWS, 384), PACK_K768: (PACK_ROWS, 768), PACK_IN: (768, PACK_ROWS)}
+
+
+def pack_index_in():
+    u = torch.arange(768 * PACK_ROWS // 8)
+    lane, t = u % 64, u // 64
+    nb, s, wv = t % 3, (t // 3) % 24, t // 72
+    p, ks = s // 6, s % 6
+    return torch.stack([192 * p + 48 * wv + 16 * nb + (lane % 16), 32 * ks + 8 * (lane // 16)], dim=1)
+
+
+def pack_in_frags_ref(W):
+    assert tuple(W.shape) == (768, PACK_ROWS)
+    idx = pack_index_in().to(W.device)
+    cols = idx[:, 1:2] + torch.arange(8, device=W.device)
+    return W[idx[:, 0:1], cols].reshape(-1)
+
+
+def pack_weight_frags_jobs(srcs, dsts, layouts):
+    lib = L.lib()
+    for lo in range(0, len(srcs), 96):
+        a, b, c = srcs[lo:lo + 96], dsts[lo:lo + 96], [int(x) for x in layouts[lo:lo + 96]]
+        assert all(t.dtype == torch.bfloat16 and t.is_contiguous() and tuple(t.shape) == _PACK_SHAPES[k] for t, k in zip(a, c))
+        assert all(t.dtype == torch.bfloat16 and t.is_contiguous() and t.numel() == s_.numel() for t, s_ in zip(b, a))
+        k = len(a)
+        ins = (ctypes.c_void_p * k)(*[t.data_ptr() for t in a])
+        outs = (ctypes.c_void_p * k)(*[t.data_ptr() for t in b])
+        lay = (ctypes.c_int * k)(*c)
+        L.check(lib.fv_pack_weight_frags_jobs(ins, outs, lay, L.i32(k), L.stream_of(a[0])), "pack_weight_frags_jobs")
 
 
 XPROJ_WIDTHS = (44, 56, 80, 96, 112, 34, 36, 38, 64)
diff --git a/include/fastvim_hip.h b/include/fastvim_hip.h
--- a/include/fastvim_hip.h
+++ b/include/fastvim_hip.h
@@ -193,6 +193,14 @@
                                          long ldw, const float* residual, const float* norm_weight,
                                          const float* row_scale, int rows_per_scale, void* y, float* residual_out,
                                          float* rstd, float eps, fv_stream_t stream);
+int fv_mixer_combine_out_proj_addnorm_inproj_ok(int batch, int rows, int cols, int tokens_per_patch, int d_inner,
+                                                int d_model, int dtype);
+int fv_mixer_combine_out_proj_addnorm_inproj_pk(const void* xz, const void* skip, const float* yc, const float* ln_w,
+                                         const float* ln_b, float ln_eps, void* g, float* mean, float* rstd_ln, int batch,
+                                         int rows, int cols, int tok_stride_row, int tok_stride_col, const void* W,
+                                         long ldw, const float* residual, const float* norm_weight,
+                                         const float* row_scale, int rows_per_scale, void* y, float* residual_out,
+                                         float* rstd, float eps, fv_stream_t stream, const void* W_in_pk, void* xz_out);
 
 int fv_mixer_conv_pool_bwd_dgrad_ok(int batch, int rows, int cols, int tokens_per_patch, int d_inner, int d_model,
                                     int pool_max, int dtype);
@@ -220,6 +228,9 @@
 
 int fv_pack_weight_frags_batched(const void* const* srcs, void* const* dsts, int njobs, int K, fv_stream_t stream);
 
+enum { FV_PACK_K384 = 0, FV_PACK_K768 = 1, FV_PACK_IN = 2 };
+int fv_pack_weight_frags_jobs(const void* const* srcs, void* const* dsts, const int* layouts, int njobs, fv_stream_t stream);
+
 int fv_gemm_bf16_addnorm2(const void* A, const void* W, const float* residual, const float* norm_weight,
                           const float* row_scale, int rows_per_scale, void* y, float* residual_out, float* rstd, int M,
                           int N, int K, long lda, long ldw, float eps, const void* W2, void* C2, int N2, long ldw2,
```

Result: faster. 26450 images/sec (median of 6 runs) (+2.9%).
